# wolny/pytorch-3dunet

Measured on AMD Instinct MI355X. Metric: volumetric patches/sec (fwd+bwd), UNet3D f_maps=32 patch 64x128x128, higher is better.
Workload: dtype f32

## Files before the change

include/u3d.h:

```cpp
#ifndef U3D_H
#define U3D_H

#include <stddef.h>
#include <stdint.h>

#ifdef __cplusplus
extern "C" {
#endif

#define U3D_VERSION 128

#define U3D_OK 0
#define U3D_EINVAL (-1)
#define U3D_EHIP (-2)
#define U3D_EARCH (-3)
#define U3D_EWORKSPACE (-4)

typedef void* u3d_stream_t;

typedef struct {
    const float* p0;
    const float* p1;
    const int32_t* zmap;
    const int32_t* ymap;
    const int32_t* xmap;
    const float* affine;
    int32_t C0, C1;
    int32_t D1, H1, W1;
} u3d_src_t;

int u3d_version(void);
const char* u3d_last_error(void);
int u3d_check_device(int device);
int u3d_set_tuning(int key, int value);
int u3d_set_profile_buffer(void* device_buffer, size_t bytes);
int u3d_debug_stream_pass(int device, u3d_stream_t stream, float* buf, long long n, int blocks, int passes, double min_seconds);
int u3d_debug_mfma_f32_rate(int device, u3d_stream_t stream, float* sink, int iters, int mode, double* flop_out);

size_t u3d_packed_weight_floats(int Cin, int Cout, int mode);
int u3d_pack_weights(int device, u3d_stream_t stream, const float* w, int Cout, int Cin, int mode, float* packed);
typedef struct {
    const float* w;
    float* packed;
    int64_t first;
    int32_t Cout, Cin, mode, cin_stride;
} u3d_pack_desc_t;
int u3d_pack_weights_batch(int device, u3d_stream_t stream, const u3d_pack_desc_t* descs_device, int n,
                           int64_t total_floats);
long long u3d_pack_weights_cells_blocks(const float* w, int Cin, int Cout, int mode, int cin_stride);
int u3d_pack_weights_batch_cells(int device, u3d_stream_t stream, const u3d_pack_desc_t* descs_device, int n, long long total_blocks);

int u3d_conv3d(int device, u3d_stream_t stream, const u3d_src_t* src, const float* packed_w, float* out,
               int N, int D, int H, int W, int Cout, int relu, double* out_stats, const u3d_src_t* gx,
               double* gstats);

int u3d_conv3d_residual(int device, u3d_stream_t stream, const u3d_src_t* src, const float* packed_w, float* out,
                        int N, int D, int H, int W, int Cout, int relu, double* out_stats, const float* residual);

long long u3d_conv3d_workspace_floats(int N, int D, int H, int W, int Cin, int Cout);
int u3d_conv3d_ex(int device, u3d_stream_t stream, const u3d_src_t* src, const float* packed_w, float* out, int N,
                  int D, int H, int W, int Cout, int relu, double* out_stats, const u3d_src_t* gx, double* gstats,
                  const float* residual, float* workspace, long long workspace_floats);

int u3d_conv3d_ex_reps(int device, u3d_stream_t stream, const u3d_src_t* src, const float* packed_w, float* out, int N,
                       int D, int H, int W, int Cout, int relu, double* out_stats, const u3d_src_t* gx, double* gstats,
                       const float* residual, float* workspace, long long workspace_floats, int stat_reps);

long long u3d_subpixel_packed_floats(int C1, int Cout);
long long u3d_subpixel_dgrad_packed_floats(int Cout, int C1);
int u3d_pack_subpixel_dgrad_weights(int device, u3d_stream_t stream, const float* w, int Cout, int Cin_total, int c_off,
                                    int C1, float* packed);
int u3d_subpixel_conv_dgrad(int device, u3d_stream_t stream, const float* dz, const float* packed, const float* x_low,
                            float* dlow, double* gstats, int N, int D1, int H1, int W1, int C1, int Cout);
int u3d_subpixel_conv_dgrad_reps(int device, u3d_stream_t stream, const float* dz, const float* packed, const float* x_low, float* dlow,
                                 double* gstats, int N, int D1, int H1, int W1, int C1, int Cout, int reps);
int u3d_pack_subpixel_weights(int device, u3d_stream_t stream, const float* w, int Cout, int Cin_total, int c_off, int C1,
                              float* packed);
long long u3d_subpixel_fwd_workspace_floats(int N, int D1, int H1, int W1, int C1, int Cout);
int u3d_subpixel_conv_fwd(int device, u3d_stream_t stream, const float* low, const float* affine,
                          long long affine_sample_stride, const float* packed, float* out, int N, int D1, int H1, int W1,
                          int C1, int Cout, float* workspace, long long workspace_floats);

size_t u3d_wgrad_workspace_floats(int N, int D, int H, int W, int Cin, int Cout);
int u3d_conv3d_wgrad(int device, u3d_stream_t stream, const u3d_src_t* src, const float* dz, float* dw, int N,
                     int D, int H, int W, int Cout, float* workspace, size_t workspace_floats);

int u3d_conv3d_variant(int N, int D, int H, int W, int Cin, int Cout, int src_kind, int has_workspace);
int u3d_conv3d_wgrad_variant(int N, int D, int H, int W, int Cin, int Cout, int src_kind);

int u3d_conv3d_wgrad_strided(int device, u3d_stream_t stream, const u3d_src_t* src, const float* dz, float* dw,
                             int dw_cin_stride, int N, int D, int H, int W, int Cout, float* workspace,
                             size_t workspace_floats);

typedef struct u3d_gn_bwd_job {
    const double* gstats_lo;
    const double* gstats_hi;
    const float* mean_rstd;
    const float* gamma;
    float* dgamma;
    float* dbeta;
    float* coef;
    float* coef_hi;
    double count;
    int32_t C0, C1, N, G;
    float hi_scale;
    int32_t reps_lo;
    int32_t reps_hi;
    int32_t reserved;
} u3d_gn_bwd_job_t;
int u3d_conv3d_wgrad_job_supported(int N, int C, int G);
int u3d_conv3d_wgrad_job(int device, u3d_stream_t stream, const u3d_src_t* src, const float* dz, float* dw, int dw_cin_stride,
                         int N, int D, int H, int W, int Cout, float* workspace, size_t workspace_floats,
                         const u3d_gn_bwd_job_t* job);

long long u3d_subpixel_wgrad_workspace_floats(int N, int D1, int H1, int W1, int C1, int Cout);
int u3d_subpixel_conv_wgrad(int device, u3d_stream_t stream, const float* low, const float* affine,
                            long long affine_sample_stride, const float* dz, float* dw, int dw_cin_stride, int N, int D1,
                            int H1, int W1, int C1, int Cout, float* workspace, long long workspace_floats);

int u3d_subpixel_conv_fwd_win(int device, u3d_stream_t stream, const float* low, const float* affine, long long affine_sample_stride,
                              const float* packed, float* out, int N, int D1, int H1, int W1, int C1, int Cout, const int* win);
int u3d_subpixel_conv_dgrad_win(int device, u3d_stream_t stream, const float* dz, const float* packed, const float* x_low, float* dlow,
                                double* gstats, int N, int D1, int H1, int W1, int C1, int Cout, const int* win);
int u3d_subpixel_conv_wgrad_win(int device, u3d_stream_t stream, const float* low, const float* affine, long long affine_sample_stride,
                                const float* dz, float* dw, int dw_cin_stride, int N, int D1, int H1, int W1, int C1, int Cout,
                                float* workspace, long long workspace_floats, const int* win);
int u3d_conv3d_box(int device, u3d_stream_t stream, const u3d_src_t* src, const float* packed_w, float* out, int N, int D, int H, int W,
                   int Cout, const int* out_box, const int* in_mask);
int u3d_conv3d_wgrad_box(int device, u3d_stream_t stream, const u3d_src_t* src, const float* dz, float* dw, int N, int D, int H, int W,
                         int Cout, float* workspace, size_t workspace_floats, const int* box);
int u3d_gn_bwd_apply_children(int device, u3d_stream_t stream, const float* dlow, const float* x, const float* coef, int Ctot, int coff,
                              int N, int D1, int H1, int W1, int C, int ez, int ey, int ex, int relu_mask, float* out);
int u3d_chan_stats_children(int device, u3d_stream_t stream, const float* x_low, int N, int D1, int H1, int W1, int C, int ez, int ey,
                            int ex, double* stats);
int u3d_nearest_childsum_add(int device, u3d_stream_t stream, const float* dv, const float* x_low, float* dlow, double* gstats, int N,
                             int D, int H, int W, int D1, int H1, int W1, int C, const int32_t* zlo, const int32_t* ylo,
                             const int32_t* xlo, int cz, int cy, int cx);

int u3d_conv3d_small_cin_fwd(int device, u3d_stream_t stream, const float* x, const float* affine, const float* w,
                             float* out, int N, int D, int H, int W, int Cin, int Cout, int relu, double* out_stats);
int u3d_conv3d_small_cin_fwd_reps(int device, u3d_stream_t stream, const float* x, const float* affine, const float* w, float* out, int N,
                                  int D, int H, int W, int Cin, int Cout, int relu, double* out_stats, int reps);
size_t u3d_small_cin_bwd_workspace_floats(int N, int D, int H, int W, int Cin, int Cout);
int u3d_conv3d_small_cin_bwd(int device, u3d_stream_t stream, const float* x, const float* affine, const float* dz,
                             const float* w, float* dw, double* gstats, int N, int D, int H, int W, int Cin, int Cout,
                             float* workspace, size_t workspace_floats);

int u3d_conv3d_naive(int device, u3d_stream_t stream, const u3d_src_t* src, const float* w, float* out, int N,
                     int D, int H, int W, int Cin, int Cout, int relu, int flip);

int u3d_chan_stats(int device, u3d_stream_t stream, const u3d_src_t* src, int N, int D, int H, int W,
                   double* stats);
int u3d_chan_stats_reps(int device, u3d_stream_t stream, const u3d_src_t* src, int N, int D, int H, int W, double* stats, int reps);
int u3d_gn_finalize(int device, u3d_stream_t stream, const double* stats0, int C0, double scale0,
                    const double* stats1, int C1, double scale1, int N, int G, double count, const float* gamma,
                    const float* beta, float eps, float* affine, float* mean_rstd);

int u3d_gn_bwd_finalize(int device, u3d_stream_t stream, const double* gstats, const float* mean_rstd,
                        const float* gamma, int N, int C, int G, double count, float* dgamma, float* dbeta,
                        float* coef);
int u3d_gn_finalize_split(int device, u3d_stream_t stream, const double* stats0, int C0, double scale0, const double* stats1, int C1,
                          double scale1, int N, int G, double count, const float* gamma, const float* beta, float eps, float* affine,
                          float* mean_rstd, int Csplit, float* affine_lo, float* affine_hi);
int u3d_gn_finalize_reps(int device, u3d_stream_t stream, const double* stats0, int C0, double scale0, int reps0, const double* stats1,
                         int C1, double scale1, int reps1, int N, int G, double count, const float* gamma, const float* beta, float eps,
                         float* affine, float* mean_rstd, int Csplit, float* affine_lo, float* affine_hi);
int u3d_gn_bwd_finalize_split_supported(int N, int C, int G);
int u3d_gn_bwd_finalize_split(int device, u3d_stream_t stream, const double* gstats_lo, int C0, const double* gstats_hi, int C1,
                              const float* mean_rstd, const float* gamma, int N, int G, double count, float* dgamma, float* dbeta,
                              float* coef, float hi_scale, float* coef_hi);

int u3d_gn_bwd_apply(int device, u3d_stream_t stream, const float* dg, int Cdg, int coff, const float* x, int Cx,
                     const float* coef, int Ctot, int64_t voxels_per_n, int N, int relu_mask, float* out);

int u3d_gn_bwd_apply_add(int device, u3d_stream_t stream, const float* dg, int Cdg, int coff, const float* x, int Cx,
                         const float* coef, int Ctot, int64_t voxels_per_n, int N, int relu_mask, const float* add,
                         float* out);

int u3d_gn_bwd_apply_up(int device, u3d_stream_t stream, const float* dg, int Cdg, int coff, const float* x1,
                        int C1, const float* coef, int Ctot, int N, int D, int H, int W, int D1, int H1, int W1,
                        const int32_t* zlo, const int32_t* ylo, const int32_t* xlo, int relu_mask, float* out);

int u3d_maxpool2_fwd(int device, u3d_stream_t stream, const float* x, int N, int D, int H, int W, int C,
                     float* out, uint8_t* argmax, double* out_stats);
int u3d_maxpool2_bwd_merge(int device, u3d_stream_t stream, const float* dg, const float* pooled,
                           const uint8_t* argmax, const float* coef, const float* skip_grad, const float* e,
                           int N, int D, int H, int W, int C, int relu_mask, float* out);
int u3d_maxpool2_bwd_merge_gn(int device, u3d_stream_t stream, const float* dg, const float* pooled,
                              const uint8_t* argmax, const float* coef, const float* skip_dg, int Cdg,
                              const float* skip_coef, int Ctot, const float* e, int N, int D, int H, int W, int C,
                              int relu_mask, float* out);

int u3d_conv1x1_head_fwd(int device, u3d_stream_t stream, const float* x, const float* w, const float* b, int N,
                         int64_t V, int Cin, int Cout, int act, float* logits, float* probs);
int u3d_conv1x1_head_bwd(int device, u3d_stream_t stream, const float* dlogits, const float* x, const float* w,
                         int N, int64_t V, int Cin, int Cout, int relu_mask, float* dx, double* acc);
int u3d_conv1x1_head_bwd_reps(int device, u3d_stream_t stream, const float* dlogits, const float* x, const float* w, int N, int64_t V,
                              int Cin, int Cout, int relu_mask, float* dx, double* acc, int reps);
int u3d_cvt_f64_f32(int device, u3d_stream_t stream, const double* src, float* dst, int64_t n);
int u3d_cvt_f64_f32_sum(int device, u3d_stream_t stream, const double* src, float* dst, int64_t n, int reps);

typedef struct {
    float* p;
    const float* g;
    float* m;
    float* v;
    int64_t first;
    int64_t numel;
} u3d_adam_desc_t;
int u3d_adam_step(int device, u3d_stream_t stream, const u3d_adam_desc_t* descs_device, int n, int64_t total_padded, double lr,
                  double beta1, double beta2, double eps, double weight_decay, int64_t step);

int u3d_conv1x1_fwd(int device, u3d_stream_t stream, const float* x, const float* w, const float* bias, float* y, int N,
                    int64_t V, int Cin, int Cout, double* out_stats);
int u3d_conv1x1_bwd(int device, u3d_stream_t stream, const float* dy, const float* x, const float* w, int N, int64_t V,
                    int Cin, int Cout, float* dx, double* acc);
int u3d_pack_convtr_weights(int device, u3d_stream_t stream, const float* w, int Cin, int Cout, int mode, float* packed);
int u3d_convtr3d_fwd(int device, u3d_stream_t stream, const float* x, const float* w, float* t, int N, int D1, int H1,
                     int W1, int Cin, int Cout, const float* packed);
long long u3d_convtr3d_subpixel_packed_floats(int Cin, int Cout);
int u3d_pack_convtr3d_subpixel(int device, u3d_stream_t stream, const float* w, int Cin, int Cout, float* packed);
int u3d_convtr3d_fwd_subpixel(int device, u3d_stream_t stream, const float* x, const float* packed, float* t, int N, int D1,
                              int H1, int W1, int Cin, int Cout);
int u3d_convtr3d_bwd(int device, u3d_stream_t stream, const float* dt, const float* x, const float* w, int N, int D1,
                     int H1, int W1, int Cin, int Cout, int relu_mask, float* dx, double* acc, const float* packed_t);
int u3d_nearest_add_fwd(int device, u3d_stream_t stream, const float* skip, const float* t, const int32_t* zmap,
                        const int32_t* ymap, const int32_t* xmap, int N, int D, int H, int W, int Dt, int Ht, int Wt, int C,
                        float* out, double* out_stats);
int u3d_nearest_sum_bwd(int device, u3d_stream_t stream, const float* dj, const int32_t* zlo, const int32_t* ylo,
                        const int32_t* xlo, int N, int D, int H, int W, int Dt, int Ht, int Wt, int C, float* dt);

int u3d_se_gate_fwd(int device, u3d_stream_t stream, const double* ystats, double count, const float* w1, const float* b1,
                    const float* w2, const float* b2, int N, int C, int Cr, float* s, float* h, float* gc);
int u3d_se_apply_fwd(int device, u3d_stream_t stream, const float* y, const float* gc, const float* ws, const float* bs, int N,
                     int64_t V, int C, int mode, float* out, float* a);
int u3d_se_bwd_reduce(int device, u3d_stream_t stream, const float* dout, const float* y, const float* gc, const float* a,
                      const float* ws, int N, int64_t V, int C, int mode, float* dls, double* acc_gc, double* acc_ws);
int u3d_se_gate_bwd(int device, u3d_stream_t stream, const double* acc_gc, const float* gc, const float* h, const float* s,
                    const float* w1, const float* w2, int N, int C, int Cr, double count, float* dz2, float* dz1, float* ds,
                    float* dw1, float* db1, float* dw2, float* db2);
int u3d_se_bwd_apply(int device, u3d_stream_t stream, const float* dout, const float* y, const float* gc, const float* a,
                     const float* ws, const float* dls, const float* ds, int N, int64_t V, int C, int mode, int relu_mask,
                     float* out);

long long u3d_bce_dice_scratch_doubles(int N, int C, int64_t V);
int u3d_bce_dice_fwd(int device, u3d_stream_t stream, const float* logits, const float* target, const float* weight,
                     int N, int C, int64_t V, float w_bce, float w_dice, float eps, double* sums, float* loss,
                     float* coef);
int u3d_bce_dice_bwd(int device, u3d_stream_t stream, const float* logits, const float* target, const float* coef,
                     const float* grad_out, int N, int C, int64_t V, float* dlogits);

int u3d_conv3d_bf16_supported(int Cin, int Cout);
long long u3d_packed_weight_bf16_elems(int Cin, int Cout, int mode);
int u3d_pack_weights_bf16(int device, u3d_stream_t stream, const float* w, int Cout, int Cin, int mode, void* packed);
long long u3d_pack_weights_bf16_blocks(int Cin, int Cout, int mode);
int u3d_pack_weights_bf16_batch(int device, u3d_stream_t stream, const u3d_pack_desc_t* descs_device, int n, long long total_blocks);
int u3d_conv3d_bf16(int device, u3d_stream_t stream, const float* x, const float* affine, const void* packed_w, float* out,
                    int N, int D, int H, int W, int Cin, int Cout, int relu, double* out_stats, const float* gx,
                    double* gstats, const float* residual);
long long u3d_conv3d_bf16_workspace_floats(int N, int D, int H, int W, int Cin, int Cout);
int u3d_conv3d_bf16_tile_variant(int N, int D, int H, int W, int Cin, int Cout, int b16);
int u3d_conv3d_bf16_ex(int device, u3d_stream_t stream, const float* x, const float* affine, const void* packed_w, float* out,
                       int N, int D, int H, int W, int Cin, int Cout, int relu, double* out_stats, const float* gx,
                       double* gstats, const float* residual, float* workspace, long long workspace_floats);

long long u3d_packed_weight_f32s_elems(int Cin, int Cout, int mode);
// ... 125 lines not shown
```

pytorch-3dunet_amd/csrc/u3d_conv.hip:

```cpp
#include <type_traits>
#include <utility>

#include "u3d_common.h"
#include "u3d_gn.h"
#include "u3d_subpix.h"

int g_u3d_tune[24] = {0};

namespace cv {
constexpr int TZ = 4, TY = 8, TX = 8;
constexpr int HZ = TZ + 2, HY = TY + 2, HX = TX + 2;
constexpr int CC = 16;
constexpr int CS = 16;
constexpr int RS = HX * CS + 4;
constexpr int PS = HY * RS;
constexpr int TILE_FLOATS = HZ * PS + 4;
constexpr int CNT_OFF = 2 * TILE_FLOATS;
constexpr int RED_OFF = CNT_OFF + 16;
constexpr int LDS_FLOATS = RED_OFF + 4 * 3 * 32 * 2;
constexpr int NITEMS = HZ * HY * HX * (CC / 4);
constexpr int NIT = (NITEMS + 255) / 256;
constexpr int NSTEP = 27 * (CC / 8);
constexpr int NSTEP_PAIRY = 36 * (CC / 8);
constexpr int NSTEP_N16 = 27;
// ... 965 lines not shown
            using X1 = std::integral_constant<int, 0xB1>;
            using X2 = std::integral_constant<int, 0x4E>;
            const int vrow = ((n * D + z) * H + T.y0) * W + T.x0 + vl;
            const int xrow = ((n * p.gx.D1 + (z >> 1)) * p.gx.H1 + (T.y0 >> 1)) * p.gx.W1 + ((T.x0 + vl) >> 1);
#pragma unroll
            for (int nt = 0; nt < NT; ++nt) {
                f32x4 q1 = {0.f, 0.f, 0.f, 0.f}, q2 = {0.f, 0.f, 0.f, 0.f};
                f32x4 tq[4 * MT];
#pragma unroll
                for (int mt = 0; mt < MT; ++mt)
#pragma unroll
                    for (int bi = 0; bi < 4; ++bi) {
                        const float a0 = acc[mt][nt][4 * bi + 0], a1 = acc[mt][nt][4 * bi + 1];
                        const float a2 = acc[mt][nt][4 * bi + 2], a3 = acc[mt][nt][4 * bi + 3];
                        const float t0 = xlane(a1, X1{}), t1 = xlane(a0, X1{}), t2 = xlane(a3, X1{}), t3 = xlane(a2, X1{});
                        const float c0 = odd ? t0 : a0, c1 = odd ? a1 : t1, c2 = odd ? t2 : a2, c3 = odd ? a3 : t3;
                        const float u0 = xlane(c2, X2{}), u2 = xlane(c0, X2{}), u1 = xlane(c3, X2{}), u3 = xlane(c1, X2{});
                        tq[4 * mt + bi] = f32x4{hi ? u0 : c0, hi ? u1 : c1, hi ? c2 : u2, hi ? c3 : u3};
                    }
                const int ysh = PAIRY ? (cq >> 2) : 0;
                const int co = PAIRY ? 4 * (cq & 3) : (cb * NT + nt) * 32 + 4 * cq;
                auto yoff = [&](int st) { return PAIRY ? 2 * st + ysh : st; };
                const bool cok = co < p.Cout && (!RAG || T.x0 + vl < W);
                auto row_in = [&](int st) { return !RAG || (z < D && T.y0 + yoff(st) < H); };
                float* orow = p.out + (size_t)vrow * p.Cout + co;
                const bool xfrom0 = co < p.gx.C0 || !cok;
                const float* xb = !cok ? p.gx.p0 : (xfrom0 ? p.gx.p0 + co : p.gx.p1 + (co - p.gx.C0));
                const int xcs = xfrom0 ? p.gx.C0 : p.gx.C1;
#pragma unroll
                for (int half = 0; half < MT; ++half) {
                    f32x4 xv[4];
                    if (want_g) {
#pragma unroll
                        for (int k = 0; k < 4; ++k) {
                            const int yo = yoff(4 * half + k);
                            int xi = xfrom0 ? vrow + yo * W : xrow + (yo >> 1) * p.gx.W1;
                            if constexpr (RAG) xi = (cok && row_in(4 * half + k)) ? xi : 0;
                            xv[k] = *reinterpret_cast<const f32x4*>(xb + (size_t)xi * xcs);
                        }
                    } else if (p.res) {
#pragma unroll
                        for (int k = 0; k < 4; ++k) {
                            size_t ri = (size_t)(vrow + yoff(4 * half + k) * W) * p.Cout + (cok ? co : 0);
                            if constexpr (RAG) ri = (cok && row_in(4 * half + k)) ? ri : 0;
                            xv[k] = *reinterpret_cast<const f32x4*>(p.res + ri);
                        }
                    }
#pragma unroll
                    for (int k = 0; k < 4; ++k) {
                        const int st = 4 * half + k;
                        if (!row_in(st)) continue;
                        f32x4 val = tq[st];
                        if (p.res) val += xv[k];
                        if (p.relu) {
#pragma unroll
                            for (int e = 0; e < 4; ++e) val[e] = fmaxf(val[e], 0.f);
                        }
                        if (cok) *reinterpret_cast<f32x4*>(orow + (size_t)yoff(st) * W * p.Cout) = val;
                        if (RAG || p.Cout % 32 != 0) {
#pragma unroll
                            for (int e = 0; e < 4; ++e) val[e] = cok ? val[e] : 0.f;
                        }
                        q1 += val;
                        q2 += want_g ? val * xv[k] : val * val;
                    }
                }
                if (want_stats || want_g) {
                    if constexpr (CARRY) {
                        sq1 += q1;
                        sq2 += q2;
                    } else {
                        stat_reduce(q1, q2, n, nt, co - (PAIRY ? 0 : (cb * NT + nt) * 32));
                    }
                }
            }
        }
        if (ntiles == DBG_TILE) U3D_DBG_STAMP(22);
        ++ntiles;
        if (!has_next_tile || TN.n != T.n || TN.cb != T.cb) {
            if constexpr (CARRY) {
                if (want_stats || want_g) {
                    if constexpr (N16) {
#pragma unroll
                        for (int e = 0; e < 4; ++e) {
                            float a = sq1[e], b2 = sq2[e];
#pragma unroll
                            for (int msk = 8; msk > 0; msk >>= 1) {
                                a += __shfl_xor(a, msk);
                                b2 += __shfl_xor(b2, msk);
                            }
                            if (v16 == 0) {
                                double* r = &red[(((T.n & 1) * NT) * 32 + 4 * kq + e) * 2];
                                __hip_atomic_fetch_add(r, (double)a, __ATOMIC_RELAXED, __HIP_MEMORY_SCOPE_WORKGROUP);
                                __hip_atomic_fetch_add(r + 1, (double)b2, __ATOMIC_RELAXED, __HIP_MEMORY_SCOPE_WORKGROUP);
                            }
                        }
                    } else {
                        const int cq_ = (l >> 2) & 7;
                        stat_reduce(sq1, sq2, T.n, 0, PAIRY ? 4 * (cq_ & 3) : 4 * cq_);
                    }
                    sq1 = f32x4{0.f, 0.f, 0.f, 0.f};
                    sq2 = f32x4{0.f, 0.f, 0.f, 0.f};
                }
            }
            flush_stats(T.n, T.cb);
        }
        if (!has_next_tile) break;
        if constexpr (!ZEROC) {
#pragma unroll
            for (int mt = 0; mt < MT; ++mt)
#pragma unroll
                for (int nt = 0; nt < NT; ++nt)
#pragma unroll
                    for (int r = 0; r < 16; ++r) acc[mt][nt][r] = 0.f;
        }
        wi = nwi;
        dT = dTN;
        T = TN;
        wq = wqn;
    }
    if constexpr (DBG) {
        if (l == 0) dbgw[4] = ntiles;
    }
    U3D_DBG_STAMP(6);
}

namespace wg {
constexpr int TZ = 2, TY = 8, TX = 8;
constexpr int HZ = TZ + 2, HY = TY + 2, HX = TX + 2;
constexpr int CC = 32;
constexpr int CSg = 32, RSg = HX * CSg, PSg = HY * RSg;
constexpr int G_FLOATS = HZ * PSg;
constexpr int TV = TZ * TY * TX;
constexpr int DZ_FLOATS = TV * 32;
constexpr int DUMMY_OFF = G_FLOATS + DZ_FLOATS;
constexpr int BUF_FLOATS = G_FLOATS + DZ_FLOATS + 4;
constexpr int LDS_FLOATS = 2 * BUF_FLOATS;
constexpr int NTHR = 512;
constexpr int NITEMS_G = HZ * HY * HX * (CC / 4);
constexpr int NIT_G = (NITEMS_G + NTHR - 1) / NTHR;
constexpr int NIT_DZ = TV * 8 / NTHR;
constexpr int MAX_MAP_INTS = 4096;
}

struct WgradParams {
    u3d_src_t src;
    const float* dz;
    float* partial;
    int N, D, H, W, Cout;
    int nchunks, nkb, S;
    int tz, ty, tx, ntiles, tps;
    int vec, dzvec;
    int bz0, by0, bx0, bz1, by1, bx1;
};

template <bool VEC, bool REG = false, bool PAIR = false>
__global__ __launch_bounds__(512, 2) void conv3d_wgrad_kernel(const WgradParams p) {
    using namespace wg;
    constexpr int NA = PAIR ? 4 : 7;
    extern __shared__ __attribute__((aligned(16))) float lds[];
    int* zmapl = reinterpret_cast<int*>(lds + 2 * BUF_FLOATS);
    __builtin_amdgcn_s_setprio(3);
    const int t = threadIdx.x;
    const int l = t & 63, i = l & 31, h = l >> 5;
    const int w = __builtin_amdgcn_readfirstlane(t >> 6);
    const int tg = w & 3, hf = w >> 2;

    const int logical = u3d_xcd_remap(blockIdx.x, gridDim.x);
    const int kb = logical % p.nkb;
    const int chunk = (logical / p.nkb) % p.nchunks;
    const int s = logical / (p.nkb * p.nchunks);
    const int D = p.D, H = p.H, W = p.W;
    const int Ctot = p.src.C0 + p.src.C1;
    int* ymapl = zmapl + D;
    int* xmapl = ymapl + H;
    if (p.src.C1 > 0) {
        for (int k = t; k < D; k += NTHR) zmapl[k] = p.src.zmap[k];
        for (int k = t; k < H; k += NTHR) ymapl[k] = p.src.ymap[k];
        for (int k = t; k < W; k += NTHR) xmapl[k] = p.src.xmap[k];
        __syncthreads();
    }

    f32x16 acc[NA];
#pragma unroll
    for (int k = 0; k < NA; ++k)
#pragma unroll
        for (int r = 0; r < 16; ++r) acc[k][r] = 0.f;

    const int q = t & 7, tv = t >> 3;
    const int cq = chunk * CC + 4 * q;
    const int co = kb * 32 + 4 * q;
    const bool cok = cq < Ctot, from0 = cq < p.src.C0, dcok = co < p.Cout;
    const float* gbase = !cok ? p.src.p0 : (from0 ? p.src.p0 + cq : p.src.p1 + (cq - p.src.C0));
    const int Cs = (from0 || !cok) ? p.src.C0 : p.src.C1;
    const float* dzbase = p.dz + (dcok ? co : 0);

    constexpr int NPFC = NIT_G + NIT_DZ;
    int rel[NPFC], loff[NPFC];
    unsigned fz0 = 0, fz1 = 0, fy0 = 0, fy1 = 0, fx0 = 0, fx1 = 0, fdead = 0;
    if constexpr (REG) {
        const int vz = D % TZ ? D % TZ : TZ, vy = H % TY ? H % TY : TY, vx = W % TX ? W % TX : TX;
#pragma unroll
        for (int it = 0; it < NIT_G; ++it) {
            const int vox = tv + 64 * it;
            const int hz = vox / (HY * HX);
            const int rem = vox - hz * (HY * HX);
            const int hy = rem / HX;
            const int hx = rem - hy * HX;
            const bool in = vox < HZ * HY * HX;
            rel[it] = from0 ? ((hz - 1) * H + (hy - 1)) * W + (hx - 1)
                            : (((hz - 1) >> 1) * p.src.H1 + ((hy - 1) >> 1)) * p.src.W1 + ((hx - 1) >> 1);
            loff[it] = in ? hz * PSg + hy * RSg + hx * CSg + 4 * q : DUMMY_OFF;
            fz0 |= (in && hz == 0 ? 1u : 0u) << it;
            fz1 |= (in && hz > vz ? 1u : 0u) << it;
            fy0 |= (in && hy == 0 ? 1u : 0u) << it;
            fy1 |= (in && hy > vy ? 1u : 0u) << it;
            fx0 |= (in && hx == 0 ? 1u : 0u) << it;
            fx1 |= (in && hx > vx ? 1u : 0u) << it;
            fdead |= (in && cok ? 0u : 1u) << it;
        }
#pragma unroll
        for (int it = 0; it < NIT_DZ; ++it) {
            const int vox = tv + 64 * it;
            rel[NIT_G + it] = ((vox >> 6) * H + ((vox >> 3) & 7)) * W + (vox & 7);
            loff[NIT_G + it] = G_FLOATS + vox * 32 + 4 * q;
            fz1 |= ((vox >> 6) >= vz ? 1u : 0u) << (NIT_G + it);
            fy1 |= (((vox >> 3) & 7) >= vy ? 1u : 0u) << (NIT_G + it);
            fx1 |= ((vox & 7) >= vx ? 1u : 0u) << (NIT_G + it);
        }
        fdead |= (dcok ? 0u : 3u) << NIT_G;
    }
    auto tile_invalid = [&](int z0, int y0, int x0) {
        unsigned inv = fdead;
        inv |= z0 == 0 ? fz0 : 0u;
        inv |= z0 + TZ >= D ? fz1 : 0u;
        inv |= y0 == 0 ? fy0 : 0u;
        inv |= y0 + TY >= H ? fy1 : 0u;
        inv |= x0 == 0 ? fx0 : 0u;
        inv |= x0 + TX >= W ? fx1 : 0u;
        return inv;
    };

    struct TileC {
        int n, z0, y0, x0;
        int base, dzb;
        unsigned inv;
    };
    struct TileIdx {
        int xi, yi, zi, n;
    };
    auto tile_decode = [&](int tile) {
        TileIdx d;
        d.xi = tile % p.tx;
        tile /= p.tx;
        d.yi = tile % p.ty;
        tile /= p.ty;
        d.zi = tile % p.tz;
        d.n = tile / p.tz;
        return d;
    };
    auto tile_next = [&](const TileIdx& a) {
        TileIdx r = a;
        r.xi += 1;
        int c = r.xi >= p.tx ? 1 : 0;
        r.xi = c ? 0 : r.xi;
        r.yi += c;
        c = r.yi >= p.ty ? 1 : 0;
        r.yi = c ? 0 : r.yi;
        r.zi += c;
        c = r.zi >= p.tz ? 1 : 0;
        r.zi = c ? 0 : r.zi;
        r.n += c;
        return r;
    };
    auto tile_coords = [&](const TileIdx& d) {
        TileC c;
        c.x0 = (REG ? 0 : p.bx0) + d.xi * TX;
        c.y0 = (REG ? 0 : p.by0) + d.yi * TY;
        c.z0 = (REG ? 0 : p.bz0) + d.zi * TZ;
        c.n = d.n;
        c.base = c.dzb = 0;
        c.inv = 0;
        if constexpr (REG) {
            c.dzb = ((c.n * D + c.z0) * H + c.y0) * W + c.x0;
            const int b1 = ((c.n * p.src.D1 + (c.z0 >> 1)) * p.src.H1 + (c.y0 >> 1)) * p.src.W1 + (c.x0 >> 1);
            c.base = from0 ? c.dzb : b1;
            c.inv = tile_invalid(c.z0, c.y0, c.x0);
        }
        return c;
    };
    auto g_item = [&](const TileC& c, int it, int& off, bool& ok, int& idx) {
        const int vox = tv + 64 * it;
        const int hz = vox / (HY * HX);
        const int rem = vox - hz * (HY * HX);
        const int hy = rem / HX;
        const int hx = rem - hy * HX;
        off = vox < HZ * HY * HX ? hz * PSg + hy * RSg + hx * CSg + 4 * q : DUMMY_OFF;
        const int gz = c.z0 - 1 + hz, gy = c.y0 - 1 + hy, gxx = c.x0 - 1 + hx;
        ok = cok && vox < HZ * HY * HX && gz >= 0 && gz < D && gy >= 0 && gy < H && gxx >= 0 && gxx < W;
        const int zc = min(max(gz, 0), D - 1), yc = min(max(gy, 0), H - 1), xc = min(max(gxx, 0), W - 1);
        idx = ((c.n * D + zc) * H + yc) * W + xc;
        if (p.src.C1 > 0) {
            const int idx1 = ((c.n * p.src.D1 + zmapl[zc]) * p.src.H1 + ymapl[yc]) * p.src.W1 + xmapl[xc];
            idx = from0 ? idx : idx1;
        }
        idx = ok ? idx : 0;
    };
    auto dz_item = [&](const TileC& c, int it, bool& ok, int& idx) {
        const int vox = tv + 64 * it;
        const int z = c.z0 + (vox >> 6), y = c.y0 + ((vox >> 3) & 7), x = c.x0 + (vox & 7);
        ok = dcok && z < p.bz1 && y < p.by1 && x < p.bx1;
        idx = ok ? ((c.n * D + z) * H + y) * W + x : 0;
    };
    auto load_affine = [&](int n, f32x4& ga, f32x4& gb) {
        ga = f32x4{1.f, 1.f, 1.f, 1.f};
        gb = f32x4{0.f, 0.f, 0.f, 0.f};
        if (p.src.affine) {
            const float* ap = p.src.affine + ((size_t)n * Ctot + (cok ? cq : 0)) * 2;
            const f32x4 lo = *reinterpret_cast<const f32x4*>(ap);
            const f32x4 hi = *reinterpret_cast<const f32x4*>(ap + 4);
            ga = f32x4{lo[0], lo[2], hi[0], hi[2]};
            gb = f32x4{lo[1], lo[3], hi[1], hi[3]};
        }
    };
    auto pf_load = [&](const TileC& c, int k) {
        bool ok;
        int idx, off;
        if constexpr (REG) {
            ok = ((c.inv >> k) & 1u) == 0;
            if (k < NIT_G) return *reinterpret_cast<const f32x4*>(gbase + (size_t)(ok ? c.base + rel[k] : 0) * Cs);
            return *reinterpret_cast<const f32x4*>(dzbase + (size_t)(ok ? c.dzb + rel[k] : 0) * p.Cout);
        }
        if (k < NIT_G) {
            g_item(c, k, off, ok, idx);
            return *reinterpret_cast<const f32x4*>(gbase + (size_t)idx * Cs);
        }
        dz_item(c, k - NIT_G, ok, idx);
        return *reinterpret_cast<const f32x4*>(dzbase + (size_t)idx * p.Cout);
    };
    auto pf_store = [&](float* buf, const TileC& c, int k, f32x4 raw, const f32x4& ga, const f32x4& gb) {
        bool ok;
        int idx, off;
        if constexpr (REG) {
            ok = ((c.inv >> k) & 1u) == 0;
            f32x4 val = k < NIT_G ? raw * ga + gb : raw;
#pragma unroll
            for (int e = 0; e < 4; ++e) val[e] = ok ? val[e] : 0.f;
            *reinterpret_cast<f32x4*>(&buf[loff[k]]) = val;
            return;
        }
        if (k < NIT_G) {
            g_item(c, k, off, ok, idx);
            f32x4 val = raw * ga + gb;
#pragma unroll
            for (int e = 0; e < 4; ++e) val[e] = ok ? val[e] : 0.f;
            *reinterpret_cast<f32x4*>(&buf[off]) = val;
        } else {
            dz_item(c, k - NIT_G, ok, idx);
#pragma unroll
            for (int e = 0; e < 4; ++e) raw[e] = ok ? raw[e] : 0.f;
            *reinterpret_cast<f32x4*>(&buf[G_FLOATS + (tv + 64 * (k - NIT_G)) * 32 + 4 * q]) = raw;
        }
    };
    auto stage_scalar = [&](float* buf, const TileC& c) {
        f32x4 ga, gb;
        u3d_load_affine(p.src.affine, c.n, Ctot, cq, false, ga, gb);
#pragma unroll 1
        for (int it = 0; it < NIT_G; ++it) {
            const int vox = tv + 64 * it;
            if (vox >= HZ * HY * HX) continue;
            const int hz = vox / (HY * HX), rem = vox - hz * (HY * HX), hy = rem / HX, hx = rem - hy * HX;
            const int gz = c.z0 - 1 + hz, gy = c.y0 - 1 + hy, gxx = c.x0 - 1 + hx;
            f32x4 val = {0.f, 0.f, 0.f, 0.f};
            if (gz >= 0 && gz < D && gy >= 0 && gy < H && gxx >= 0 && gxx < W) {
                int v0, v1;
                u3d_vox_index(p.src, c.n, gz, gy, gxx, D, H, W, v0, v1);
                val = u3d_load_quad(p.src, v0, v1, cq, false) * ga + gb;
            }
            *reinterpret_cast<f32x4*>(&buf[hz * PSg + hy * RSg + hx * CSg + 4 * q]) = val;
        }
#pragma unroll 1
        for (int it = 0; it < NIT_DZ; ++it) {
            const int vox = tv + 64 * it;
            const int z = c.z0 + (vox >> 6), y = c.y0 + ((vox >> 3) & 7), x = c.x0 + (vox & 7);
            f32x4 val = {0.f, 0.f, 0.f, 0.f};
            if (z < p.bz1 && y < p.by1 && x < p.bx1) {
                const float* sp = p.dz + ((size_t)((c.n * D + z) * H + y) * W + x) * p.Cout + co;
#pragma unroll
                for (int e = 0; e < 4; ++e)
                    if (co + e < p.Cout) val[e] = sp[e];
            }
            *reinterpret_cast<f32x4*>(&buf[G_FLOATS + vox * 32 + 4 * q]) = val;
        }
    };

    constexpr int NPF = NIT_G + NIT_DZ;
    constexpr int ST0 = 20;
    static_assert(2 * (NPF - 1) < ST0 && ST0 + NPF <= 32, "prefetch schedule must fit the 32 groups of a tile");
    const int tile_begin = s * p.tps, tile_end = min(p.ntiles, (s + 1) * p.tps);

    TileIdx tix = tile_decode(tile_begin);
    if (tile_begin < tile_end) {
        const TileC c = tile_coords(tix);
        if constexpr (VEC) {
            f32x4 ga, gb;
            load_affine(c.n, ga, gb);
            f32x4 v[NPF];
#pragma unroll
            for (int k = 0; k < NPF; ++k) v[k] = pf_load(c, k);
#pragma unroll
            for (int k = 0; k < NPF; ++k) pf_store(lds, c, k, v[k], ga, gb);
        } else {
            stage_scalar(lds, c);
        }
    }
    __syncthreads();

    int abase[NA];
#pragma unroll
    for (int k = 0; k < NA; ++k) {
        const int tap = PAIR ? 2 * (tg + 4 * k) + (i >> 4) : tg + 4 * k;
        const int toff = tap < 27 ? (tap / 9) * PSg + ((tap / 3) % 3) * RSg + (tap % 3) * CSg : 0;
        abase[k] = (PAIR ? (i & 15) : i) + h * CSg + hf * PSg + toff;
    }
    int bbase = G_FLOATS + (hf * 64 + h) * 32 + i;
    int cur = 0;
    __builtin_amdgcn_s_setprio(0);

    f32x4 gan = {1.f, 1.f, 1.f, 1.f}, gbn = {0.f, 0.f, 0.f, 0.f};
    int n_aff = -1;
    for (int tile = tile_begin; tile < tile_end; ++tile) {
        const bool has_next = tile + 1 < tile_end;
        if (has_next) tix = tile_next(tix);
        const TileC cn = tile_coords(tix);
        float* nbuf = lds + (cur ^ 1) * BUF_FLOATS;
        f32x4 v[NPF];
        if constexpr (VEC) {
            if (cn.n != n_aff) {
                load_affine(cn.n, gan, gbn);
                n_aff = cn.n;
            }
        }
        const float* gl = lds + cur * BUF_FLOATS;

        float aop[2][NA], bop[2];
        bop[0] = gl[bbase];
#pragma unroll
        for (int k = 0; k < NA; ++k) aop[0][k] = gl[abase[k]];
#pragma unroll
        for (int g = 0; g < 32; ++g) {
            if constexpr (VEC) {
                if (g % 2 == 0 && g / 2 < NPF) v[g / 2] = pf_load(cn, g / 2);
                if (g >= ST0 && g - ST0 < NPF) pf_store(nbuf, cn, g - ST0, v[g - ST0], gan, gbn);
            }
            if (g + 1 < 32) {
                const int row = (g + 1) >> 2, tq = (g + 1) & 3;
                const int goff = row * RSg + 2 * tq * CSg;
                bop[(g + 1) & 1] = gl[bbase + (row * 8 + 2 * tq) * 32];
#pragma unroll
                for (int k = 0; k < NA; ++k) aop[(g + 1) & 1][k] = gl[abase[k] + goff];
            }
            __builtin_amdgcn_sched_barrier(0);
#pragma unroll
            for (int k = 0; k < NA; ++k) acc[k] = __builtin_amdgcn_mfma_f32_32x32x2f32(aop[g & 1][k], bop[g & 1], acc[k], 0, 0, 0);
            __builtin_amdgcn_sched_barrier(0);
        }
        if constexpr (!VEC) {
            if (has_next) stage_scalar(nbuf, cn);
        }
        __syncthreads();
        cur ^= 1;
    }

    __builtin_amdgcn_s_setprio(3);
    float* red = lds;
    if (hf == 1) {
#pragma unroll
        for (int k = 0; k < NA; ++k)
#pragma unroll
            for (int r = 0; r < 16; ++r) red[((tg * 7 + k) * 16 + r) * 64 + l] = acc[k][r];
    }
    __syncthreads();
    if (hf == 0) {
        float* dst = p.partial + ((size_t)((s * p.nchunks + chunk) * p.nkb + kb) * 27) * 1024;
#pragma unroll
        for (int k = 0; k < NA; ++k) {
#pragma unroll
            for (int r = 0; r < 16; ++r) {
                const int row = (r & 3) + 8 * (r >> 2) + 4 * h;
                const int tap = PAIR ? 2 * (tg + 4 * k) + (row >> 4) : tg + 4 * k;
                const int c = PAIR ? (row & 15) : row;
                if (tap < 27) dst[((size_t)tap * 32 + c) * 32 + i] = acc[k][r] + red[((tg * 7 + k) * 16 + r) * 64 + l];
            }
        }
    }
}

template <int G>
__global__ __launch_bounds__(256) void wgrad_reduce_kernel(const float* __restrict__ partial, float* __restrict__ dw,
                                                           int S, int nchunks, int nkb, int Cin, int Cout, int cstride,
                                                           int has_job, u3d_gn_bwd_job_t job) {
    __shared__ float red[4][64];
    if (has_job && blockIdx.x == 0) {
        extern __shared__ double shb[];
        u3d_gn_bwd_finalize_body(job.gstats_lo, job.mean_rstd, job.gamma, job.N, job.C0 + job.C1, job.G, job.count, 1, 1, job.dgamma,
                                 job.dbeta, job.coef, job.gstats_hi, job.C0, job.hi_scale, job.coef_hi, shb, job.reps_lo, job.reps_hi);
        return;
    }
    const long long total = (long long)Cin * 27 * Cout;
    const int lane = G == 1 ? (int)threadIdx.x : (int)(threadIdx.x & 63), grp = G == 1 ? 0 : (int)(threadIdx.x >> 6);
    const long long idx = (long long)(blockIdx.x - (has_job ? 1 : 0)) * (G == 1 ? 256 : 64) + lane;
    float sum = 0.f;
    int k = 0, tap = 0, c = 0;
    if (idx < total) {
        k = (int)(idx % Cout);
        const long long r = idx / Cout;
        tap = (int)(r % 27);
        c = (int)(r / 27);
        const int chunk = c >> 5, kb = k >> 5;
        const size_t off = ((size_t)(chunk * nkb + kb) * 27 + tap) * 1024 + (c & 31) * 32 + (k & 31);
        const size_t sstride = (size_t)nchunks * nkb * 27 * 1024;
        const int per = (S + G - 1) / G;
        const int s0 = grp * per, s1 = min(S, s0 + per);
        float a0 = 0.f, a1 = 0.f, a2 = 0.f, a3 = 0.f;
        int s = s0;
        for (; s + 3 < s1; s += 4) {
            a0 += partial[(size_t)s * sstride + off];
            a1 += partial[(size_t)(s + 1) * sstride + off];
            a2 += partial[(size_t)(s + 2) * sstride + off];
            a3 += partial[(size_t)(s + 3) * sstride + off];
        }
        for (; s < s1; ++s) a0 += partial[(size_t)s * sstride + off];
        sum = (a0 + a1) + (a2 + a3);
    }
    if constexpr (G == 1) {
        if (idx < total) dw[((size_t)k * cstride + c) * 27 + tap] = sum;
    } else {
        red[grp][lane] = sum;
        __syncthreads();
        if (grp == 0 && idx < total)
            dw[((size_t)k * cstride + c) * 27 + tap] = (red[0][lane] + red[1][lane]) + (red[2][lane] + red[3][lane]);
    }
}

__device__ __forceinline__ int pack_image_of(long long idx, int nchunks, int ntot, long long& id) {
    const long long std_total = ((long long)nchunks * cv::NSTEP + cv::PACK_PAD) * ntot * 256;
    const long long pair_total = ((long long)nchunks * cv::NSTEP_PAIRY + cv::PACK_PAD) * 256;
    if (idx < std_total) {
        id = idx;
        return 0;
    }
    if (idx < std_total + pair_total) {
        id = idx - std_total;
        return 1;
    }
    id = idx - std_total - pair_total;
    return 2;
}

__device__ __forceinline__ float pack_elem_n16(const float* __restrict__ w, int Cout, int Cin, int cstride, int mode, int nchunks,
                                               long long id) {
    const int j = (int)(id & 3);
    const int lane = (int)((id >> 2) & 63);
    const long long r = id >> 8;
    const int tap = (int)(r % cv::NSTEP_N16), ch = (int)(r / cv::NSTEP_N16);
    const int kc = ch * 16 + 4 * (lane >> 4) + j, nc = lane & 15;
    if (ch >= nchunks) return 0.f;
    if (mode == 0) return (kc < Cin && nc < Cout) ? w[((size_t)nc * cstride + kc) * 27 + tap] : 0.f;
    return (kc < Cout && nc < Cin) ? w[((size_t)kc * cstride + nc) * 27 + (26 - tap)] : 0.f;
}

__device__ __forceinline__ float pack_elem(const float* __restrict__ w, int Cout, int Cin, int cstride, int mode, int nchunks,
                                           int ntot, long long idx) {
    long long id;
    const int image = pack_image_of(idx, nchunks, ntot, id);
    if (image == 2) return pack_elem_n16(w, Cout, Cin, cstride, mode, nchunks, id);
    const bool pair = image == 1;
    const int j = (int)(id & 3);
    const int lane = (int)((id >> 2) & 63);
    long long r = id >> 8;
    const int nstep = pair ? cv::NSTEP_PAIRY : cv::NSTEP;
    const int ntg = pair ? 0 : (int)(r % ntot);
    if (!pair) r /= ntot;
    const int st = (int)(r % nstep);
    const int ch = (int)(r / nstep);
    const int kc = ch * 16 + 8 * (st & 1) + 4 * (lane >> 5) + j;
    int tap = st >> 1;
    int nc = ntg * 32 + (lane & 31);
    bool tap_ok = true;
    if (pair) {
        const int tz = tap / 12, ty4 = (tap / 3) % 4, tx = tap % 3;
        const int ty = ty4 - ((lane & 31) >> 4);
        tap_ok = ty >= 0 && ty <= 2;
        tap = (tz * 3 + ty) * 3 + tx;
        nc = lane & 15;
    }
    float v = 0.f;
    if (ch >= nchunks || !tap_ok) {
    } else if (mode == 0) {
        if (kc < Cin && nc < Cout) v = w[((size_t)nc * cstride + kc) * 27 + tap];
    } else {
        if (kc < Cout && nc < Cin) v = w[((size_t)kc * cstride + nc) * 27 + (26 - tap)];
    }
    return v;
}
// ... 598 lines not shown
        const dim3 rgrid((unsigned)slots), rblock(256);
        const bool virt = p.src.C1 > 0;
        const bool noaff = p.src.affine == nullptr && g_u3d_tune[7] == 0;
        p.dbg = (!ragged && g_u3d_prof_buf && (size_t)slots * 4 <= g_u3d_prof_records) ? g_u3d_prof_buf : nullptr;
        if (ragged) {
            if (Cout <= 16 && nt == 1 && p.ntot == 1) {
                p.wp = packed_w + ((size_t)p.nchunks * cv::NSTEP + cv::PACK_PAD) * 256 + ((size_t)p.nchunks * cv::NSTEP_PAIRY + cv::PACK_PAD) * 256;
                if (virt)
                    hipLaunchKernelGGL((conv3d_mfma_reg_kernel<1, true, false, false, true, true, true>), rgrid, rblock, shmem, st, p);
                else if (noaff)
                    hipLaunchKernelGGL((conv3d_mfma_reg_kernel<1, false, false, false, false, true, true>), rgrid, rblock, shmem, st, p);
                else
                    hipLaunchKernelGGL((conv3d_mfma_reg_kernel<1, false, false, false, true, true, true>), rgrid, rblock, shmem, st, p);
                U3D_LAUNCH_CHECK();
                return 0;
            }
#define U3D_RAG_LAUNCH(NT_)                                                                                                        \
    do {                                                                                                                           \
        if (virt)                                                                                                                  \
            hipLaunchKernelGGL((conv3d_mfma_reg_kernel<NT_, true, false, false, true, false, true>), rgrid, rblock, shmem, st, p);  \
        else if (noaff)                                                                                                            \
            hipLaunchKernelGGL((conv3d_mfma_reg_kernel<NT_, false, false, false, false, false, true>), rgrid, rblock, shmem, st, p); \
        else                                                                                                                       \
            hipLaunchKernelGGL((conv3d_mfma_reg_kernel<NT_, false, false, false, true, false, true>), rgrid, rblock, shmem, st, p); \
    } while (0)
            if (nt == 3)
                U3D_RAG_LAUNCH(3);
            else if (nt == 2)
                U3D_RAG_LAUNCH(2);
            else
                U3D_RAG_LAUNCH(1);
#undef U3D_RAG_LAUNCH
            U3D_LAUNCH_CHECK();
            return 0;
        }
        if (Cout <= 16 && nt == 1 && p.ntot == 1 && !p.dbg && g_u3d_tune[4] != 1) {
            const size_t std_floats = ((size_t)p.nchunks * cv::NSTEP + cv::PACK_PAD) * 256;
            if (g_u3d_tune[4] == 2) {
                p.wp = packed_w + std_floats;
                if (virt)
                    hipLaunchKernelGGL((conv3d_mfma_reg_kernel<1, true, false, true>), rgrid, rblock, shmem, st, p);
                else if (noaff)
                    hipLaunchKernelGGL((conv3d_mfma_reg_kernel<1, false, false, true, false>), rgrid, rblock, shmem, st, p);
                else
                    hipLaunchKernelGGL((conv3d_mfma_reg_kernel<1, false, false, true>), rgrid, rblock, shmem, st, p);
            } else {
                p.wp = packed_w + std_floats + ((size_t)p.nchunks * cv::NSTEP_PAIRY + cv::PACK_PAD) * 256;
                if (virt)
                    hipLaunchKernelGGL((conv3d_mfma_reg_kernel<1, true, false, false, true, true>), rgrid, rblock, shmem, st, p);
                else if (noaff)
                    hipLaunchKernelGGL((conv3d_mfma_reg_kernel<1, false, false, false, false, true>), rgrid, rblock, shmem, st, p);
                else
                    hipLaunchKernelGGL((conv3d_mfma_reg_kernel<1, false, false, false, true, true>), rgrid, rblock, shmem, st, p);
            }
            U3D_LAUNCH_CHECK();
            return 0;
        }
#define U3D_REG_LAUNCH(NT_)                                                                                \
    do {                                                                                                   \
        if (p.dbg && virt)                                                                                 \
            hipLaunchKernelGGL((conv3d_mfma_reg_kernel<NT_, true, true>), rgrid, rblock, shmem, st, p);    \
        else if (p.dbg)                                                                                    \
            hipLaunchKernelGGL((conv3d_mfma_reg_kernel<NT_, false, true>), rgrid, rblock, shmem, st, p);   \
        else if (virt)                                                                                     \
            hipLaunchKernelGGL((conv3d_mfma_reg_kernel<NT_, true, false>), rgrid, rblock, shmem, st, p);   \
        else if (noaff)                                                                                    \
            hipLaunchKernelGGL((conv3d_mfma_reg_kernel<NT_, false, false, false, false>), rgrid, rblock,   \
                               shmem, st, p);                                                              \
        else                                                                                               \
            hipLaunchKernelGGL((conv3d_mfma_reg_kernel<NT_, false, false>), rgrid, rblock, shmem, st, p);  \
    } while (0)
        if (nt == 3)
            U3D_REG_LAUNCH(3);
        else if (nt == 2)
            U3D_REG_LAUNCH(2);
        else
            U3D_REG_LAUNCH(1);
#undef U3D_REG_LAUNCH
        U3D_LAUNCH_CHECK();
        return 0;
    }
    const bool vec = p.vec != 0;
    const dim3 grid((unsigned)nblk), block(256);
    p.dbg = (vec && g_u3d_prof_buf && (size_t)nblk * 4 <= g_u3d_prof_records) ? g_u3d_prof_buf : nullptr;
#define U3D_CONV_LAUNCH(NT_)                                                                     \
    do {                                                                                         \
        if (p.dbg && NT_ == 1 && g_u3d_tune[2] == 1)                                             \
            hipLaunchKernelGGL((conv3d_mfma_kernel<1, true, true, 1>), grid, block, shmem, st, p); \
        else if (p.dbg && NT_ == 1 && g_u3d_tune[2] == 2)                                        \
            hipLaunchKernelGGL((conv3d_mfma_kernel<1, true, true, 2>), grid, block, shmem, st, p); \
        else if (p.dbg && NT_ == 1 && g_u3d_tune[2] == 3)                                        \
            hipLaunchKernelGGL((conv3d_mfma_kernel<1, true, true, 3>), grid, block, shmem, st, p); \
        else if (p.dbg && NT_ == 1 && g_u3d_tune[2] == 7)                                        \
            hipLaunchKernelGGL((conv3d_mfma_kernel<1, true, true, 7>), grid, block, shmem, st, p); \
        else if (p.dbg)                                                                          \
            hipLaunchKernelGGL((conv3d_mfma_kernel<NT_, true, true>), grid, block, shmem, st, p); \
        else if (vec)                                                                            \
            hipLaunchKernelGGL((conv3d_mfma_kernel<NT_, true>), grid, block, shmem, st, p);      \
        else                                                                                     \
            hipLaunchKernelGGL((conv3d_mfma_kernel<NT_, false>), grid, block, shmem, st, p);     \
    } while (0)
    if (nt == 3)
        U3D_CONV_LAUNCH(3);
    else if (nt == 2)
        U3D_CONV_LAUNCH(2);
    else
        U3D_CONV_LAUNCH(1);
#undef U3D_CONV_LAUNCH
    U3D_LAUNCH_CHECK();
    return 0;
}

static void wgrad_plan(int N, int D, int H, int W, int Cin, int Cout, WgradParams& p) {
    p.nchunks = cdiv(Cin, 32);
    p.nkb = cdiv(Cout, 32);
    p.tz = cdiv(D, wg::TZ), p.ty = cdiv(H, wg::TY), p.tx = cdiv(W, wg::TX);
    p.ntiles = N * p.tz * p.ty * p.tx;
    const int pairs = p.nchunks * p.nkb;
    const int ncu = 256;
    long long best_cost = -1;
    int best_S = 1;
    for (int rounds = 1; rounds <= 8; ++rounds) {
        int S = (rounds * ncu) / pairs;
        if (S < 1) S = 1;
        if (S > p.ntiles) S = p.ntiles;
        const int tps = cdiv(p.ntiles, S);
        S = cdiv(p.ntiles, tps);
        const long long cost = (long long)cdiv(S * pairs, ncu) * (tps + 2);
        if (best_cost < 0 || cost < best_cost) {
            best_cost = cost;
            best_S = S;
        }
    }
    if (g_u3d_tune[1] > 0) best_S = g_u3d_tune[1] > p.ntiles ? p.ntiles : g_u3d_tune[1];
    p.tps = cdiv(p.ntiles, best_S);
    p.S = cdiv(p.ntiles, p.tps);
}

extern "C" size_t u3d_wgrad_workspace_floats(int N, int D, int H, int W, int Cin, int Cout) {
    WgradParams p;
    wgrad_plan(N, D, H, W, Cin, Cout, p);
    return (size_t)p.S * p.nchunks * p.nkb * 27 * 1024;
}

static int wgrad_set_lds_once(int device) {
    static bool done[64] = {false};
    if (device >= 0 && device < 64 && done[device]) return 0;
    U3D_HIP(hipFuncSetAttribute(reinterpret_cast<const void*>(conv3d_wgrad_kernel<true, true>),
                                hipFuncAttributeMaxDynamicSharedMemorySize, (wg::LDS_FLOATS + wg::MAX_MAP_INTS) * sizeof(float)));
    U3D_HIP(hipFuncSetAttribute(reinterpret_cast<const void*>(conv3d_wgrad_kernel<true, true, true>),
                                hipFuncAttributeMaxDynamicSharedMemorySize, (wg::LDS_FLOATS + wg::MAX_MAP_INTS) * sizeof(float)));
    U3D_HIP(hipFuncSetAttribute(reinterpret_cast<const void*>(conv3d_wgrad_kernel<true>),
                                hipFuncAttributeMaxDynamicSharedMemorySize, (wg::LDS_FLOATS + wg::MAX_MAP_INTS) * sizeof(float)));
    U3D_HIP(hipFuncSetAttribute(reinterpret_cast<const void*>(conv3d_wgrad_kernel<false>),
                                hipFuncAttributeMaxDynamicSharedMemorySize, (wg::LDS_FLOATS + wg::MAX_MAP_INTS) * sizeof(float)));
    if (device >= 0 && device < 64) done[device] = true;
    return 0;
}

static int conv3d_wgrad_impl(int device, u3d_stream_t stream, const u3d_src_t* src, const float* dz, float* dw, int cstride,
                             int N, int D, int H, int W, int Cout, float* workspace, size_t workspace_floats, const int* box = nullptr,
                             const u3d_gn_bwd_job_t* job = nullptr);

extern "C" int u3d_conv3d_wgrad_box(int device, u3d_stream_t stream, const u3d_src_t* src, const float* dz, float* dw, int N, int D,
                                    int H, int W, int Cout, float* workspace, size_t workspace_floats, const int* box) {
    U3D_REQUIRE(box != nullptr, "u3d_conv3d_wgrad_box: box is NULL");
    return conv3d_wgrad_impl(device, stream, src, dz, dw, 0, N, D, H, W, Cout, workspace, workspace_floats, box);
}

extern "C" int u3d_conv3d_wgrad(int device, u3d_stream_t stream, const u3d_src_t* src, const float* dz, float* dw,
                                int N, int D, int H, int W, int Cout, float* workspace, size_t workspace_floats) {
    return conv3d_wgrad_impl(device, stream, src, dz, dw, 0, N, D, H, W, Cout, workspace, workspace_floats);
}

extern "C" int u3d_conv3d_wgrad_strided(int device, u3d_stream_t stream, const u3d_src_t* src, const float* dz, float* dw,
                                        int dw_cin_stride, int N, int D, int H, int W, int Cout, float* workspace,
                                        size_t workspace_floats) {
    U3D_REQUIRE(src && dw_cin_stride >= src->C0 + src->C1, "u3d_conv3d_wgrad_strided: dw_cin_stride < channels of src");
    return conv3d_wgrad_impl(device, stream, src, dz, dw, dw_cin_stride, N, D, H, W, Cout, workspace, workspace_floats);
}

static size_t wgrad_job_lds_bytes(int N, int C, int G) { return sizeof(double) * (4 * (size_t)N * C + 2 * (size_t)N * G); }

extern "C" int u3d_conv3d_wgrad_job_supported(int N, int C, int G) {
    return (N > 0 && C > 0 && G > 0 && C % G == 0 && wgrad_job_lds_bytes(N, C, G) + 1024 <= 64 * 1024) ? 1 : 0;
}

extern "C" int u3d_conv3d_wgrad_job(int device, u3d_stream_t stream, const u3d_src_t* src, const float* dz, float* dw,
                                    int dw_cin_stride, int N, int D, int H, int W, int Cout, float* workspace,
                                    size_t workspace_floats, const u3d_gn_bwd_job_t* job) {
    U3D_REQUIRE(src && (dw_cin_stride == 0 || dw_cin_stride >= src->C0 + src->C1), "u3d_conv3d_wgrad_job: dw_cin_stride < channels of src");
    if (job) {
        U3D_REQUIRE(job->gstats_lo && job->mean_rstd && job->gamma && job->dgamma && job->dbeta && job->coef && job->C0 > 0 &&
                        job->C1 >= 0 && (job->C1 == 0) == (job->gstats_hi == nullptr) && (job->coef_hi == nullptr || job->C1 > 0) &&
                        job->reps_lo >= 0 && job->reps_lo <= 64 && job->reps_hi >= 0 && job->reps_hi <= 64,
                    "u3d_conv3d_wgrad_job: bad job");
        U3D_REQUIRE(u3d_conv3d_wgrad_job_supported(job->N, job->C0 + job->C1, job->G) == 1,
                    "u3d_conv3d_wgrad_job: the reduction of %d x %d channels in %d groups does not fit one block's LDS", job->N,
                    job->C0 + job->C1, job->G);
    }
    return conv3d_wgrad_impl(device, stream, src, dz, dw, dw_cin_stride, N, D, H, W, Cout, workspace, workspace_floats, nullptr, job);
}

static int conv3d_wgrad_impl(int device, u3d_stream_t stream, const u3d_src_t* src, const float* dz, float* dw, int cstride,
                             int N, int D, int H, int W, int Cout, float* workspace, size_t workspace_floats, const int* box,
                             const u3d_gn_bwd_job_t* job) {
    U3D_ENTER(device);
    if (int e = check_src(src, "u3d_conv3d_wgrad")) return e;
    U3D_REQUIRE(dz && dw && workspace && N > 0 && D > 0 && H > 0 && W > 0 && Cout > 0, "u3d_conv3d_wgrad: bad argument");
    U3D_REQUIRE((long long)N * D * H * W < (1ll << 31), "u3d_conv3d_wgrad: N*D*H*W must be < 2^31");
    WgradParams p;
    const int Cin = src->C0 + src->C1;
    p.bz0 = p.by0 = p.bx0 = 0, p.bz1 = D, p.by1 = H, p.bx1 = W;
    if (box) {
        U3D_REQUIRE(box[0] >= 0 && box[1] >= 0 && box[2] >= 0 && box[3] <= D && box[4] <= H && box[5] <= W && box[0] < box[3] &&
                        box[1] < box[4] && box[2] < box[5], "u3d_conv3d_wgrad_box: box outside the volume or empty");
        p.bz0 = box[0], p.by0 = box[1], p.bx0 = box[2], p.bz1 = box[3], p.by1 = box[4], p.bx1 = box[5];
    }
    wgrad_plan(N, p.bz1 - p.bz0, p.by1 - p.by0, p.bx1 - p.bx0, Cin, Cout, p);
    const size_t need = (size_t)p.S * p.nchunks * p.nkb * 27 * 1024;
    if (workspace_floats < need)
        return u3d_set_err(U3D_EWORKSPACE, "u3d_conv3d_wgrad: workspace %zu < %zu floats", workspace_floats, need);
    p.src = *src;
    p.dz = dz;
    p.partial = workspace;
    p.N = N, p.D = D, p.H = H, p.W = W, p.Cout = Cout;
    p.vec = src_vec_ok(src) ? 1 : 0;
    p.dzvec = (Cout % 4 == 0 && ((uintptr_t)dz & 15) == 0) ? 1 : 0;
    if (int e = wgrad_set_lds_once(device)) return e;
    const int nblk = p.S * p.nchunks * p.nkb;
    U3D_REQUIRE(D + H + W <= wg::MAX_MAP_INTS, "u3d_conv3d_wgrad: D+H+W must be <= %d", wg::MAX_MAP_INTS);
    const size_t shmem = (wg::LDS_FLOATS + (size_t)(D + H + W)) * sizeof(float);
    const bool reg = !box && (g_u3d_tune[3] != 2 || (D % wg::TZ == 0 && H % wg::TY == 0 && W % wg::TX == 0)) &&
                     (src->C1 == 0 || (D == 2 * src->D1 && H == 2 * src->H1 && W == 2 * src->W1));
    if (p.vec && p.dzvec && reg && Cin <= 16)
        hipLaunchKernelGGL((conv3d_wgrad_kernel<true, true, true>), dim3(nblk), dim3(wg::NTHR), shmem, (hipStream_t)stream, p);
    else if (p.vec && p.dzvec && reg)
        hipLaunchKernelGGL((conv3d_wgrad_kernel<true, true>), dim3(nblk), dim3(wg::NTHR), shmem, (hipStream_t)stream, p);
    else if (p.vec && p.dzvec)
        hipLaunchKernelGGL(conv3d_wgrad_kernel<true>, dim3(nblk), dim3(wg::NTHR), shmem, (hipStream_t)stream, p);
    else
        hipLaunchKernelGGL(conv3d_wgrad_kernel<false>, dim3(nblk), dim3(wg::NTHR), shmem, (hipStream_t)stream, p);
    U3D_LAUNCH_CHECK();
    const long long total = (long long)Cin * 27 * Cout;
    const bool one_group = p.S <= 16 && g_u3d_tune[23] != 1;
    const int rblocks = (int)((total + (one_group ? 255 : 63)) / (one_group ? 256 : 64));
    u3d_gn_bwd_job_t jb = {};
    size_t job_lds = 0;
    if (job) {
        jb = *job;
        if (!jb.gstats_hi) jb.C1 = 0, jb.hi_scale = 1.0f, jb.coef_hi = nullptr;
        if (jb.reps_lo < 1) jb.reps_lo = 1;
        if (jb.reps_hi < 1 || !jb.gstats_hi) jb.reps_hi = 1;
        job_lds = wgrad_job_lds_bytes(jb.N, jb.C0 + jb.C1, jb.G);
    }
    if (one_group)
        hipLaunchKernelGGL(wgrad_reduce_kernel<1>, dim3(rblocks + (job ? 1 : 0)), dim3(256), job_lds, (hipStream_t)stream, workspace, dw, p.S,
                           p.nchunks, p.nkb, Cin, Cout, cstride > 0 ? cstride : Cin, job ? 1 : 0, jb);
    else
        hipLaunchKernelGGL(wgrad_reduce_kernel<4>, dim3(rblocks + (job ? 1 : 0)), dim3(256), job_lds, (hipStream_t)stream, workspace, dw, p.S,
                           p.nchunks, p.nkb, Cin, Cout, cstride > 0 ? cstride : Cin, job ? 1 : 0, jb);
    U3D_LAUNCH_CHECK();
    return 0;
}

extern "C" int u3d_conv3d_variant(int N, int D, int H, int W, int Cin, int Cout, int src_kind, int has_workspace) {
    if (N <= 0 || D <= 0 || H <= 0 || W <= 0 || Cin <= 0 || Cout <= 0) return -1;
    if (Cin % 4 != 0 || Cout % 4 != 0) return 0;
    const long long ntiles = (long long)N * cdiv(D, cv::TZ) * cdiv(H, cv::TY) * cdiv(W, cv::TX);
    const int nchunks = cdiv(Cin, 16), ntot = cdiv(Cout, 32);
    if (has_workspace && splitk_shape(N, D, H, W, Cin, Cout) && g_u3d_tune[7] != 2) {
        if (splitk_count(g_u3d_ncu_seen, ntiles, ntot, nchunks, nullptr) >= 2) return 3;
    }
    const bool ragged = D % cv::TZ != 0 || H % cv::TY != 0 || W % cv::TX != 0;
    if (src_kind == 2 || g_u3d_tune[3] == 1 || (g_u3d_tune[3] == 2 && ragged)) return 0;
    return ragged ? 2 : 1;
}

extern "C" int u3d_conv3d_wgrad_variant(int N, int D, int H, int W, int Cin, int Cout, int src_kind) {
    if (N <= 0 || D <= 0 || H <= 0 || W <= 0 || Cin <= 0 || Cout <= 0) return -1;
    if (Cin % 4 != 0 || Cout % 4 != 0) return 0;
    const bool ragged = D % wg::TZ != 0 || H % wg::TY != 0 || W % wg::TX != 0;
    if (src_kind == 2 || (g_u3d_tune[3] == 2 && ragged)) return 0;
    return (ragged ? 2 : 1) | (Cin <= 16 ? 4 : 0);
}

extern "C" int u3d_conv3d_naive(int device, u3d_stream_t stream, const u3d_src_t* src, const float* w, float* out,
                                int N, int D, int H, int W, int Cin, int Cout, int relu, int flip) {
    U3D_ENTER(device);
    if (int e = check_src(src, "u3d_conv3d_naive")) return e;
    U3D_REQUIRE(w && out && Cin == src->C0 + src->C1, "u3d_conv3d_naive: bad argument");
    const long long total = (long long)N * D * H * W * Cout;
    const int blocks = (int)((total + 255) / 256 > 65536 ? 65536 : (total + 255) / 256);
    hipLaunchKernelGGL(conv3d_naive_kernel, dim3(blocks), dim3(256), 0, (hipStream_t)stream, *src, w, out, N, D, H,
                       W, Cin, Cout, relu, flip);
    U3D_LAUNCH_CHECK();
    return 0;
}
```

pytorch-3dunet_amd/csrc/u3d_gn.h:

```cpp
#pragma once
#include "u3d_common.h"

__device__ __forceinline__ double u3d_sum_replicas(const double* __restrict__ p, size_t stride, int reps) {
    double v = p[0];
    for (int r0 = 1; r0 < reps; r0 += 8) {
        double t[8];
#pragma unroll
        for (int j = 0; j < 8; ++j) t[j] = r0 + j < reps ? p[(size_t)(r0 + j) * stride] : 0.0;
#pragma unroll
        for (int j = 0; j < 8; ++j) v += t[j];
    }
    return v;
}

__device__ inline void u3d_gn_bwd_finalize_body(const double* __restrict__ gs, const float* __restrict__ mean_rstd,
                                                const float* __restrict__ gamma, int N, int C, int G, double count, int staged, int par,
                                                float* __restrict__ dgamma, float* __restrict__ dbeta, float* __restrict__ coef,
                                                const double* __restrict__ gs_hi, int C0, float hi_scale, float* __restrict__ coef_hi,
                                                double* shb, int reps = 1, int reps_hi = 1) {

#pragma clang fp contract(off)
    const double* src = gs;
    if (staged) {
        if (gs_hi) {
            const int C1 = C - C0;
            for (int i = threadIdx.x; i < N * C * 2; i += blockDim.x) {
                const int e = i & 1, nc = i >> 1, n = nc / C, c = nc - n * C;
                shb[i] = c < C0 ? u3d_sum_replicas(gs + ((size_t)n * C0 + c) * 2 + e, (size_t)N * C0 * 2, reps)
                                : u3d_sum_replicas(gs_hi + ((size_t)n * C1 + (c - C0)) * 2 + e, (size_t)N * C1 * 2, reps_hi);
            }
        } else {
            for (int i = threadIdx.x; i < N * C * 2; i += blockDim.x) shb[i] = u3d_sum_replicas(gs + i, (size_t)N * C * 2, reps);
        }
        __syncthreads();
        src = shb;
    }
    const int cpg = C / G;
    const double m = count * cpg;
    double* pa = shb + 2 * (size_t)N * C;
    double* pb = pa + (size_t)N * C;
    double* qr = pb + (size_t)N * C;
    if (par) {
        for (int i = threadIdx.x; i < N * C; i += blockDim.x) {
            const int n = i / C, c = i - n * C, g = c / cpg;
            const double mean = (double)mean_rstd[((size_t)n * G + g) * 2], rstd = (double)mean_rstd[((size_t)n * G + g) * 2 + 1];
            const double S1 = src[(size_t)i * 2], S2 = src[(size_t)i * 2 + 1], gm = (double)gamma[c];
            pa[i] = gm * S1;
            pb[i] = gm * rstd * (S2 - mean * S1);
        }
        __syncthreads();
    }
    for (int pair = threadIdx.x; pair < N * G; pair += blockDim.x) {
        const int n = pair / G, g = pair - n * G;
        const double mean = (double)mean_rstd[(size_t)pair * 2], rstd = (double)mean_rstd[(size_t)pair * 2 + 1];
        double A = 0.0, B = 0.0;
        for (int c = g * cpg; c < (g + 1) * cpg; ++c) {
            if (par) {
                A += pa[(size_t)n * C + c];
                B += pb[(size_t)n * C + c];
            } else {
                const double S1 = src[((size_t)n * C + c) * 2], S2 = src[((size_t)n * C + c) * 2 + 1];
                const double gm = (double)gamma[c];
                A += gm * S1;
                B += gm * rstd * (S2 - mean * S1);
            }
        }
        const double q = -rstd * rstd * B / m;
        const double r = -rstd * A / m + rstd * rstd * mean * B / m;
        if (par) {
            qr[(size_t)pair * 2] = q;
            qr[(size_t)pair * 2 + 1] = r;
        } else {
            for (int c = g * cpg; c < (g + 1) * cpg; ++c) {
                coef[((size_t)n * 3 + 0) * C + c] = (float)(rstd * (double)gamma[c]);
                coef[((size_t)n * 3 + 1) * C + c] = (float)q;
                coef[((size_t)n * 3 + 2) * C + c] = (float)r;
            }
        }
    }
    if (par) {
        __syncthreads();
        for (int i = threadIdx.x; i < N * C; i += blockDim.x) {
            const int n = i / C, c = i - n * C, pair = n * G + c / cpg;
            const double rstd = (double)mean_rstd[(size_t)pair * 2 + 1];
            const float fp = (float)(rstd * (double)gamma[c]), fq = (float)qr[(size_t)pair * 2], fr = (float)qr[(size_t)pair * 2 + 1];
            coef[((size_t)n * 3 + 0) * C + c] = fp;
            coef[((size_t)n * 3 + 1) * C + c] = fq;
            coef[((size_t)n * 3 + 2) * C + c] = fr;
            if (coef_hi && c >= C0) {
                const int C1 = C - C0;
                coef_hi[((size_t)n * 3 + 0) * C1 + (c - C0)] = fp;
                coef_hi[((size_t)n * 3 + 1) * C1 + (c - C0)] = fq * hi_scale;
                coef_hi[((size_t)n * 3 + 2) * C1 + (c - C0)] = fr * hi_scale;
            }
        }
    }
    for (int c = threadIdx.x; c < C; c += blockDim.x) {
        const int g = c / cpg;
        double dg = 0.0, db = 0.0;
        for (int n = 0; n < N; ++n) {
            const double mean = (double)mean_rstd[((size_t)n * G + g) * 2], rstd = (double)mean_rstd[((size_t)n * G + g) * 2 + 1];
            const double S1 = src[((size_t)n * C + c) * 2], S2 = src[((size_t)n * C + c) * 2 + 1];
            dg += rstd * (S2 - mean * S1);
            db += S1;
        }
        dgamma[c] = (float)dg;
        dbeta[c] = (float)db;
    }
}
```

pytorch-3dunet_amd/csrc/u3d_ops.hip:

```cpp
#include "u3d_common.h"
#include "u3d_gn.h"

#include <string.h>

extern int g_u3d_tune[24];

static thread_local char g_err[512] = "";

int u3d_set_err(int code, const char* fmt, ...) {
    va_list ap;
    va_start(ap, fmt);
    vsnprintf(g_err, sizeof(g_err), fmt, ap);
    va_end(ap);
    return code;
}

int u3d_device_guard::enter(int device) {
    hipError_t e = hipGetDevice(&prev);
    if (e != hipSuccess) return u3d_set_err(U3D_EHIP, "hipGetDevice failed: %s", hipGetErrorString(e));
    if (device >= 0 && prev != device) {
        e = hipSetDevice(device);
        if (e != hipSuccess) return u3d_set_err(U3D_EHIP, "hipSetDevice(%d) failed: %s", device, hipGetErrorString(e));
        switched = true;
    }
// ... 318 lines not shown
        double s, ss;
        if (c < C0) {
            const double* q = st0 + ((size_t)n * C0 + c) * 2;
            s = sc0 * u3d_sum_replicas(q, (size_t)gridDim.x * C0 * 2, reps0);
            ss = sc0 * u3d_sum_replicas(q + 1, (size_t)gridDim.x * C0 * 2, reps0);
        } else {
            const double* q = st1 + ((size_t)n * C1 + (c - C0)) * 2;
            s = sc1 * u3d_sum_replicas(q, (size_t)gridDim.x * C1 * 2, reps1);
            ss = sc1 * u3d_sum_replicas(q + 1, (size_t)gridDim.x * C1 * 2, reps1);
        }
        sh[2 * c] = s;
        sh[2 * c + 1] = ss;
    }
    __syncthreads();
    for (int g = t; g < G; g += blockDim.x) {
        double s = 0.0, ss = 0.0;
        for (int c = g * cpg; c < (g + 1) * cpg; ++c) {
            s += sh[2 * c];
            ss += sh[2 * c + 1];
        }
        const double m = count * cpg;
        const double mean = s / m;
        double var = ss / m - mean * mean;
        if (var < 0.0) var = 0.0;
        const double rstd = 1.0 / sqrt(var + (double)eps);
        gmr[2 * g] = mean;
        gmr[2 * g + 1] = rstd;
        mean_rstd[((size_t)n * G + g) * 2] = (float)mean;
        mean_rstd[((size_t)n * G + g) * 2 + 1] = (float)rstd;
    }
    __syncthreads();
    for (int c = t; c < C; c += blockDim.x) {
        const int g = c / cpg;
        const double a = gmr[2 * g + 1] * (double)gamma[c];
        const float fa = (float)a, fb = (float)((double)beta[c] - gmr[2 * g] * a);
        affine[((size_t)n * C + c) * 2] = fa;
        affine[((size_t)n * C + c) * 2 + 1] = fb;
        if (affine_lo && c < Cs) {
            affine_lo[((size_t)n * Cs + c) * 2] = fa;
            affine_lo[((size_t)n * Cs + c) * 2 + 1] = fb;
        }
        if (affine_hi && c >= Cs) {
            affine_hi[((size_t)n * (C - Cs) + (c - Cs)) * 2] = fa;
            affine_hi[((size_t)n * (C - Cs) + (c - Cs)) * 2 + 1] = fb;
        }
    }
}

static int gn_finalize_impl(int device, u3d_stream_t stream, const double* stats0, int C0, double scale0, const double* stats1, int C1,
                            double scale1, int N, int G, double count, const float* gamma, const float* beta, float eps, float* affine,
                            float* mean_rstd, float* affine_lo, float* affine_hi, int Csplit, int reps0 = 1, int reps1 = 1) {
    U3D_ENTER(device);
    const int C = C0 + C1;
    U3D_REQUIRE(reps0 >= 1 && reps0 <= 64 && reps1 >= 1 && reps1 <= 64, "u3d_gn_finalize_reps: replica counts must be 1 .. 64");
    U3D_REQUIRE(stats0 && C0 > 0 && C1 >= 0 && (C1 == 0 || stats1) && gamma && beta && affine && mean_rstd && N > 0 && G > 0 &&
                    count > 0.0 && Csplit >= 0 && Csplit <= C, "u3d_gn_finalize: bad argument");
    U3D_REQUIRE(C % G == 0, "u3d_gn_finalize: channels %d not divisible by groups %d", C, G);
    U3D_REQUIRE(C <= 4096, "u3d_gn_finalize: more than 4096 channels");
    hipLaunchKernelGGL(gn_finalize_kernel, dim3(N), dim3(256), sizeof(double) * 2 * ((size_t)C + G), (hipStream_t)stream,
                       stats0, C0, scale0, stats1, C1, scale1, N, G, count, gamma, beta, eps, affine, mean_rstd, affine_lo, affine_hi, Csplit,
                       reps0, reps1);
    U3D_LAUNCH_CHECK();
    return 0;
}

extern "C" int u3d_gn_finalize(int device, u3d_stream_t stream, const double* stats0, int C0, double scale0,
                               const double* stats1, int C1, double scale1, int N, int G, double count,
                               const float* gamma, const float* beta, float eps, float* affine, float* mean_rstd) {
    return gn_finalize_impl(device, stream, stats0, C0, scale0, stats1, C1, scale1, N, G, count, gamma, beta, eps, affine, mean_rstd,
                            nullptr, nullptr, 0);
}

extern "C" int u3d_gn_finalize_split(int device, u3d_stream_t stream, const double* stats0, int C0, double scale0,
                                     const double* stats1, int C1, double scale1, int N, int G, double count,
                                     const float* gamma, const float* beta, float eps, float* affine, float* mean_rstd,
                                     int Csplit, float* affine_lo, float* affine_hi) {
    return gn_finalize_impl(device, stream, stats0, C0, scale0, stats1, C1, scale1, N, G, count, gamma, beta, eps, affine, mean_rstd,
                            affine_lo, affine_hi, Csplit);
}

extern "C" int u3d_gn_finalize_reps(int device, u3d_stream_t stream, const double* stats0, int C0, double scale0, int reps0,
                                    const double* stats1, int C1, double scale1, int reps1, int N, int G, double count,
                                    const float* gamma, const float* beta, float eps, float* affine, float* mean_rstd,
                                    int Csplit, float* affine_lo, float* affine_hi) {
    return gn_finalize_impl(device, stream, stats0, C0, scale0, stats1, C1, scale1, N, G, count, gamma, beta, eps, affine, mean_rstd,
                            affine_lo, affine_hi, Csplit, reps0, reps1);
}

__global__ __launch_bounds__(256) void gn_bwd_finalize_kernel(const double* __restrict__ gs, const float* __restrict__ mean_rstd,
                                                              const float* __restrict__ gamma, int N, int C, int G,
                                                              double count, int staged, int par, float* __restrict__ dgamma,
                                                              float* __restrict__ dbeta, float* __restrict__ coef,
                                                              const double* __restrict__ gs_hi, int C0, float hi_scale,
                                                              float* __restrict__ coef_hi) {
    extern __shared__ double shb[];
    u3d_gn_bwd_finalize_body(gs, mean_rstd, gamma, N, C, G, count, staged, par, dgamma, dbeta, coef, gs_hi, C0, hi_scale, coef_hi, shb);
}

extern "C" int u3d_gn_bwd_finalize(int device, u3d_stream_t stream, const double* gstats, const float* mean_rstd,
                                   const float* gamma, int N, int C, int G, double count, float* dgamma,
                                   float* dbeta, float* coef) {
    U3D_ENTER(device);
    U3D_REQUIRE(gstats && mean_rstd && gamma && dgamma && dbeta && coef && N > 0 && C > 0 && G > 0 && C % G == 0,
                "u3d_gn_bwd_finalize: bad argument");
    const size_t bytes = sizeof(double) * 2 * (size_t)N * C;
    const int staged = bytes <= 48 * 1024 ? 1 : 0;
    const size_t par_bytes = 2 * bytes + sizeof(double) * 2 * (size_t)N * G;
    const int par = staged && par_bytes <= 64 * 1024 ? 1 : 0;
    hipLaunchKernelGGL(gn_bwd_finalize_kernel, dim3(1), dim3(256), par ? par_bytes : (staged ? bytes : 0), (hipStream_t)stream, gstats,
                       mean_rstd, gamma, N, C, G, count, staged, par, dgamma, dbeta, coef, (const double*)nullptr, C, 1.0f, (float*)nullptr);
    U3D_LAUNCH_CHECK();
    return 0;
}

extern "C" int u3d_gn_bwd_finalize_split_supported(int N, int C, int G) {
    const size_t bytes = sizeof(double) * 2 * (size_t)N * C;
    return (N > 0 && C > 0 && G > 0 && 2 * bytes + sizeof(double) * 2 * (size_t)N * G <= 64 * 1024) ? 1 : 0;
}

extern "C" int u3d_gn_bwd_finalize_split(int device, u3d_stream_t stream, const double* gstats_lo, int C0, const double* gstats_hi,
                                         int C1, const float* mean_rstd, const float* gamma, int N, int G, double count,
                                         float* dgamma, float* dbeta, float* coef, float hi_scale, float* coef_hi) {
    U3D_ENTER(device);
    const int C = C0 + C1;
    U3D_REQUIRE(gstats_lo && gstats_hi && mean_rstd && gamma && dgamma && dbeta && coef && N > 0 && C0 > 0 && C1 > 0 && G > 0 &&
                    C % G == 0, "u3d_gn_bwd_finalize_split: bad argument");
    U3D_REQUIRE(u3d_gn_bwd_finalize_split_supported(N, C, G) == 1, "u3d_gn_bwd_finalize_split: N * C = %d exceeds the staged path", N * C);
    const size_t bytes = sizeof(double) * 2 * (size_t)N * C;
    const size_t par_bytes = 2 * bytes + sizeof(double) * 2 * (size_t)N * G;
    hipLaunchKernelGGL(gn_bwd_finalize_kernel, dim3(1), dim3(256), par_bytes, (hipStream_t)stream, gstats_lo, mean_rstd, gamma, N, C, G,
                       count, 1, 1, dgamma, dbeta, coef, gstats_hi, C0, hi_scale, coef_hi);
    U3D_LAUNCH_CHECK();
    return 0;
}

template <bool VEC, typename T = float>
__global__ void gn_bwd_apply_kernel(const T* __restrict__ dg, int Cdg, int coff, const T* __restrict__ x,
                                    int Cx, const float* __restrict__ coef, int Ctot, long long Vn, int N,
                                    int relu_mask, const T* __restrict__ add, T* __restrict__ out) {
    if (VEC) {
        const int Q = Cx >> 2;
        const long long total = (long long)N * Vn * Q;
        for (long long idx = (long long)blockIdx.x * blockDim.x + threadIdx.x; idx < total;
             idx += (long long)gridDim.x * blockDim.x) {
            const int qd = (int)(idx % Q);
            const long long v = idx / Q;
            const int n = (int)(v / Vn);
            const int c = 4 * qd;
            const f32x4 d = u3d_ldq(dg + (size_t)v * Cdg + coff + c);
            const f32x4 xv = u3d_ldq(x + (size_t)v * Cx + c);
            const f32x4 p = *reinterpret_cast<const f32x4*>(coef + ((size_t)n * 3 + 0) * Ctot + coff + c);
            const f32x4 q = *reinterpret_cast<const f32x4*>(coef + ((size_t)n * 3 + 1) * Ctot + coff + c);
            const f32x4 r = *reinterpret_cast<const f32x4*>(coef + ((size_t)n * 3 + 2) * Ctot + coff + c);
            f32x4 o = p * d + q * xv + r;
            if (add) o += u3d_ldq(add + (size_t)v * Cx + c);
            if (relu_mask) {
#pragma unroll
                for (int e = 0; e < 4; ++e) o[e] = xv[e] > 0.f ? o[e] : 0.f;
            }
            u3d_stq(out + (size_t)v * Cx + c, o);
        }
    } else {
        const long long total = (long long)N * Vn * Cx;
        for (long long idx = (long long)blockIdx.x * blockDim.x + threadIdx.x; idx < total;
             idx += (long long)gridDim.x * blockDim.x) {
            const int c = (int)(idx % Cx);
            const long long v = idx / Cx;
            const int n = (int)(v / Vn);
            const float d = u3d_ld(dg + (size_t)v * Cdg + coff + c);
            const float xv = u3d_ld(x + idx);
            float o = coef[((size_t)n * 3 + 0) * Ctot + coff + c] * d + coef[((size_t)n * 3 + 1) * Ctot + coff + c] * xv +
                      coef[((size_t)n * 3 + 2) * Ctot + coff + c];
            if (add) o += u3d_ld(add + idx);
            if (relu_mask && !(xv > 0.f)) o = 0.f;
            u3d_st(out + idx, o);
        }
    }
}

__global__ __launch_bounds__(256) void gn_bwd_apply_oct_b16_kernel(const __bf16* __restrict__ dg, int Cdg, int coff,
                                                                   const __bf16* __restrict__ x, int Cx, const float* __restrict__ coef,
                                                                   int Ctot, long long Vn, int N, int relu_mask,
                                                                   const __bf16* __restrict__ add, __bf16* __restrict__ out) {
    typedef __bf16 b16x8 __attribute__((ext_vector_type(8)));
    const int Q = Cx >> 3;
    const long long total = (long long)N * Vn * Q;
    for (long long idx = (long long)blockIdx.x * blockDim.x + threadIdx.x; idx < total; idx += (long long)gridDim.x * blockDim.x) {
        const int qd = (int)(idx % Q);
        const long long v = idx / Q;
        const int n = (int)(v / Vn);
        const int c = 8 * qd;
        const b16x8 d8 = *reinterpret_cast<const b16x8*>(dg + (size_t)v * Cdg + coff + c);
        const b16x8 x8 = *reinterpret_cast<const b16x8*>(x + (size_t)v * Cx + c);
        b16x8 a8 = {};
        if (add) a8 = *reinterpret_cast<const b16x8*>(add + (size_t)v * Cx + c);
        const float* cp = coef + ((size_t)n * 3) * Ctot + coff + c;
        b16x8 o8;
#pragma unroll
        for (int hq = 0; hq < 2; ++hq) {
            const f32x4 p = *reinterpret_cast<const f32x4*>(cp + 4 * hq);
            const f32x4 q = *reinterpret_cast<const f32x4*>(cp + Ctot + 4 * hq);
            const f32x4 r = *reinterpret_cast<const f32x4*>(cp + 2 * (size_t)Ctot + 4 * hq);
#pragma unroll
            for (int e = 0; e < 4; ++e) {
                const float xv = (float)x8[4 * hq + e];
                float o = p[e] * (float)d8[4 * hq + e] + q[e] * xv + r[e];
                if (add) o += (float)a8[4 * hq + e];
                if (relu_mask) o = xv > 0.f ? o : 0.f;
                o8[4 * hq + e] = (__bf16)o;
            }
        }
        *reinterpret_cast<b16x8*>(out + (size_t)v * Cx + c) = o8;
    }
}

template <typename T>
static int gn_bwd_apply_impl(int device, u3d_stream_t stream, const T* dg, int Cdg, int coff, const T* x, int Cx,
                             const float* coef, int Ctot, int64_t voxels_per_n, int N, int relu_mask, const T* add,
                             T* out);

extern "C" int u3d_gn_bwd_apply(int device, u3d_stream_t stream, const float* dg, int Cdg, int coff, const float* x,
                                int Cx, const float* coef, int Ctot, int64_t voxels_per_n, int N, int relu_mask,
                                float* out) {
    return gn_bwd_apply_impl<float>(device, stream, dg, Cdg, coff, x, Cx, coef, Ctot, voxels_per_n, N, relu_mask, nullptr, out);
}

extern "C" int u3d_gn_bwd_apply_b16(int device, u3d_stream_t stream, const void* dg, int Cdg, int coff, const void* x, int Cx,
                                    const float* coef, int Ctot, int64_t voxels_per_n, int N, int relu_mask, const void* add,
                                    void* out) {
    return gn_bwd_apply_impl<__bf16>(device, stream, (const __bf16*)dg, Cdg, coff, (const __bf16*)x, Cx, coef, Ctot, voxels_per_n, N,
                                     relu_mask, (const __bf16*)add, (__bf16*)out);
}

extern "C" int u3d_gn_bwd_apply_add(int device, u3d_stream_t stream, const float* dg, int Cdg, int coff, const float* x,
                                    int Cx, const float* coef, int Ctot, int64_t voxels_per_n, int N, int relu_mask,
                                    const float* add, float* out) {
    if (add == nullptr) return u3d_set_err(U3D_EINVAL, "u3d_gn_bwd_apply_add: add is NULL");
    return gn_bwd_apply_impl<float>(device, stream, dg, Cdg, coff, x, Cx, coef, Ctot, voxels_per_n, N, relu_mask, add, out);
}

template <typename T>
static int gn_bwd_apply_impl(int device, u3d_stream_t stream, const T* dg, int Cdg, int coff, const T* x, int Cx,
                             const float* coef, int Ctot, int64_t voxels_per_n, int N, int relu_mask, const T* add,
                             T* out) {
    U3D_ENTER(device);
    U3D_REQUIRE(dg && x && coef && out && Cdg > 0 && Cx > 0 && coff >= 0 && coff + Cx <= Cdg && Ctot >= coff + Cx &&
                    voxels_per_n > 0 && N > 0,
                "u3d_gn_bwd_apply: bad argument");
    const bool vec = (Cdg % 4 == 0) && (Cx % 4 == 0) && (coff % 4 == 0) && (Ctot % 4 == 0) &&
                     (((uintptr_t)dg | (uintptr_t)x | (uintptr_t)out | (uintptr_t)add) & u3d_vec_align<T>::mask) == 0 &&
                     ((uintptr_t)coef & 15) == 0;
    if constexpr (sizeof(T) == 2) {
        if (vec && Cdg % 8 == 0 && Cx % 8 == 0 && coff % 8 == 0 && Ctot % 8 == 0 &&
            (((uintptr_t)dg | (uintptr_t)x | (uintptr_t)out | (uintptr_t)add) & 15) == 0) {
            const long long total = (long long)N * voxels_per_n * (Cx / 8);
            hipLaunchKernelGGL(gn_bwd_apply_oct_b16_kernel, dim3(grid_for(total, 16384)), dim3(256), 0, (hipStream_t)stream,
                               reinterpret_cast<const __bf16*>(dg), Cdg, coff, reinterpret_cast<const __bf16*>(x), Cx, coef, Ctot,
                               (long long)voxels_per_n, N, relu_mask, reinterpret_cast<const __bf16*>(add), reinterpret_cast<__bf16*>(out));
            U3D_LAUNCH_CHECK();
            return 0;
        }
    }
    if (vec) {
        const long long total = (long long)N * voxels_per_n * (Cx / 4);
        hipLaunchKernelGGL((gn_bwd_apply_kernel<true, T>), dim3(grid_for(total, 16384)), dim3(256), 0, (hipStream_t)stream,
                           dg, Cdg, coff, x, Cx, coef, Ctot, (long long)voxels_per_n, N, relu_mask, add, out);
    } else {
        const long long total = (long long)N * voxels_per_n * Cx;
        hipLaunchKernelGGL((gn_bwd_apply_kernel<false, T>), dim3(grid_for(total, 16384)), dim3(256), 0,
                           (hipStream_t)stream, dg, Cdg, coff, x, Cx, coef, Ctot, (long long)voxels_per_n, N,
                           relu_mask, add, out);
    }
    U3D_LAUNCH_CHECK();
    return 0;
}

template <int VW>
__global__ void gn_bwd_apply_up_kernel(const float* __restrict__ dg, int Cdg, int coff, const float* __restrict__ x1,
                                       int C1, const float* __restrict__ coef, int Ctot, int N, int D, int H, int W,
                                       int D1, int H1, int W1, const int* __restrict__ zlo,
                                       const int* __restrict__ ylo, const int* __restrict__ xlo, int relu_mask,
                                       float* __restrict__ out) {
    const int Q = C1 / VW;
    const long long total = (long long)N * D1 * H1 * W1 * Q;
    for (long long idx = (long long)blockIdx.x * blockDim.x + threadIdx.x; idx < total;
         idx += (long long)gridDim.x * blockDim.x) {
        const int c = (int)(idx % Q) * VW;
        long long v = idx / Q;
        const int xx = (int)(v % W1);
        v /= W1;
        const int yy = (int)(v % H1);
        v /= H1;
        const int zz = (int)(v % D1);
        const int n = (int)(v / D1);
        float sum[VW];
#pragma unroll
        for (int k = 0; k < VW; ++k) sum[k] = 0.f;
        int cnt = 0;
        for (int z = zlo[zz]; z < zlo[zz + 1]; ++z)
            for (int y = ylo[yy]; y < ylo[yy + 1]; ++y)
                for (int x = xlo[xx]; x < xlo[xx + 1]; ++x) {
                    const float* src = dg + ((size_t)((n * D + z) * H + y) * W + x) * Cdg + coff + c;
                    if (VW == 4) {
                        const f32x4 t = *reinterpret_cast<const f32x4*>(src);
#pragma unroll
                        for (int k = 0; k < 4; ++k) sum[k] += t[k];
                    } else {
                        sum[0] += src[0];
                    }
                    ++cnt;
                }
        const size_t oi = (size_t)(idx / Q) * C1 + c;
// ... 1158 lines not shown
```

pytorch-3dunet_amd/pytorch3dunet_amd/_engine_base.py:

```python
from __future__ import annotations

import copy
import ctypes
import dataclasses
import os
import threading
from dataclasses import dataclass, field
from typing import List, Optional

import torch
import torch.nn.functional as F

from . import _native as nat
from ._native import U3DSrc

__all__ = [
    "ACT_ELU",
    "ACT_LEAKY",
    "ACT_NONE",
    "ACT_RELU",
    "CkptRec",
    "ConvRec",
    "F",
    "LayerSpec",
# ... 261 lines not shown
        if self.t1 is None:
            return None
        e = tuple(full - 2 * low for full, low in zip((self.D, self.H, self.W), (self.D1, self.H1, self.W1)))
        return e if all(v in (0, 1) for v in e) else None


def slab_boxes(dims, plus, t):
    boxes = []
    lo = [0, 0, 0]
    for a in range(3):
        if not plus[a]:
            continue
        b0, b1 = list(lo), list(dims)
        b1[a] = min(t, dims[a])
        if all(x < y for x, y in zip(b0, b1)):
            boxes.append(tuple(b0) + tuple(b1))
        lo[a] = min(t, dims[a])
    return boxes


ACT_NONE, ACT_RELU, ACT_LEAKY, ACT_ELU = 0, 1, 2, 3


@dataclass(frozen=True)
class LayerSpec:

    norm: Optional[str]
    pre: bool
    act: int
    slope: float
    inner: int
    islope: float
    drop: Optional[str]


_ACTS = {"r": (ACT_RELU, 0.0), "l": (ACT_LEAKY, 0.01), "e": (ACT_ELU, 0.0)}


def layer_spec(order: str) -> Optional[LayerSpec]:
    if not order or any(ch not in "gbcrledD" for ch in order) or order.count("c") != 1:
        return None
    drop = None
    if order[-1] in "dD":
        drop, order = order[-1], order[:-1]
    if any(ch in "dD" for ch in order) or not order:
        return None
    norms = [ch for ch in order if ch in "gb"]
    acts = [ch for ch in order if ch in "rle"]
    if len(norms) > 1 or len(acts) > 1:
        return None
    norm = norms[0] if norms else None
    a, sl = _ACTS[acts[0]] if acts else (ACT_NONE, 0.0)
    if drop and a == ACT_ELU:
        return None
    ci = order.index("c")
    if norm is None:
        return LayerSpec(None, False, a, sl, ACT_NONE, 0.0, drop) if order in ("c", "c" + "".join(acts)) else None
    ni = order.index(norm)
    if ni < ci:
        return LayerSpec(norm, True, a, sl, ACT_NONE, 0.0, drop) if order == norm + "c" + "".join(acts) else None
    if order == "c" + norm + "".join(acts):
        return LayerSpec(norm, False, a, sl, ACT_NONE, 0.0, drop)
    if acts and order == "c" + acts[0] + norm:
        return LayerSpec(norm, False, ACT_NONE, 0.0, a, sl, drop)
    return None


def parse_order(order: str):
    sp = layer_spec(order)
    return None if sp is None else (not sp.pre, sp.act, sp.slope)


@dataclass
class ConvRec:

    name: str
    src: VSrc
    affine: torch.Tensor
    mean_rstd: torch.Tensor
    y: torch.Tensor
    gn_w: torch.Tensor
    conv_w: torch.Tensor
    G: int
    idx_gw: int = -1
    idx_gb: int = -1
    idx_w: int = -1
    small: bool = False
    sub: Optional[tuple] = None
    pre_norm: bool = True
    post: Optional[tuple] = None
    norm: Optional[str] = "g"
    bn_training: bool = True
    drop: Optional[tuple] = None
    affine_lo: Optional[torch.Tensor] = None
    affine_hi: Optional[torch.Tensor] = None


@dataclass
class Tape:
    convs: List[ConvRec] = field(default_factory=list)
    pools: list = field(default_factory=list)
    head_x: Optional[torch.Tensor] = None
    dims: tuple = ()
    x0: Optional[torch.Tensor] = None
    blocks: list = field(default_factory=list)
    ups: list = field(default_factory=list)
    cats: dict = field(default_factory=dict)
    lean: bool = False
    consumed: bool = False
    bwd_pool: Optional[object] = None


class _StatPool:

    def __init__(self, dev, doubles: int):
        self.buf = torch.zeros(max(doubles, 2), dtype=torch.float64, device=dev)
        self.off = 0

    def take(self, n: int) -> torch.Tensor:
        if self.off + n > self.buf.numel():
            self.buf = torch.zeros(max(n, 1 << 16), dtype=torch.float64, device=self.buf.device)
            self.off = 0
        s = self.buf[self.off : self.off + n]
        self.off += n
        return s

    def carve(self, n: int) -> "_StatPool":
        sub = _StatPool.__new__(_StatPool)
        sub.buf = self.take(n)
        sub.off = 0
        return sub


_SIDE_STREAMS: dict = {}


def _side_stream(dev):
    key = (dev.type, dev.index)
    st = _SIDE_STREAMS.get(key)
    if st is None:
        st = _SIDE_STREAMS[key] = torch.cuda.Stream(dev)
    return st


class _BwdCtx:

    SIDE_MAX_VOXELS = int(os.environ.get("U3D_SIDE_VOXELS", 0))

    def __init__(self, dev, pool, ws, flat, engine):
        self.dev, self.pool, self.ws, self.flat = dev, pool, ws, flat
        self._e = engine
        self.side = None
        self.ws_side = None
        self.side_used = False
        self.coef_hi = None

    def gview(self, idx):
        e = self._e
        return self.flat[e.poffs[idx] : e.poffs[idx] + e.params[idx].numel()]

    def ensure_ws(self, floats):
        if self.ws.numel() < floats:
            self.ws = _empty(int(floats), dtype=_F32, device=self.dev)
        return self.ws

    def side_stream(self, ws_floats):
        if self.side is None:
            self.side = _side_stream(self.dev)
        if self.ws_side is None or self.ws_side.numel() < ws_floats:
            if self.ws_side is not None:
                self.join()
            self.ws_side = _empty(max(int(ws_floats), 4), dtype=_F32, device=self.dev)
        return self.side

    def join(self):
        if self.side_used:
            torch.cuda.current_stream(self.dev).wait_stream(self.side)
            self.side_used = False


_ALWAYS_REPACK = os.environ.get("U3D_ALWAYS_REPACK", "0") == "1"




@dataclass
class ResRec:

    name: str
    x_in: torch.Tensor
    r: torch.Tensor
    rec2: ConvRec
    rec3: ConvRec
    conv1: Optional[torch.nn.Module]
    se: Optional[dict] = None


@dataclass
class CkptRec:

    name: str
    bm: torch.nn.Module
    x_in: torch.Tensor
    out: torch.Tensor


@dataclass
class UpRec:

    x_low: torch.Tensor
    weight: torch.Tensor
    los: tuple
    tdims: tuple
    t8: bool = False
    concat: Optional[tuple] = None


_RECORD_TYPES.update({VSrc, ConvRec, Tape, ResRec, CkptRec, UpRec})
```

pytorch-3dunet_amd/pytorch3dunet_amd/_engine_conv.py:

```python
from __future__ import annotations

import copy
import ctypes
import dataclasses
import os
import threading
from dataclasses import dataclass, field
from typing import List, Optional

import torch
import torch.nn.functional as F

from . import _native as nat
from ._native import U3DSrc

from ._engine_base import *

_WGRAD_JOB = os.environ.get("U3D_WGRAD_JOB", "1") != "0"


def _reps(t) -> int:
    return getattr(t, "_u3d_reps", 1) if t is not None else 1


def _take_reps(pool, n: int, reps: int):
    t = pool.take(reps * n)
    if reps > 1:
        t._u3d_reps = reps
    return t


def _fold_reps(t):
    r = _reps(t)
    return t if r == 1 else t.view(r, -1).sum(0)


class _SubLayers(dict):

    plus = frozenset()


@dataclass
class _ConvCall:
    dev: torch.device
    conv: torch.nn.Module
    src: VSrc
    affine: torch.Tensor
    y: torch.Tensor
    N: int
    D: int
    H: int
    W: int
    Ctot: int
    Cout: int
    relu: int
    stats: bool
    pool: _StatPool
    residual: Optional[torch.Tensor]
    sub: dict
    b16: bool
    affine_lo: Optional[torch.Tensor] = None
    affine_hi: Optional[torch.Tensor] = None

    def take_stats(self, reps: int = 1):
        return _take_reps(self.pool, self.N * self.Cout * 2, reps) if self.stats else None

    @property
    def flops(self):
        return 54.0 * self.Ctot * self.Cout * self.N * self.D * self.H * self.W


@dataclass
class _BwdCall:
    cx: "_BwdCtx"
    rec: ConvRec
    dz: torch.Tensor
    src: VSrc
    N: int
    D: int
    H: int
    W: int
    Cout: int
    bf16: bool
    b16: bool
    job: object = None
    greps: int = 1

    @property
    def flops(self):
        return 54.0 * self.src.C * self.Cout * self.N * self.D * self.H * self.W


class ConvLayers:

    def _identity_affine(self, N, C, dev):
        key = ("ida", N, C, str(dev))
        t = self._const.get(key)
        if t is None:
            t = self._const[key] = torch.tensor([1.0, 0.0], dtype=_F32, device=dev).repeat(N, C, 1).contiguous()
        return t

    def _identity_coef(self, N, C, dev):
        key = ("idc", N, C, str(dev))
        t = self._const.get(key)
        if t is None:
            t = self._const[key] = torch.tensor([1.0, 0.0, 0.0], dtype=_F32, device=dev).view(1, 3, 1).repeat(N, 1, C).contiguous()
        return t

    def _unact(self, dev, g, y):
        if self.act in (ACT_LEAKY, ACT_ELU):
            nat.call("u3d_act_bwd", dev.index, _stream(dev), _p(g), _p(y), g.numel(), self.act, self.slope, _p(g))

    def _up_scale(self, dev):
        t = getattr(self, "_up_scale_t", None)
        if t is None or t.device != dev:
            t = self._up_scale_t = torch.tensor([1.0, 8.0, 8.0], dtype=_F32, device=dev).view(1, 3, 1)
        return t

    def _subpixel_layers(self, size):
        if not self.subpixel or any(ct is not None for ct in self.dec_up) or any(self.dec_interp):
            return _SubLayers()
        dims = [tuple(size)]
        for has_pool, _, _ in self.enc:
            if has_pool:
                dims.append(tuple(d // 2 for d in dims[-1]))
        out, plus = _SubLayers(), set()
        L = len(self.enc)
        for j, (c1, _) in enumerate(self.dec):
            skip_lvl, low_lvl = L - 2 - j, L - 1 - j
            if skip_lvl < 0 or low_lvl >= len(dims) or self._cat_bf16(c1):
                continue
            C0 = self.enc[skip_lvl][2].conv.out_channels
            C1 = c1.conv.in_channels - C0
            ratio = [a - 2 * b for a, b in zip(dims[skip_lvl], dims[low_lvl])]
            if (all(r in (0, 1) for r in ratio) and (self.subpixel_plus or not any(ratio)) and C0 > 0 and C1 > 0 and C0 % 4 == 0
                    and C1 % 4 == 0 and c1.conv.out_channels % 4 == 0):
                out[id(c1.conv.weight)] = (C0, C1)
                if any(ratio):
                    plus.add(id(c1.conv.weight))
        self._sub_pairs.update(out)
        out.plus = frozenset(plus)
        return out

    def _stats_of(self, src: VSrc, st0, st1, pool: _StatPool, dev):
        if src.t1 is None:
            if st0 is None:
                st0 = _take_reps(pool, src.N * src.C0 * 2, self.stat_reps)
                s = src.struct()
                nat.call("u3d_chan_stats_reps", dev.index, _stream(dev), ctypes.byref(s), src.N, src.D, src.H, src.W, _p(st0), _reps(st0))
            return st0, src.C0, 1.0, None, 0, 0.0
        if st0 is not None and st1 is not None and src.exact2x and self.fused_stats:
            return st0, src.C0, 1.0, st1, src.C1, 8.0
        plus = src.plus
        if st0 is not None and plus is not None and any(plus) and self.fused_stats and src.C1 % 4 == 0 and src.t1.dtype == _F32:
            st1w = pool.take(src.N * src.C1 * 2)
            nat.call("u3d_chan_stats_children", dev.index, _stream(dev), _p(src.t1), src.N, src.D1, src.H1, src.W1, src.C1, *plus, _p(st1w))
            return st0, src.C0, 1.0, st1w, src.C1, 1.0
        st = _take_reps(pool, src.N * src.C * 2, self.stat_reps)
        s = src.struct()
        nat.call("u3d_chan_stats_reps", dev.index, _stream(dev), ctypes.byref(s), src.N, src.D, src.H, src.W, _p(st), _reps(st))
        return st, src.C, 1.0, None, 0, 0.0

    def _norm_finalize(self, kind, mod, st0, C0, sc0, st1, C1, sc1, N, G, count, affine, dev, split=None):
        r0, r1 = _reps(st0), _reps(st1)
        if kind == "g" and (r0 > 1 or r1 > 1):
            mean_rstd = _empty((N, G, 2), dtype=_F32, device=dev)
            sp = split if split is not None else (0, None, None)
            nat.call("u3d_gn_finalize_reps", dev.index, _stream(dev), _p(st0), C0, sc0, r0, _p(st1), C1, sc1, r1, N, G, count,
                     _p(mod.weight.detach()), _p(mod.bias.detach()), float(mod.eps), _p(affine), _p(mean_rstd), sp[0], _p(sp[1]), _p(sp[2]))
            return mean_rstd
        st0, st1 = _fold_reps(st0), _fold_reps(st1)
        if kind == "g":
            mean_rstd = _empty((N, G, 2), dtype=_F32, device=dev)
            if split is not None:
                nat.call("u3d_gn_finalize_split", dev.index, _stream(dev), _p(st0), C0, sc0, _p(st1), C1, sc1, N, G, count,
                         _p(mod.weight.detach()), _p(mod.bias.detach()), float(mod.eps), _p(affine), _p(mean_rstd), split[0],
                         _p(split[1]), _p(split[2]))
                return mean_rstd
            nat.call("u3d_gn_finalize", dev.index, _stream(dev), _p(st0), C0, sc0, _p(st1), C1, sc1, N, G, count,
                     _p(mod.weight.detach()), _p(mod.bias.detach()), float(mod.eps), _p(affine), _p(mean_rstd))
            return mean_rstd
        C = C0 + C1
        training = bool(mod.training) or mod.running_mean is None
        mean_rstd = _empty((C, 2), dtype=_F32, device=dev)
        momentum = 0.0
        rm, rv = mod.running_mean, mod.running_var
        if training and rm is not None:
            if getattr(self, "_in_recompute", False):
                rm = rv = None
            else:
                mod.num_batches_tracked.add_(1)
                momentum = (1.0 / float(mod.num_batches_tracked.item())) if mod.momentum is None else float(mod.momentum)
        nat.call("u3d_bn_finalize", dev.index, _stream(dev), _p(st0), C0, sc0, _p(st1), C1, sc1, N, count, _p(mod.weight.detach()),
                 _p(mod.bias.detach()), float(mod.eps), 1 if training else 0, momentum, _p(rm), _p(rv), _p(affine), _p(mean_rstd))
        return mean_rstd

    def _norm_bwd_job(self, cx, rec: ConvRec, gst, N, C, count, coef):
        if rec.norm != "g" or not _WGRAD_JOB or nat.get_lib().u3d_conv3d_wgrad_job_supported(N, C, rec.G) != 1:
            return None
        dev, gview = cx.dev, cx.gview
        cx.coef_hi = None
        job = nat.U3DGnBwdJob()
        if isinstance(gst, tuple):
            g0, g1 = gst
            C0 = g0.numel() // (2 * N * _reps(g0))
            coef_hi = _empty((N, 3, C - C0), dtype=_F32, device=dev) if not any(rec.src.plus) else None
            job.gstats_lo, job.gstats_hi, job.C0, job.C1, job.hi_scale, job.coef_hi = _p(g0), _p(g1), C0, C - C0, 8.0, _p(coef_hi)
            cx.coef_hi = coef_hi
        else:
            job.gstats_lo, job.gstats_hi, job.C0, job.C1, job.hi_scale, job.coef_hi = _p(gst), None, C, 0, 1.0, None
        job.reps_lo = _reps(gst[0] if isinstance(gst, tuple) else gst)
        job.reps_hi = _reps(gst[1]) if isinstance(gst, tuple) else 1
        job.mean_rstd, job.gamma = _p(rec.mean_rstd), _p(rec.gn_w.detach())
        job.dgamma, job.dbeta, job.coef = _p(gview(rec.idx_gw)), _p(gview(rec.idx_gb)), _p(coef)
        job.count, job.N, job.G = count, N, rec.G
        return job

    def _norm_bwd_finalize(self, cx, rec: ConvRec, gst, N, C, count, coef):
        dev, gview = cx.dev, cx.gview
        cx.coef_hi = None
        gst = tuple(_fold_reps(g) for g in gst) if isinstance(gst, tuple) else _fold_reps(gst)
        if isinstance(gst, tuple):
            g0, g1 = gst
            C0 = g0.numel() // (2 * N)
            if rec.norm == "g" and nat.get_lib().u3d_gn_bwd_finalize_split_supported(N, C, rec.G) == 1:
                coef_hi = _empty((N, 3, C - C0), dtype=_F32, device=dev) if not any(rec.src.plus) else None
                nat.call("u3d_gn_bwd_finalize_split", dev.index, _stream(dev), _p(g0), C0, _p(g1), C - C0, _p(rec.mean_rstd),
                         _p(rec.gn_w.detach()), N, rec.G, count, _p(gview(rec.idx_gw)), _p(gview(rec.idx_gb)), _p(coef), 8.0, _p(coef_hi))
                cx.coef_hi = coef_hi
                return
            gst = torch.cat((g0.view(N, C0, 2), g1.view(N, C - C0, 2)), dim=1)
        if rec.norm == "g":
            nat.call("u3d_gn_bwd_finalize", dev.index, _stream(dev), _p(gst), _p(rec.mean_rstd), _p(rec.gn_w.detach()), N, C, rec.G,
                     count, _p(gview(rec.idx_gw)), _p(gview(rec.idx_gb)), _p(coef))
        else:
            nat.call("u3d_bn_bwd_finalize", dev.index, _stream(dev), _p(gst), _p(rec.mean_rstd), _p(rec.gn_w.detach()), N, C, count,
                     1 if rec.bn_training else 0, _p(gview(rec.idx_gw)), _p(gview(rec.idx_gb)), _p(coef))

    _FWD_KERNELS = {
# ... 102 lines not shown
        conv_res = None if post else residual
        want_stats = ((post and spec.norm is not None and inner in (ACT_NONE, ACT_RELU))
                      or (not post and want_stats and act in (ACT_NONE, ACT_RELU)))
        bn_training = (bool(gn.training) or gn.running_mean is None) if spec.norm == "b" else True
        split = None
        if post:
            affine, mean_rstd = self._identity_affine(N, Ctot, dev), None
        else:
            st0, C0, sc0, st1, C1, sc1 = st_in
            affine = _empty((N, Ctot, 2), dtype=_F32, device=dev)
            if spec.norm == "g" and src.t1 is not None and residual is None and sub and id(conv.weight) in sub:
                Cs0, Cs1 = sub[id(conv.weight)]
                split = (Cs0, _empty((N, Cs0, 2), dtype=_F32, device=dev),
                         _empty((N, Cs1, 2), dtype=_F32, device=dev) if any(src.plus) else None)
            mean_rstd = self._norm_finalize(spec.norm, gn, st0, C0, sc0, st1, C1, sc1, N, G, float(D * H * W), affine, dev, split)
        b16 = src.t0.dtype == torch.bfloat16
        if b16:
            assert self.act_bf16 and src.t1 is None and not post and self._bf16_layer(Ctot, Cout) and act == ACT_RELU, \
                "bf16 activation storage reached a layer outside its envelope"
        y = y_out if (y_out is not None and not post) else _empty((N, D, H, W, Cout), dtype=src.t0.dtype if b16 else _F32, device=dev)
        call = _ConvCall(dev, conv, src, affine, y, N, D, H, W, Ctot, Cout, relu, bool(want_stats and self.fused_stats), pool, conv_res,
                         sub, b16, *(split[1:] if split is not None else (None, None)))
        family = self._fwd_family(call, residual)
        small = family == "small"
        dmod = getattr(sc, "dropout", None) if spec.drop == "d" else (getattr(sc, "dropout2d", None) if spec.drop == "D" else None)
        if record_only and y_out is not None and not post and not (dmod is not None and dmod.training and dmod.p > 0.0):
            if tape is not None:
                nw = gn.weight if gn is not None else None
                tape.convs.append(
                    ConvRec(name, src, affine, mean_rstd, y, nw, conv.weight, G,
                            self._pindex[id(gn.weight)] if gn is not None else -1,
                            self._pindex[id(gn.bias)] if gn is not None else self._pindex[id(conv.bias)],
                            self._pindex[id(conv.weight)], small,
                            sub.get(id(conv.weight)) if (sub and src.t1 is not None and residual is None) else None,
                            not post, None, spec.norm, bn_training, None, call.affine_lo, call.affine_hi)
                )
            return y, None
        ystats = getattr(self, self._FWD_KERNELS[family])(call)
        post_rec = None
        if post:
            if inner in (ACT_LEAKY, ACT_ELU):
                nat.call("u3d_act_fwd", dev.index, _stream(dev), _p(y), y.numel(), inner, islope, _p(y))
            z, zst = y, ystats
            aff2 = _empty((N, Cout, 2), dtype=_F32, device=dev)
            if spec.norm is None:
                nat.call("u3d_bias_table", dev.index, _stream(dev), _p(conv.bias.detach()), N, Cout, _p(aff2))
            else:
                if zst is None and (spec.norm == "g" or bn_training):
                    zst = self._stats_of(VSrc(z), None, None, pool, dev)[0]
                mean_rstd = self._norm_finalize(spec.norm, gn, zst, Cout, 1.0, None, 0, 0.0, N, G, float(D * H * W), aff2, dev)
            y = y_out if y_out is not None else _empty_like(z)
            nat.call("u3d_affine_add_act_fwd", dev.index, _stream(dev), _p(z), _p(aff2), _p(residual), N, D * H * W, Cout, act,
                     slope, _p(y))
            post_rec, ystats = (z, aff2, inner, islope), None
        elif act in (ACT_LEAKY, ACT_ELU):
            nat.call("u3d_act_fwd", dev.index, _stream(dev), _p(y), y.numel(), act, slope, _p(y))
            ystats = None
        drop_rec = None
        if dmod is not None and dmod.training and dmod.p > 0.0:
            if spec.drop == "d":
                m = F.dropout(torch.ones((N, Cout, D, H, W), dtype=_F32, device=dev), dmod.p, True)
                if Cout == 1:
                    mask = m.view(N, D, H, W, 1)
                else:
                    mask = _empty((N, D, H, W, Cout), dtype=_F32, device=dev)
                    nat.call("u3d_ncdhw_to_ndhwc", dev.index, _stream(dev), _p(m), _p(mask), N, Cout, D * H * W)
                nat.call("u3d_mul", dev.index, _stream(dev), _p(y), _p(mask), y.numel(), _p(y))
                drop_rec = ("d", mask)
            else:
                m = torch.feature_dropout(torch.ones((N, Cout, 1, 1, 1), dtype=_F32, device=dev), dmod.p, True).view(N, Cout)
                table = torch.stack((m, torch.zeros_like(m)), dim=-1).contiguous()
                nat.call("u3d_affine_act_fwd", dev.index, _stream(dev), _p(y), _p(table), N, D * H * W, Cout, ACT_NONE, 0.0, _p(y))
                drop_rec = ("D", table)
            ystats = None
        if tape is not None:
            nw = gn.weight if gn is not None else None
            tape.convs.append(
                ConvRec(name, src, affine, mean_rstd, y, nw, conv.weight, G,
                        self._pindex[id(gn.weight)] if gn is not None else -1,
                        self._pindex[id(gn.bias)] if gn is not None else self._pindex[id(conv.bias)],
                        self._pindex[id(conv.weight)], small,
                        sub.get(id(conv.weight)) if (sub and src.t1 is not None and residual is None) else None,
                        not post, post_rec, spec.norm, bn_training, drop_rec, call.affine_lo, call.affine_hi)
            )
        return y, ystats

    _WGRAD_KERNELS = {
        "bf16": "_wgrad_bf16",
        "subpixel": "_wgrad_subpixel",
        "fp32_side": "_wgrad_fp32_side",
        "fp32": "_wgrad_fp32",
    }
    _DGRAD_KERNELS = {
        "subpixel": "_dgrad_subpixel",
        "f32s": "_dgrad_f32s",
        "bf16": "_dgrad_bf16",
        "fp32": "_dgrad_fp32",
    }

    def _wgrad_family(self, c: "_BwdCall") -> str:
        if c.bf16 and c.Cout % 32 == 0:
            return "bf16"
        if c.rec.sub is not None:
            return "subpixel"
        if self.overlap_small_wgrad and c.N * c.D * c.H * c.W <= c.cx.SIDE_MAX_VOXELS and self.debug is None:
            return "fp32_side"
        return "fp32"

    def _dgrad_family(self, c: "_BwdCall") -> str:
        if c.rec.sub is not None:
            return "subpixel"
        if c.src.t1 is None and not c.rec.small and self._split_dgrad(c.src.C, c.Cout):
            return "f32s"
        return "bf16" if c.bf16 else "fp32"

    def _wgrad_bf16(self, c: "_BwdCall"):
        cx, dev, src, rec = c.cx, c.cx.dev, c.src, c.rec
        need = nat.get_lib().u3d_wgrad_bf16_workspace_floats(c.N, c.D, c.H, c.W, src.C, c.Cout)
        ws = cx.ensure_ws(need)
        dw = cx.gview(rec.idx_w)
        job = c.job
        if job is not None and nat.get_lib().u3d_conv3d_wgrad_bf16_job_supported(c.N, c.D, c.H, c.W, src.C, c.Cout, 1 if c.b16 else 0, _p(dw),
                                                                                  job.N, job.C0 + job.C1, job.G) != 1:
            job = None
        nat.call("u3d_conv3d_wgrad_bf16" + ("_b16" if c.b16 else "") + "_job", dev.index, _stream(dev), _p(src.t0), _p(rec.affine), _p(c.dz),
                 _p(dw), c.N, c.D, c.H, c.W, src.C, c.Cout, _p(ws), ws.numel(), ctypes.byref(job) if job is not None else None,
                 flops=c.flops)
        if job is not None:
            c.job = None

    def _wgrad_subpixel(self, c: "_BwdCall"):
        cx, dev, src, rec, ws = c.cx, c.cx.dev, c.src, c.rec, c.cx.ws
        C0, C1 = rec.sub
        Ct = src.C
        dwv = cx.gview(rec.idx_w)
        plus = src.plus
        if any(plus):
            win = (ctypes.c_int * 9)(c.D, c.H, c.W, *plus, *plus)
            nat.call("u3d_subpixel_conv_wgrad_win", dev.index, _stream(dev), _p(src.t1), _p(rec.affine.view(-1)[2 * C0:]), Ct * 2,
                     _p(c.dz), _p(dwv[C0 * 27:]), Ct, c.N, src.D1, src.H1, src.W1, C1, c.Cout, _p(ws), ws.numel(), win,
                     flops=128.0 * C1 * c.Cout * c.N * src.D1 * src.H1 * src.W1)
            s_up = src.up_only_struct(rec.affine_hi if rec.affine_hi is not None else rec.affine[:, C0:].contiguous())
            slice_view = dwv.view(c.Cout, Ct, 27)[:, C0:, :]
            for box in slab_boxes((c.D, c.H, c.W), plus, 2):
                tmp = _empty((c.Cout, C1, 27), dtype=_F32, device=dev)
                nat.call("u3d_conv3d_wgrad_box", dev.index, _stream(dev), ctypes.byref(s_up), _p(c.dz), _p(tmp), c.N, c.D, c.H, c.W,
                         c.Cout, _p(ws), ws.numel(), (ctypes.c_int * 6)(*box),
                         flops=54.0 * C1 * c.Cout * c.N * (box[3] - box[0]) * (box[4] - box[1]) * (box[5] - box[2]))
                slice_view += tmp
        else:
            nat.call("u3d_subpixel_conv_wgrad", dev.index, _stream(dev), _p(src.t1), _p(rec.affine.view(-1)[2 * C0:]), Ct * 2,
                     _p(c.dz), _p(dwv[C0 * 27:]), Ct, c.N, src.D1, src.H1, src.W1, C1, c.Cout, _p(ws), ws.numel(),
                     flops=128.0 * C1 * c.Cout * c.N * src.D1 * src.H1 * src.W1)
        a0 = rec.affine_lo if rec.affine_lo is not None else rec.affine[:, :C0].contiguous()
        s0 = VSrc(src.t0).struct(a0)
        nat.call("u3d_conv3d_wgrad_job", dev.index, _stream(dev), ctypes.byref(s0), _p(c.dz), _p(dwv), Ct, c.N, c.D, c.H, c.W,
                 c.Cout, _p(ws), ws.numel(), ctypes.byref(c.job) if c.job is not None else None,
                 flops=54.0 * C0 * c.Cout * c.N * c.D * c.H * c.W)
        c.job = None

    def _wgrad_fp32_side(self, c: "_BwdCall"):
        cx, dev, src, rec = c.cx, c.cx.dev, c.src, c.rec
        s_aff = src.struct(rec.affine)
        need = nat.get_lib().u3d_wgrad_workspace_floats(c.N, c.D, c.H, c.W, src.C, c.Cout)
        side = cx.side_stream(need)
        side.wait_stream(torch.cuda.current_stream(dev))
        with torch.cuda.stream(side):
            nat.call("u3d_conv3d_wgrad", dev.index, _stream(dev), ctypes.byref(s_aff), _p(c.dz), _p(cx.gview(rec.idx_w)), c.N,
                     c.D, c.H, c.W, c.Cout, _p(cx.ws_side), cx.ws_side.numel(), flops=c.flops)
        c.dz.record_stream(side)
        cx.side_used = True

    def _wgrad_fp32(self, c: "_BwdCall"):
        cx, dev, src, rec, ws = c.cx, c.cx.dev, c.src, c.rec, c.cx.ws
        s_aff = src.struct(rec.affine)
        nat.call("u3d_conv3d_wgrad_job", dev.index, _stream(dev), ctypes.byref(s_aff), _p(c.dz), _p(cx.gview(rec.idx_w)), 0, c.N, c.D,
                 c.H, c.W, c.Cout, _p(ws), ws.numel(), ctypes.byref(c.job) if c.job is not None else None, flops=c.flops)
        c.job = None

    def _dgrad_subpixel(self, c: "_BwdCall"):
        cx, dev, src, rec, ws, pool = c.cx, c.cx.dev, c.src, c.rec, c.cx.ws, c.cx.pool
        Nn, Dd, Hh, Ww, Cout = c.N, c.D, c.H, c.W, c.Cout
        C0, C1 = rec.sub
        dg0 = _empty((Nn, Dd, Hh, Ww, C0), dtype=_F32, device=dev)
        dlow = _empty_like(src.t1)
        split0 = self._split_dgrad(C0, Cout)
        plus = src.plus
        gst0 = _take_reps(pool, Nn * C0 * 2, 1 if split0 else c.greps)
        gst1 = _take_reps(pool, Nn * C1 * 2, 1 if any(plus) else c.greps)
        if split0:
            need = nat.get_lib().u3d_conv3d_bf16_workspace_floats(Nn, Dd, Hh, Ww, Cout, C0)
            kws = cx.ensure_ws(need) if need > 0 else None
            nat.call("u3d_conv3d_f32s", dev.index, _stream(dev), _p(c.dz), None, _p(self._packed_f32s(rec.conv_w, 1, dev, C0, 0)),
                     _p(dg0), Nn, Dd, Hh, Ww, Cout, C0, 0, None, _p(src.t0), _p(gst0), None, _p(kws), need,
                     flops=54.0 * C0 * Cout * Nn * Dd * Hh * Ww)
        else:
            s_dz = VSrc(c.dz).struct()
            s_x0 = VSrc(src.t0).struct()
            nat.call("u3d_conv3d_ex_reps", dev.index, _stream(dev), ctypes.byref(s_dz), _p(self._packed_sub(rec, 11, dev)), _p(dg0),
                     Nn, Dd, Hh, Ww, C0, 0, None, ctypes.byref(s_x0), _p(gst0), None, _p(ws), ws.numel(), _reps(gst0),
                     flops=54.0 * C0 * Cout * Nn * Dd * Hh * Ww)
        plus = src.plus
        if any(plus):
            win = (ctypes.c_int * 9)(Dd, Hh, Ww, *plus, *plus)
            nat.call("u3d_subpixel_conv_dgrad_win", dev.index, _stream(dev), _p(c.dz), _p(self._packed_sub(rec, 13, dev)), _p(src.t1),
                     _p(dlow), _p(gst1), Nn, src.D1, src.H1, src.W1, C1, Cout, win,
                     flops=128.0 * C1 * Cout * Nn * src.D1 * src.H1 * src.W1)
            dv = _empty((Nn, Dd, Hh, Ww, C1), dtype=_F32, device=dev)
            s_dz2 = VSrc(c.dz).struct()
            wpd1 = self._packed_sub(rec, 15, dev)
            mask = (ctypes.c_int * 3)(*(2 * e for e in plus))
            for box in slab_boxes((Dd, Hh, Ww), plus, 3):
                nat.call("u3d_conv3d_box", dev.index, _stream(dev), ctypes.byref(s_dz2), _p(wpd1), _p(dv), Nn, Dd, Hh, Ww, C1,
                         (ctypes.c_int * 6)(*box), mask,
                         flops=54.0 * C1 * Cout * Nn * (box[3] - box[0]) * (box[4] - box[1]) * (box[5] - box[2]))
            lz, ly, lx = src.los
            nat.call("u3d_nearest_childsum_add", dev.index, _stream(dev), _p(dv), _p(src.t1), _p(dlow), _p(gst1), Nn, Dd, Hh, Ww,
                     src.D1, src.H1, src.W1, C1, _p(lz), _p(ly), _p(lx), *plus)
            del dv
        else:
            nat.call("u3d_subpixel_conv_dgrad_reps", dev.index, _stream(dev), _p(c.dz), _p(self._packed_sub(rec, 13, dev)), _p(src.t1),
                     _p(dlow), _p(gst1), Nn, src.D1, src.H1, src.W1, C1, Cout, _reps(gst1),
                     flops=128.0 * C1 * Cout * Nn * src.D1 * src.H1 * src.W1)
        return (dg0, dlow), (gst0, gst1)

    def _dgrad_f32s(self, c: "_BwdCall"):
        cx, dev, src, rec = c.cx, c.cx.dev, c.src, c.rec
        dg = _empty((c.N, c.D, c.H, c.W, src.C), dtype=_F32, device=dev)
        gst = cx.pool.take(c.N * src.C * 2)
        need = nat.get_lib().u3d_conv3d_bf16_workspace_floats(c.N, c.D, c.H, c.W, c.Cout, src.C)
        kws = cx.ensure_ws(need) if need > 0 else None
        nat.call("u3d_conv3d_f32s", dev.index, _stream(dev), _p(c.dz), None, _p(self._packed_f32s(rec.conv_w, 1, dev)), _p(dg),
                 c.N, c.D, c.H, c.W, c.Cout, src.C, 0, None, _p(src.t0), _p(gst), None, _p(kws), need, flops=c.flops)
        return dg, gst

    def _dgrad_bf16(self, c: "_BwdCall"):
        cx, dev, src, rec = c.cx, c.cx.dev, c.src, c.rec
        dg = _empty((c.N, c.D, c.H, c.W, src.C), dtype=c.dz.dtype if c.b16 else _F32, device=dev)
        gst = cx.pool.take(c.N * src.C * 2)
        need = nat.get_lib().u3d_conv3d_bf16_workspace_floats(c.N, c.D, c.H, c.W, c.Cout, src.C)
        kws = cx.ensure_ws(need) if need > 0 else None
        nat.call("u3d_conv3d_bf16_ex" + ("_b16" if c.b16 else ""), dev.index, _stream(dev), _p(c.dz), None,
                 _p(self._packed_bf16(rec.conv_w, 1, dev)), _p(dg), c.N, c.D, c.H, c.W, c.Cout, src.C, 0, None, _p(src.t0), _p(gst),
                 None, _p(kws), need, flops=c.flops)
        return dg, gst

    def _dgrad_fp32(self, c: "_BwdCall"):
        cx, dev, src, rec, ws = c.cx, c.cx.dev, c.src, c.rec, c.cx.ws
        wpd = self._packed(rec.conv_w, 1, dev)
        dg = _empty((c.N, c.D, c.H, c.W, src.C), dtype=_F32, device=dev)
        gst = _take_reps(cx.pool, c.N * src.C * 2, c.greps)
        s_dz = VSrc(c.dz).struct()
        s_x = src.struct()
        nat.call("u3d_conv3d_ex_reps", dev.index, _stream(dev), ctypes.byref(s_dz), _p(wpd), _p(dg), c.N, c.D, c.H, c.W, src.C, 0, None,
                 ctypes.byref(s_x), _p(gst), None, _p(ws), ws.numel(), _reps(gst), flops=c.flops)
        return dg, gst

    def _conv_bwd(self, cx, rec: ConvRec, dz_, need_dg=True):
        dev, pool, ws, gview = cx.dev, cx.pool, cx.ws, cx.gview
        src = rec.src
        Nn, Dd, Hh, Ww = src.N, src.D, src.H, src.W
        Cout = rec.y.shape[-1]
        if rec.drop is not None:
            kind, mask = rec.drop
            g = _empty_like(dz_)
            if kind == "d":
                nat.call("u3d_mul", dev.index, _stream(dev), _p(dz_), _p(mask), dz_.numel(), _p(g))
            else:
                nat.call("u3d_affine_act_fwd", dev.index, _stream(dev), _p(dz_), _p(mask), Nn, Dd * Hh * Ww, Cout, ACT_NONE, 0.0, _p(g))
            dz_ = g
        if rec.post is not None:
            z, _, inner, islope = rec.post
            Vz = Dd * Hh * Ww
            gst2 = pool.take(Nn * Cout * 2)
            nat.call("u3d_pair_stats", dev.index, _stream(dev), _p(dz_), _p(z), Nn, Vz, Cout, _p(gst2))
            if rec.norm is None:
                nat.call("u3d_bias_grad", dev.index, _stream(dev), _p(gst2), Nn, Cout, _p(gview(rec.idx_gb)))
            else:
                coef2 = _empty((Nn, 3, Cout), dtype=_F32, device=dev)
                self._norm_bwd_finalize(cx, rec, gst2, Nn, Cout, float(Vz), coef2)
                dz_ = self._plain_apply(cx, dz_, coef2, z, 1 if inner == ACT_RELU else 0)
                if inner in (ACT_LEAKY, ACT_ELU):
                    nat.call("u3d_act_bwd", dev.index, _stream(dev), _p(dz_), _p(z), dz_.numel(), inner, islope, _p(dz_))
        if self.debug is not None:
            self.debug[rec.name + ".dz"] = dz_.clone()
        if rec.small and not need_dg:
            gst = pool.take(Nn * src.C * 2)
            nat.call("u3d_conv3d_small_cin_bwd", dev.index, _stream(dev), _p(src.t0), _p(rec.affine), _p(dz_),
                     _p(rec.conv_w.detach()), _p(gview(rec.idx_w)), _p(gst), Nn, Dd, Hh, Ww, src.C, Cout, _p(ws), ws.numel(),
                     flops=2 * 54.0 * src.C * Cout * Nn * Dd * Hh * Ww)
            if not rec.pre_norm:
                return None, self._identity_coef(Nn, src.C, dev)
            coef = _empty((Nn, 3, src.C), dtype=_F32, device=dev)
            self._norm_bwd_finalize(cx, rec, gst, Nn, src.C, float(Dd * Hh * Ww), coef)
            return None, coef
        bf16 = src.t1 is None and rec.sub is None and not rec.small and self._bf16_layer(src.C, Cout)
        b16 = src.t0.dtype == torch.bfloat16
        assert not b16 or (bf16 and Cout % 64 == 0 and dz_.dtype == torch.bfloat16)
        call = _BwdCall(cx, rec, dz_, src, Nn, Dd, Hh, Ww, Cout, bf16, b16)
        if (self.stat_reps > 1 and rec.pre_norm and rec.norm == "g" and _WGRAD_JOB and self._wgrad_family(call) in ("fp32", "subpixel")
                and nat.get_lib().u3d_conv3d_wgrad_job_supported(Nn, src.C, rec.G) == 1):
            call.greps = self.stat_reps
        dg, gst = getattr(self, self._DGRAD_KERNELS[self._dgrad_family(call)])(call)
        if self.debug is not None and rec.sub is None:
            self.debug[rec.name + ".dg"] = dg.clone()
        coef = None
        if rec.pre_norm:
            coef = _empty((Nn, 3, src.C), dtype=_F32, device=dev)
            call.job = self._norm_bwd_job(cx, rec, gst, Nn, src.C, float(Dd * Hh * Ww), coef)
        had_job = call.job is not None
        getattr(self, self._WGRAD_KERNELS[self._wgrad_family(call)])(call)
        if not rec.pre_norm:
            return dg, self._identity_coef(Nn, src.C, dev)
        if not had_job or call.job is not None:
            self._norm_bwd_finalize(cx, rec, gst, Nn, src.C, float(Dd * Hh * Ww), coef)
        return dg, coef

    def _plain_apply(self, cx, dg, coef, x, relu_mask, add=None):
        dev = cx.dev
        out = _empty_like(x)
        Nn = x.shape[0]
        C = x.shape[-1]
        if x.dtype == torch.bfloat16:
            nat.call("u3d_gn_bwd_apply_b16", dev.index, _stream(dev), _p(dg), C, 0, _p(x), C, _p(coef), C, x.numel() // (Nn * C), Nn,
                     relu_mask, _p(add), _p(out))
            return out
        if add is None:
            nat.call("u3d_gn_bwd_apply", dev.index, _stream(dev), _p(dg), C, 0, _p(x), C, _p(coef), C, x.numel() // (Nn * C), Nn,
                     relu_mask, _p(out))
        else:
            nat.call("u3d_gn_bwd_apply_add", dev.index, _stream(dev), _p(dg), C, 0, _p(x), C, _p(coef), C,
                     x.numel() // (Nn * C), Nn, relu_mask, _p(add), _p(out))
        return out

    def _wgrad_workspace(self, tape, dev):
        return _empty(max(self._wgrad_workspace_floats(tape.convs), 4), dtype=_F32, device=dev)

    def _layer_ws_floats(self, N, D, H, W, Cin, Cout, sub=None, small=False, virtual=False):
        lib = nat.get_lib()
        if small:
            return lib.u3d_small_cin_bwd_workspace_floats(N, D, H, W, Cin, Cout)
        if sub is not None:
            boxes = slab_boxes((D, H, W), (D % 2, H % 2, W % 2), 2)
            return max([lib.u3d_wgrad_workspace_floats(N, D, H, W, sub[0], Cout),
                        lib.u3d_subpixel_wgrad_workspace_floats(N, D // 2, H // 2, W // 2, sub[1], Cout),
                        lib.u3d_conv3d_workspace_floats(N, D, H, W, Cout, sub[0])] +
                       [lib.u3d_wgrad_workspace_floats(N, b[3] - b[0], b[4] - b[1], b[5] - b[2], sub[1], Cout) for b in boxes])
        if not virtual and self._bf16_layer(Cin, Cout):
            need = lib.u3d_conv3d_bf16_workspace_floats(N, D, H, W, Cout, Cin)
            wg = lib.u3d_wgrad_bf16_workspace_floats(N, D, H, W, Cin, Cout)
            return max(need, wg)
        return max(lib.u3d_wgrad_workspace_floats(N, D, H, W, Cin, Cout), lib.u3d_conv3d_workspace_floats(N, D, H, W, Cout, Cin))

    def _wgrad_workspace_floats(self, convs):
        need = 0
        for r in convs:
            need = max(need, self._layer_ws_floats(r.src.N, r.src.D, r.src.H, r.src.W, r.src.C, r.y.shape[-1], r.sub, r.small,
                                                   r.src.t1 is not None))
        return int(need)
```

pytorch-3dunet_amd/pytorch3dunet_amd/_engine_unet.py:

```python
from __future__ import annotations

import copy
import ctypes
import dataclasses
import os
import threading
from dataclasses import dataclass, field
from typing import List, Optional

import torch
import torch.nn.functional as F

from . import _native as nat
from ._native import U3DSrc

from ._engine_base import *
from ._engine_conv import ConvLayers, _reps, _take_reps
from ._engine_weights import WeightImages



class UNet3DEngine(WeightImages, ConvLayers):

    def __init__(self, model):
        self.model = model
        self._pack_cache: dict = {}
        self.grad_sync = None
        self.debug = None
        self.fused_stats = True
        self.stat_reps = max(1, min(64, int(os.environ.get("U3D_STAT_REPS", "8"))))
        self.small_cin = True
        self.overlap_small_wgrad = True
        self.subpixel = os.environ.get("U3D_SUBPIXEL", "1") != "0"
        self.subpixel_plus = os.environ.get("U3D_SUBPIXEL_PLUS", "1") != "0"
        self.bf16 = bool(getattr(model, "compute_bf16", False))
        self.split = bool(getattr(model, "compute_split", False)) and not self.bf16
        self.checkpoint_encoders = bool(getattr(model, "checkpoint_encoders", False))
        self.checkpoint_levels = getattr(model, "checkpoint_levels", None)
        self.lean_tape = False
        self.act_bf16 = False
        self._sub_pairs: dict = {}
        self._lock = threading.RLock()
        self.hip_graph = bool(getattr(model, "hip_graph", False))
        self._graph_steps: dict = {}
        self._graph_off_reason = None
        self._placed = None
        self._salt = 0
        self._const: dict = {}
        spec = parse_order(getattr(model, "layer_order", "gcr")) or (False, ACT_RELU, 0.0)
        self.post_norm, self.act, self.slope = spec
        self.mask = 1 if self.act == ACT_RELU else 0
        self.params = module_params(model)
        self._pids = [id(p) for p in self.params]
        self._first_param_owner, self._first_param_name = next(
            ((mod, name) for mod in model.modules() for name, p in mod._parameters.items() if p is self.params[0]), (None, None))
        self._pindex = _PIndex({id(p): i for i, p in enumerate(self.params)})
        self._build_layer_table(model)
        self._virtual_w = self._virtual_weights()
        n_enc = sum(p.numel() for p in module_params(model.encoders))
        self.n_enc_params = n_enc
        self.enc_level_offs = [0]
        for enc in model.encoders:
            self.enc_level_offs.append(self.enc_level_offs[-1] + sum(p.numel() for p in module_params(enc)))
        assert self.enc_level_offs[-1] == n_enc
        self.n_params = sum(p.numel() for p in self.params)
        offs, o = [], 0
        for p in self.params:
            offs.append(o)
            o += p.numel()
        self.poffs = offs

    MIN_BUCKET_FLOATS = int(os.environ.get("U3D_MIN_BUCKET_MB", "1")) * (1 << 20) // 4

    def _sync_encoder_level(self, cx, flat, level: int, pending_hi: int) -> int:
        lo = self.enc_level_offs[level]
        if level > 0 and pending_hi - lo < self.MIN_BUCKET_FLOATS:
            return pending_hi
        if pending_hi > lo:
            cx.join()
            self.grad_sync.launch(flat[lo:pending_hi])
        return lo

    def _virtual_weights(self):
        return {id(c1.conv.weight) for c1, _ in self.dec if not self._cat_bf16(c1)}

    def _cat_bf16(self, c1) -> bool:
        return bool(self.bf16) and layer_spec(c1.order).pre and self._bf16_layer(c1.conv.in_channels, c1.conv.out_channels) and \
            os.environ.get("U3D_BF16_CAT", "1") != "0"

    def _build_layer_table(self, model):
        self.enc = []
        for enc in model.encoders:
            bm = enc.basic_module
            self.enc.append((enc.pooling is not None, bm.SingleConv1, bm.SingleConv2))
        self.dec = []
        self.dec_up = []
        for dec in model.decoders:
            bm = dec.basic_module
            self.dec.append((bm.SingleConv1, bm.SingleConv2))
            self.dec_up.append(getattr(getattr(dec.upsampling, "upsample", None), "conv_transposed", None))
        self.dec_interp = [getattr(dec.upsampling, "mode", None) if getattr(dec.upsampling, "mode", None) in ("trilinear", "area")
                           else None for dec in model.decoders]

    def forward(self, x: torch.Tensor, save: bool):
        m = self.model
        dev = x.device
        N, Cin, D, H, W = x.shape
        x = x.contiguous()
        if Cin == 1:
            x0 = x.view(N, D, H, W, 1)
        else:
            x0 = _empty((N, D, H, W, Cin), dtype=_F32, device=dev)
            nat.call("u3d_ncdhw_to_ndhwc", dev.index, _stream(dev), _p(x), _p(x0), N, Cin, D * H * W)
        tape = Tape() if save else None
        if tape is not None:
            tape.x0 = x0
            tape.dims = (N, Cin, D, H, W)
        sub = self._subpixel_layers((D, H, W))
        self._repack_all(dev, (0, 1) if save else (0,), sub)
        tot = 0
        R = self.stat_reps
        for _, c1, c2 in self.enc:
            tot += N * (4 * c1.conv.in_channels + (3 + R) * (c1.conv.out_channels + c2.conv.out_channels)) * 2
        for c1, c2 in self.dec:
            tot += N * (4 * c1.conv.in_channels + (3 + R) * (c1.conv.out_channels + c2.conv.out_channels)) * 2
        fcm = self.model.final_conv
        btot = 0
        if save:
            btot = R * (fcm.out_channels * fcm.in_channels + fcm.out_channels)
            for _, c1, c2 in self.enc:
                btot += R * N * (c1.conv.in_channels + c2.conv.in_channels) * 2
            for c1, c2 in self.dec:
                btot += R * N * (c1.conv.in_channels + c2.conv.in_channels) * 2
        pool = _StatPool(dev, tot + btot)
        if tape is not None:
            tape.bwd_pool = pool.carve(btot)

        feats = []
        cur, cur_st = x0, None
        for i, (has_pool, c1, c2) in enumerate(self.enc):
            if has_pool:
                Np, Dp, Hp, Wp, Cp = cur.shape
                pooled = _empty((Np, Dp // 2, Hp // 2, Wp // 2, Cp), dtype=_F32, device=dev)
                argmax = _empty(pooled.shape, dtype=torch.uint8, device=dev)
                pst = None if self.post_norm else _take_reps(pool, Np * Cp * 2, self.stat_reps)
                nat.call("u3d_maxpool2_fwd", dev.index, _stream(dev), _p(cur), Np, Dp, Hp, Wp, Cp, _p(pooled), _p(argmax), None)
                if pst is not None:
                    s_p = VSrc(pooled).struct()
                    nat.call("u3d_chan_stats_reps", dev.index, _stream(dev), ctypes.byref(s_p), Np, Dp // 2, Hp // 2, Wp // 2, _p(pst),
                             _reps(pst))
                if tape is not None:
                    tape.pools.append((pooled, argmax, cur))
                cur, cur_st = pooled, pst
            src = VSrc(cur)
            stats_of = (lambda *a: None) if self.post_norm else self._stats_of
            y1, s1 = self._single_conv_fwd(c1, f"enc{i}.c1", src, stats_of(src, cur_st, None, pool, dev), pool, tape)
            src2 = VSrc(y1)
            y2, s2 = self._single_conv_fwd(c2, f"enc{i}.c2", src2, stats_of(src2, s1, None, pool, dev), pool, tape)
            feats.append((y2, s2))
            cur, cur_st = y2, s2

        skips = feats[:-1][::-1]
        for j, ((c1, c2), (sk, sk_st)) in enumerate(zip(self.dec, skips)):
            ct = self.dec_up[j]
            if ct is not None:
                Nl, D1, H1, W1, Cl = cur.shape
                Cs = ct.out_channels
                t = _empty((Nl, 2 * D1 - 1, 2 * H1 - 1, 2 * W1 - 1, Cs), dtype=_F32, device=dev)
                if self.subpixel and Cl % 4 == 0 and Cs % 4 == 0:
                    nat.call("u3d_convtr3d_fwd_subpixel", dev.index, _stream(dev), _p(cur), _p(self._packed_convtr(ct.weight, 2, dev)),
                             _p(t), Nl, D1, H1, W1, Cl, Cs, flops=2.0 * 27 * Cl * Cs * Nl * D1 * H1 * W1)
                else:
                    nat.call("u3d_convtr3d_fwd", dev.index, _stream(dev), _p(cur), _p(ct.weight.detach()), _p(t), Nl, D1, H1, W1, Cl,
                             Cs, _p(self._packed_convtr(ct.weight, 0, dev)), flops=2.0 * 27 * Cl * Cs * Nl * D1 * H1 * W1)
                if tape is not None:
                    tape.ups.append(UpRec(cur, ct.weight, None, tuple(t.shape[1:4])))
                cur, cur_st = t, None
            elif self.dec_interp[j] is not None:
                Nl, D1, H1, W1, Cl = cur.shape
                _, Ds, Hs, Ws, _ = sk.shape
                tabs = [_resample_tables(dev, self.dec_interp[j], a, b) for a, b in ((D1, Ds), (H1, Hs), (W1, Ws))]
                up = _empty((Nl, Ds, Hs, Ws, Cl), dtype=_F32, device=dev)
                nat.call("u3d_resample2_fwd", dev.index, _stream(dev), _p(cur), _p(tabs[0][0]), _p(tabs[1][0]), _p(tabs[2][0]),
                         _p(tabs[0][1]), _p(tabs[1][1]), _p(tabs[2][1]), Nl, D1, H1, W1, Ds, Hs, Ws, Cl, _p(up))
                if tape is not None:
                    tape.ups.append(UpRec(cur, None, tabs, (Ds, Hs, Ws)))
                cur, cur_st = up, None
            src = VSrc(sk, cur)
            st_in = stats_of(src, sk_st, cur_st, pool, dev)
            if self._cat_bf16(c1):
                cat = _empty((src.N, src.D, src.H, src.W, src.C), dtype=_F32, device=dev)
                nat.call("u3d_nearest_cat_fwd", dev.index, _stream(dev), _p(sk), _p(cur), _p(src.maps[0]), _p(src.maps[1]), _p(src.maps[2]),
                         src.N, src.D, src.H, src.W, src.D1, src.H1, src.W1, src.C0, src.C1, _p(cat))
                if tape is not None:
                    tape.cats[j] = src
                y1, s1 = self._single_conv_fwd(c1, f"dec{j}.c1", VSrc(cat), st_in, pool, tape)
                del cat
            else:
                y1, s1 = self._single_conv_fwd(c1, f"dec{j}.c1", src, st_in, pool, tape, sub=sub)
            src2 = VSrc(y1)
            y2, s2 = self._single_conv_fwd(c2, f"dec{j}.c2", src2, stats_of(src2, s1, None, pool, dev), pool, tape)
            cur, cur_st = y2, s2

        fc = m.final_conv
        Co, Cf = fc.out_channels, fc.in_channels
        V = D * H * W
        logits = _empty((N, Co, D, H, W), dtype=_F32, device=dev)
        act = 0
        probs = None
        if m.final_activation is not None:
            act = 1 if isinstance(m.final_activation, torch.nn.Sigmoid) else 2
            probs = _empty_like(logits)
        nat.call("u3d_conv1x1_head_fwd", dev.index, _stream(dev), _p(cur), _p(fc.weight.detach()), _p(fc.bias.detach()), N, V,
                 Cf, Co, act, _p(logits), _p(probs))
        if tape is not None:
            tape.head_x = cur
            if self.debug is not None:
                self.debug["tape"] = tape
        return logits, probs, tape

    def backward(self, tape: Tape, dlogits: torch.Tensor, need_input_grad: bool):
        m = self.model
        dev = dlogits.device
        N, Cin, D, H, W = tape.dims
        V = D * H * W
        dlogits = dlogits.contiguous()
        flat = _empty(self.n_params, dtype=_F32, device=dev)

        def gview(idx):
            p = self.params[idx]
            return flat[self.poffs[idx] : self.poffs[idx] + p.numel()]

        fc = m.final_conv
        Co, Cf = fc.out_channels, fc.in_channels
        tot = self.stat_reps * (Co * Cf + Co) + sum(self.stat_reps * N * r.src.C * 2 for r in tape.convs)
        pool = getattr(tape, "bwd_pool", None)
        tape.bwd_pool = None
        if pool is None or pool.buf.numel() < tot or pool.buf.device != dev or torch.cuda.is_current_stream_capturing():
            pool = _StatPool(dev, tot)
        ws = self._wgrad_workspace(tape, dev)

        hreps = self.stat_reps
        hacc = pool.take(hreps * (Co * Cf + Co))
        dz = _empty_like(tape.head_x)
        nat.call("u3d_conv1x1_head_bwd_reps", dev.index, _stream(dev), _p(dlogits), _p(tape.head_x), _p(fc.weight.detach()), N, V,
                 Cf, Co, self.mask, _p(dz), _p(hacc), hreps)
        self._unact(dev, dz, tape.head_x)
        iw, ib = self._pindex[id(fc.weight)], self._pindex[id(fc.bias)]
        assert self.poffs[ib] == self.poffs[iw] + Co * Cf
        nat.call("u3d_cvt_f64_f32_sum", dev.index, _stream(dev), _p(hacc), _p(gview(iw)), Co * Cf + Co, hreps)

        n_levels = len(self.enc)
        n_dec = len(self.dec)
        mk = self.mask
        skip_grad = {}

        cx = _BwdCtx(dev, pool, ws, flat, self)

        def conv_bwd(rec: ConvRec, dz_, need_dg=True):
            return self._conv_bwd(cx, rec, dz_, need_dg)

        def plain_apply(dg, coef, x, relu_mask):
            return self._plain_apply(cx, dg, coef, x, relu_mask)

        recs = tape.convs
        enc_recs = [(recs[2 * i], recs[2 * i + 1]) for i in range(n_levels)]
        dec_recs = [(recs[2 * n_levels + 2 * j], recs[2 * n_levels + 2 * j + 1]) for j in range(n_dec)]

        for j in range(n_dec - 1, -1, -1):
            r1, r2 = dec_recs[j]
            dg2, coef2 = conv_bwd(r2, dz)
            dz1 = plain_apply(dg2, coef2, r2.src.t0, mk)
            self._unact(dev, dz1, r2.src.t0)
            del dg2
            dg1, coef1 = conv_bwd(r1, dz1)
            src = tape.cats.get(j, r1.src)
            C0, C1, Ct = src.C0, src.C1, src.C
            lvl = n_levels - 2 - j
            dzl = _empty_like(src.t1)
            if r1.sub is not None:
                dg0, dlow = dg1
                skip_grad[lvl] = (dg0, C0, coef1, Ct)
                if any(src.plus):
                    nat.call("u3d_gn_bwd_apply_children", dev.index, _stream(dev), _p(dlow), _p(src.t1), _p(coef1), Ct, C0, src.N, src.D1,
                             src.H1, src.W1, C1, *src.plus, mk, _p(dzl))
                else:
                    coef_up = cx.coef_hi if cx.coef_hi is not None else coef1[:, :, C0:] * self._up_scale(dev)
                    nat.call("u3d_gn_bwd_apply", dev.index, _stream(dev), _p(dlow), C1, 0, _p(src.t1), C1, _p(coef_up), C1,
                             src.D1 * src.H1 * src.W1, src.N, mk, _p(dzl))
                del dg0, dlow
            else:
                skip_grad[lvl] = (dg1, Ct, coef1, Ct)
                lz, ly, lx = src.los
                nat.call("u3d_gn_bwd_apply_up", dev.index, _stream(dev), _p(dg1), Ct, C0, _p(src.t1), C1, _p(coef1), Ct, src.N,
                         src.D, src.H, src.W, src.D1, src.H1, src.W1, _p(lz), _p(ly), _p(lx),
                         0 if (self.dec_up[j] is not None or self.dec_interp[j] is not None) else mk, _p(dzl))
            del dg1
            if self.dec_up[j] is not None:
                up = tape.ups[j]
                xl = up.x_low
                Nl, D1, H1, W1, Cl = xl.shape
                Cs = up.weight.shape[1]
                acc = pool.take(up.weight.numel())
                dxl = _empty_like(xl)
                nat.call("u3d_convtr3d_bwd", dev.index, _stream(dev), _p(dzl), _p(xl), _p(up.weight.detach()), Nl, D1, H1, W1, Cl, Cs,
                         mk, _p(dxl), _p(acc), _p(self._packed_convtr(up.weight, 1, dev)), flops=4.0 * 27 * Cl * Cs * Nl * D1 * H1 * W1)
                nat.call("u3d_cvt_f64_f32", dev.index, _stream(dev), _p(acc), _p(gview(self._pindex[id(up.weight)])),
                         up.weight.numel())
                self._unact(dev, dxl, xl)
                dzl = dxl
            elif self.dec_interp[j] is not None:
                up = tape.ups[j]
                xl = up.x_low
                Nl, D1, H1, W1, Cl = xl.shape
                Ds, Hs, Ws = up.tdims
                tz, ty, tx = up.los
                dxl = _empty_like(xl)
                nat.call("u3d_resample2_bwd", dev.index, _stream(dev), _p(dzl), _p(tz[2]), _p(ty[2]), _p(tx[2]), _p(tz[0]), _p(ty[0]),
                         _p(tx[0]), _p(tz[1]), _p(ty[1]), _p(tx[1]), Nl, D1, H1, W1, Ds, Hs, Ws, Cl, _p(dxl))
                if self.act != ACT_NONE:
                    nat.call("u3d_act_bwd", dev.index, _stream(dev), _p(dxl), _p(xl), dxl.numel(), self.act, self.slope, _p(dxl))
                dzl = dxl
            else:
                self._unact(dev, dzl, src.t1)
            dz = dzl

        if self.grad_sync is not None:
            cx.join()
            self.grad_sync.launch(flat[self.n_enc_params :])

        dx0 = None
        pending_hi = self.n_enc_params
        for i in range(n_levels - 1, -1, -1):
            r1, r2 = enc_recs[i]
            dg2, coef2 = conv_bwd(r2, dz)
            dz1 = plain_apply(dg2, coef2, r2.src.t0, mk)
            self._unact(dev, dz1, r2.src.t0)
            del dg2
            dg1, coef1 = conv_bwd(r1, dz1, need_dg=(i > 0 or need_input_grad))
            if self.grad_sync is not None:
                pending_hi = self._sync_encoder_level(cx, flat, i, pending_hi)
            if i > 0:
                pooled, argmax, e_in = tape.pools[i - 1]
                Ne, De, He, We, Ce = e_in.shape
                out = _empty_like(e_in)
                sk = skip_grad.pop(i - 1, None)
                if sk is None:
                    nat.call("u3d_maxpool2_bwd_merge", dev.index, _stream(dev), _p(dg1), _p(pooled), _p(argmax), _p(coef1), None,
                             _p(e_in), Ne, De, He, We, Ce, mk, _p(out))
                else:
                    sdg, sCdg, scoef, sCt = sk
                    nat.call("u3d_maxpool2_bwd_merge_gn", dev.index, _stream(dev), _p(dg1), _p(pooled), _p(argmax), _p(coef1),
                             _p(sdg), sCdg, _p(scoef), sCt, _p(e_in), Ne, De, He, We, Ce, mk, _p(out))
                    del sk, sdg, scoef
                self._unact(dev, out, e_in)
                dz = out
            elif need_input_grad:
                dx0 = plain_apply(dg1, coef1, tape.x0, 0)
            del dg1

        cx.join()
        if self.grad_sync is not None:
            self.grad_sync.finish()

        dx = None
        if dx0 is not None:
            if Cin == 1:
                dx = dx0.view(N, 1, D, H, W)
            else:
                dx = _empty((N, Cin, D, H, W), dtype=_F32, device=dev)
                nat.call("u3d_ndhwc_to_ncdhw", dev.index, _stream(dev), _p(dx0), _p(dx), N, Cin, V)
        return flat, dx
```

pytorch-3dunet_amd/pytorch3dunet_amd/_native.py:

```python
from __future__ import annotations

import ctypes
import os
import threading
from ctypes import POINTER, c_char_p, c_double, c_float, c_int, c_int32, c_int64, c_size_t, c_void_p

_HERE = os.path.dirname(os.path.abspath(__file__))
LIB_PATH = os.environ.get("U3D_LIB_PATH") or os.path.join(_HERE, "lib", "libu3d_hip.so")

U3D_OK = 0


class U3DSrc(ctypes.Structure):

    _fields_ = [
        ("p0", c_void_p),
        ("p1", c_void_p),
        ("zmap", c_void_p),
        ("ymap", c_void_p),
        ("xmap", c_void_p),
        ("affine", c_void_p),
        ("C0", c_int32),
        ("C1", c_int32),
        ("D1", c_int32),
        ("H1", c_int32),
        ("W1", c_int32),
    ]


class U3DAdamDesc(ctypes.Structure):

    _fields_ = [("p", c_void_p), ("g", c_void_p), ("m", c_void_p), ("v", c_void_p), ("first", c_int64), ("numel", c_int64)]


class U3DGnBwdJob(ctypes.Structure):

    _fields_ = [("gstats_lo", c_void_p), ("gstats_hi", c_void_p), ("mean_rstd", c_void_p), ("gamma", c_void_p), ("dgamma", c_void_p),
                ("dbeta", c_void_p), ("coef", c_void_p), ("coef_hi", c_void_p), ("count", ctypes.c_double), ("C0", c_int32),
                ("C1", c_int32), ("N", c_int32), ("G", c_int32), ("hi_scale", ctypes.c_float), ("reps_lo", c_int32), ("reps_hi", c_int32), ("reserved", c_int32)]


class U3DPackDesc(ctypes.Structure):

    _fields_ = [("w", c_void_p), ("packed", c_void_p), ("first", c_int64), ("Cout", c_int32), ("Cin", c_int32),
                ("mode", c_int32), ("cin_stride", c_int32)]


_PROTOS = {
    "u3d_version": (c_int, []),
    "u3d_debug_stream_pass": (c_int, [c_int, c_void_p, c_void_p, c_int64, c_int, c_int, c_double]),
    "u3d_debug_mfma_f32_rate": (c_int, [c_int, c_void_p, c_void_p, c_int, c_int, POINTER(c_double)]),
    "u3d_last_error": (c_char_p, []),
    "u3d_check_device": (c_int, [c_int]),
    "u3d_set_tuning": (c_int, [c_int, c_int]),
    "u3d_set_profile_buffer": (c_int, [c_void_p, c_size_t]),
    "u3d_packed_weight_floats": (c_size_t, [c_int, c_int, c_int]),
    "u3d_pack_weights": (c_int, [c_int, c_void_p, c_void_p, c_int, c_int, c_int, c_void_p]),
    "u3d_pack_weights_batch": (c_int, [c_int, c_void_p, c_void_p, c_int, c_int64]),
    "u3d_pack_weights_cells_blocks": (c_int64, [c_void_p, c_int, c_int, c_int, c_int]),
    "u3d_pack_weights_batch_cells": (c_int, [c_int, c_void_p, c_void_p, c_int, c_int64]),
    "u3d_conv3d": (
        c_int,
        [c_int, c_void_p, POINTER(U3DSrc), c_void_p, c_void_p, c_int, c_int, c_int, c_int, c_int, c_int, c_void_p,
         POINTER(U3DSrc), c_void_p],
    ),
    "u3d_wgrad_workspace_floats": (c_size_t, [c_int, c_int, c_int, c_int, c_int, c_int]),
    "u3d_conv3d_variant": (c_int, [c_int, c_int, c_int, c_int, c_int, c_int, c_int, c_int]),
    "u3d_conv3d_wgrad_variant": (c_int, [c_int, c_int, c_int, c_int, c_int, c_int, c_int]),
    "u3d_conv3d_wgrad": (
        c_int,
        [c_int, c_void_p, POINTER(U3DSrc), c_void_p, c_void_p, c_int, c_int, c_int, c_int, c_int, c_void_p, c_size_t],
    ),
    "u3d_conv3d_small_cin_fwd": (
        c_int,
        [c_int, c_void_p, c_void_p, c_void_p, c_void_p, c_void_p, c_int, c_int, c_int, c_int, c_int, c_int, c_int, c_void_p],
    ),
    "u3d_conv3d_small_cin_fwd_reps": (
        c_int,
        [c_int, c_void_p, c_void_p, c_void_p, c_void_p, c_void_p, c_int, c_int, c_int, c_int, c_int, c_int, c_int, c_void_p, c_int],
    ),
    "u3d_small_cin_bwd_workspace_floats": (c_size_t, [c_int, c_int, c_int, c_int, c_int, c_int]),
    "u3d_conv3d_small_cin_bwd": (
        c_int,
        [c_int, c_void_p, c_void_p, c_void_p, c_void_p, c_void_p, c_void_p, c_void_p, c_int, c_int, c_int, c_int, c_int,
         c_int, c_void_p, c_size_t],
    ),
    "u3d_conv3d_naive": (
        c_int,
        [c_int, c_void_p, POINTER(U3DSrc), c_void_p, c_void_p, c_int, c_int, c_int, c_int, c_int, c_int, c_int, c_int],
    ),
    "u3d_chan_stats": (c_int, [c_int, c_void_p, POINTER(U3DSrc), c_int, c_int, c_int, c_int, c_void_p]),
    "u3d_chan_stats_reps": (c_int, [c_int, c_void_p, POINTER(U3DSrc), c_int, c_int, c_int, c_int, c_void_p, c_int]),
    "u3d_gn_finalize": (
        c_int,
        [c_int, c_void_p, c_void_p, c_int, c_double, c_void_p, c_int, c_double, c_int, c_int, c_double, c_void_p,
         c_void_p, c_float, c_void_p, c_void_p],
    ),
    "u3d_gn_bwd_finalize": (
        c_int,
        [c_int, c_void_p, c_void_p, c_void_p, c_void_p, c_int, c_int, c_int, c_double, c_void_p, c_void_p, c_void_p],
    ),
    "u3d_gn_finalize_split": (
        c_int,
        [c_int, c_void_p, c_void_p, c_int, c_double, c_void_p, c_int, c_double, c_int, c_int, c_double, c_void_p,
         c_void_p, c_float, c_void_p, c_void_p, c_int, c_void_p, c_void_p],
    ),
    "u3d_gn_bwd_finalize_split_supported": (c_int, [c_int, c_int, c_int]),
    "u3d_chan_stats_children": (c_int, [c_int, c_void_p, c_void_p, c_int, c_int, c_int, c_int, c_int, c_int, c_int, c_int, c_void_p]),
    "u3d_adam_step": (c_int, [c_int, c_void_p, c_void_p, c_int, c_int64, c_double, c_double, c_double, c_double, c_double, c_int64]),
    "u3d_gn_bwd_finalize_split": (
        c_int,
        [c_int, c_void_p, c_void_p, c_int, c_void_p, c_int, c_void_p, c_void_p, c_int, c_int, c_double, c_void_p, c_void_p,
         c_void_p, c_float, c_void_p],
    ),
    "u3d_gn_bwd_apply": (
        c_int,
        [c_int, c_void_p, c_void_p, c_int, c_int, c_void_p, c_int, c_void_p, c_int, c_int64, c_int, c_int, c_void_p],
    ),
    "u3d_gn_bwd_apply_up": (
        c_int,
        [c_int, c_void_p, c_void_p, c_int, c_int, c_void_p, c_int, c_void_p, c_int, c_int, c_int, c_int, c_int, c_int,
         c_int, c_int, c_void_p, c_void_p, c_void_p, c_int, c_void_p],
    ),
    "u3d_maxpool2_fwd": (c_int, [c_int, c_void_p, c_void_p, c_int, c_int, c_int, c_int, c_int, c_void_p, c_void_p, c_void_p]),
    "u3d_maxpool2_bwd_merge": (
        c_int,
        [c_int, c_void_p, c_void_p, c_void_p, c_void_p, c_void_p, c_void_p, c_void_p, c_int, c_int, c_int, c_int, c_int,
         c_int, c_void_p],
    ),
    "u3d_maxpool2_bwd_merge_gn": (
        c_int,
        [c_int, c_void_p, c_void_p, c_void_p, c_void_p, c_void_p, c_void_p, c_int, c_void_p, c_int, c_void_p, c_int, c_int,
         c_int, c_int, c_int, c_int, c_void_p],
    ),
    "u3d_conv1x1_head_fwd": (
        c_int,
        [c_int, c_void_p, c_void_p, c_void_p, c_void_p, c_int, c_int64, c_int, c_int, c_int, c_void_p, c_void_p],
    ),
    "u3d_conv1x1_head_bwd": (
        c_int,
        [c_int, c_void_p, c_void_p, c_void_p, c_void_p, c_int, c_int64, c_int, c_int, c_int, c_void_p, c_void_p],
    ),
    "u3d_conv1x1_head_bwd_reps": (
        c_int,
        [c_int, c_void_p, c_void_p, c_void_p, c_void_p, c_int, c_int64, c_int, c_int, c_int, c_void_p, c_void_p, c_int],
    ),
    "u3d_conv3d_wgrad_strided": (
        c_int,
        [c_int, c_void_p, POINTER(U3DSrc), c_void_p, c_void_p, c_int, c_int, c_int, c_int, c_int, c_int, c_void_p, c_size_t],
    ),
    "u3d_conv3d_ex_reps": (
        c_int,
        [c_int, c_void_p, POINTER(U3DSrc), c_void_p, c_void_p, c_int, c_int, c_int, c_int, c_int, c_int, c_void_p, POINTER(U3DSrc),
         c_void_p, c_void_p, c_void_p, c_int64, c_int],
    ),
    "u3d_gn_finalize_reps": (
        c_int,
        [c_int, c_void_p, c_void_p, c_int, c_double, c_int, c_void_p, c_int, c_double, c_int, c_int, c_int, c_double, c_void_p, c_void_p,
         c_float, c_void_p, c_void_p, c_int, c_void_p, c_void_p],
    ),
    "u3d_conv3d_wgrad_job_supported": (c_int, [c_int, c_int, c_int]),
    "u3d_conv3d_wgrad_job": (
        c_int,
        [c_int, c_void_p, POINTER(U3DSrc), c_void_p, c_void_p, c_int, c_int, c_int, c_int, c_int, c_int, c_void_p, c_size_t,
         POINTER(U3DGnBwdJob)],
    ),
    "u3d_subpixel_wgrad_workspace_floats": (c_int64, [c_int, c_int, c_int, c_int, c_int, c_int]),
    "u3d_subpixel_conv_wgrad": (
        c_int,
        [c_int, c_void_p, c_void_p, c_void_p, c_int64, c_void_p, c_void_p, c_int, c_int, c_int, c_int, c_int, c_int, c_int,
         c_void_p, c_int64],
    ),
    "u3d_convtr3d_subpixel_packed_floats": (c_int64, [c_int, c_int]),
    "u3d_pack_convtr3d_subpixel": (c_int, [c_int, c_void_p, c_void_p, c_int, c_int, c_void_p]),
    "u3d_convtr3d_fwd_subpixel": (
        c_int, [c_int, c_void_p, c_void_p, c_void_p, c_void_p, c_int, c_int, c_int, c_int, c_int, c_int],
    ),
    "u3d_subpixel_packed_floats": (c_int64, [c_int, c_int]),
    "u3d_subpixel_dgrad_packed_floats": (c_int64, [c_int, c_int]),
    "u3d_pack_subpixel_dgrad_weights": (c_int, [c_int, c_void_p, c_void_p, c_int, c_int, c_int, c_int, c_void_p]),
    "u3d_subpixel_conv_dgrad": (
        c_int,
        [c_int, c_void_p, c_void_p, c_void_p, c_void_p, c_void_p, c_void_p, c_int, c_int, c_int, c_int, c_int, c_int],
    ),
    "u3d_subpixel_conv_dgrad_reps": (
        c_int,
        [c_int, c_void_p, c_void_p, c_void_p, c_void_p, c_void_p, c_void_p, c_int, c_int, c_int, c_int, c_int, c_int, c_int],
    ),
    "u3d_pack_subpixel_weights": (c_int, [c_int, c_void_p, c_void_p, c_int, c_int, c_int, c_int, c_void_p]),
    "u3d_subpixel_conv_fwd_win": (c_int, [c_int, c_void_p, c_void_p, c_void_p, c_int64, c_void_p, c_void_p, c_int, c_int, c_int, c_int,
                                          c_int, c_int, POINTER(c_int)]),
    "u3d_subpixel_conv_dgrad_win": (c_int, [c_int, c_void_p, c_void_p, c_void_p, c_void_p, c_void_p, c_void_p, c_int, c_int, c_int, c_int,
                                            c_int, c_int, POINTER(c_int)]),
    "u3d_subpixel_conv_wgrad_win": (c_int, [c_int, c_void_p, c_void_p, c_void_p, c_int64, c_void_p, c_void_p, c_int, c_int, c_int, c_int,
                                            c_int, c_int, c_int, c_void_p, c_int64, POINTER(c_int)]),
    "u3d_conv3d_box": (c_int, [c_int, c_void_p, POINTER(U3DSrc), c_void_p, c_void_p, c_int, c_int, c_int, c_int, c_int, POINTER(c_int),
                               POINTER(c_int)]),
    "u3d_conv3d_wgrad_box": (c_int, [c_int, c_void_p, POINTER(U3DSrc), c_void_p, c_void_p, c_int, c_int, c_int, c_int, c_int, c_void_p,
                                     c_size_t, POINTER(c_int)]),
    "u3d_gn_bwd_apply_children": (c_int, [c_int, c_void_p, c_void_p, c_void_p, c_void_p, c_int, c_int, c_int, c_int, c_int, c_int, c_int,
                                          c_int, c_int, c_int, c_int, c_void_p]),
    "u3d_nearest_childsum_add": (c_int, [c_int, c_void_p, c_void_p, c_void_p, c_void_p, c_void_p, c_int, c_int, c_int, c_int, c_int, c_int,
                                         c_int, c_int, c_void_p, c_void_p, c_void_p, c_int, c_int, c_int]),
    "u3d_subpixel_fwd_workspace_floats": (c_int64, [c_int, c_int, c_int, c_int, c_int, c_int]),
    "u3d_subpixel_conv_fwd": (
        c_int,
        [c_int, c_void_p, c_void_p, c_void_p, c_int64, c_void_p, c_void_p, c_int, c_int, c_int, c_int, c_int, c_int,
         c_void_p, c_int64],
    ),
    "u3d_conv3d_workspace_floats": (c_int64, [c_int, c_int, c_int, c_int, c_int, c_int]),
    "u3d_conv3d_ex": (
        c_int,
        [c_int, c_void_p, POINTER(U3DSrc), c_void_p, c_void_p, c_int, c_int, c_int, c_int, c_int, c_int, c_void_p,
         POINTER(U3DSrc), c_void_p, c_void_p, c_void_p, c_int64],
    ),
    "u3d_conv3d_residual": (
        c_int,
        [c_int, c_void_p, POINTER(U3DSrc), c_void_p, c_void_p, c_int, c_int, c_int, c_int, c_int, c_int, c_void_p, c_void_p],
    ),
    "u3d_gn_bwd_apply_add": (
        c_int,
        [c_int, c_void_p, c_void_p, c_int, c_int, c_void_p, c_int, c_void_p, c_int, c_int64, c_int, c_int, c_void_p, c_void_p],
    ),
    "u3d_conv1x1_fwd": (c_int, [c_int, c_void_p, c_void_p, c_void_p, c_void_p, c_void_p, c_int, c_int64, c_int, c_int, c_void_p]),
    "u3d_conv1x1_bwd": (c_int, [c_int, c_void_p, c_void_p, c_void_p, c_void_p, c_int, c_int64, c_int, c_int, c_void_p, c_void_p]),
    "u3d_pack_convtr_weights": (c_int, [c_int, c_void_p, c_void_p, c_int, c_int, c_int, c_void_p]),
    "u3d_convtr3d_fwd": (c_int, [c_int, c_void_p, c_void_p, c_void_p, c_void_p, c_int, c_int, c_int, c_int, c_int, c_int, c_void_p]),
    "u3d_convtr3d_bwd": (
        c_int,
        [c_int, c_void_p, c_void_p, c_void_p, c_void_p, c_int, c_int, c_int, c_int, c_int, c_int, c_int, c_void_p, c_void_p,
         c_void_p],
    ),
    "u3d_nearest_add_fwd": (
        c_int,
        [c_int, c_void_p, c_void_p, c_void_p, c_void_p, c_void_p, c_void_p, c_int, c_int, c_int, c_int, c_int, c_int, c_int,
         c_int, c_void_p, c_void_p],
    ),
    "u3d_nearest_sum_bwd": (
        c_int,
        [c_int, c_void_p, c_void_p, c_void_p, c_void_p, c_void_p, c_int, c_int, c_int, c_int, c_int, c_int, c_int, c_int,
         c_void_p],
    ),
    "u3d_se_gate_fwd": (
        c_int,
        [c_int, c_void_p, c_void_p, c_double, c_void_p, c_void_p, c_void_p, c_void_p, c_int, c_int, c_int, c_void_p, c_void_p,
         c_void_p],
    ),
    "u3d_se_apply_fwd": (
        c_int, [c_int, c_void_p, c_void_p, c_void_p, c_void_p, c_void_p, c_int, c_int64, c_int, c_int, c_void_p, c_void_p]),
    "u3d_se_bwd_reduce": (
        c_int,
        [c_int, c_void_p, c_void_p, c_void_p, c_void_p, c_void_p, c_void_p, c_int, c_int64, c_int, c_int, c_void_p, c_void_p,
         c_void_p],
    ),
    "u3d_se_gate_bwd": (
        c_int,
        [c_int, c_void_p, c_void_p, c_void_p, c_void_p, c_void_p, c_void_p, c_void_p, c_int, c_int, c_int, c_double, c_void_p,
         c_void_p, c_void_p, c_void_p, c_void_p, c_void_p, c_void_p],
    ),
    "u3d_se_bwd_apply": (
        c_int,
        [c_int, c_void_p, c_void_p, c_void_p, c_void_p, c_void_p, c_void_p, c_void_p, c_void_p, c_int, c_int64, c_int, c_int,
         c_int, c_void_p],
    ),
    "u3d_se_apply_fwd_b16": (
        c_int, [c_int, c_void_p, c_void_p, c_void_p, c_void_p, c_void_p, c_int, c_int64, c_int, c_int, c_void_p, c_void_p]),
    "u3d_se_bwd_reduce_b16": (
        c_int,
        [c_int, c_void_p, c_void_p, c_void_p, c_void_p, c_void_p, c_void_p, c_int, c_int64, c_int, c_int, c_void_p, c_void_p,
         c_void_p],
    ),
    "u3d_se_bwd_apply_b16": (
        c_int,
        [c_int, c_void_p, c_void_p, c_void_p, c_void_p, c_void_p, c_void_p, c_void_p, c_void_p, c_int, c_int64, c_int, c_int,
         c_int, c_void_p],
    ),
    "u3d_bce_dice_scratch_doubles": (c_int64, [c_int, c_int, c_int64]),
    "u3d_bce_dice_fwd": (
        c_int,
        [c_int, c_void_p, c_void_p, c_void_p, c_void_p, c_int, c_int, c_int64, c_float, c_float, c_float, c_void_p, c_void_p,
         c_void_p],
    ),
    "u3d_bce_dice_bwd": (c_int, [c_int, c_void_p, c_void_p, c_void_p, c_void_p, c_void_p, c_int, c_int, c_int64, c_void_p]),
    "u3d_conv3d_bf16_supported": (c_int, [c_int, c_int]),
    "u3d_packed_weight_bf16_elems": (c_int64, [c_int, c_int, c_int]),
    "u3d_packed_weight_f32s_elems": (c_int64, [c_int, c_int, c_int]),
    "u3d_pack_weights_f32s": (c_int, [c_int, c_void_p, c_void_p, c_int, c_int, c_int, c_int, c_int, c_void_p]),
    "u3d_conv3d_f32s": (
        c_int,
        [c_int, c_void_p, c_void_p, c_void_p, c_void_p, c_void_p] + [c_int] * 7 + [c_void_p, c_void_p, c_void_p, c_void_p, c_void_p,
                                                                                 c_int64],
    ),
    "u3d_pack_weights_bf16": (c_int, [c_int, c_void_p, c_void_p, c_int, c_int, c_int, c_void_p]),
    "u3d_conv3d_bf16_ex_b16": (c_int, [c_int, c_void_p, c_void_p, c_void_p, c_void_p, c_void_p, c_int, c_int, c_int, c_int, c_int,
                                       c_int, c_int, c_void_p, c_void_p, c_void_p, c_void_p, c_void_p, c_int64]),
    "u3d_conv3d_wgrad_bf16_b16": (c_int, [c_int, c_void_p, c_void_p, c_void_p, c_void_p, c_void_p, c_int, c_int, c_int, c_int, c_int,
                                          c_int, c_void_p, c_int64]),
    "u3d_convtr3d_fwd_t8_b16": (c_int, [c_int, c_void_p, c_void_p, c_void_p, c_void_p, c_int, c_int, c_int, c_int, c_int, c_int]),
    "u3d_convtr3d_dgrad_t8_b16": (c_int, [c_int, c_void_p, c_void_p, c_void_p, c_void_p, c_void_p, c_int, c_int, c_int, c_int, c_int,
                                          c_int]),
    "u3d_convtr3d_wgrad_t8_b16": (c_int, [c_int, c_void_p, c_void_p, c_void_p, c_void_p, c_int, c_int, c_int, c_int, c_int, c_int,
                                          c_void_p, c_int64]),
    "u3d_conv1x1_fwd_b16": (c_int, [c_int, c_void_p, c_void_p, c_int, c_void_p, c_void_p, c_void_p, c_int, c_int64, c_int, c_int,
                                    c_void_p]),
    "u3d_conv1x1_mfma_b16_supported": (c_int, [c_int, c_int]),
    "u3d_conv1x1_fwd_mfma_b16": (c_int, [c_int, c_void_p, c_void_p, c_void_p, c_void_p, c_void_p, c_int, c_int64, c_int, c_int,
                                         c_void_p]),
    "u3d_conv1x1_bwd_mfma_b16_workspace_floats": (c_int64, [c_int, c_int, c_int, c_int, c_int, c_int]),
    "u3d_conv1x1_bwd_mfma_b16": (c_int, [c_int, c_void_p, c_void_p, c_void_p, c_void_p, c_int, c_int, c_int, c_int, c_int, c_int,
                                         c_void_p, c_void_p, c_void_p, c_void_p, c_int64]),
    "u3d_conv1x1_bwd_b16": (c_int, [c_int, c_void_p, c_void_p, c_void_p, c_int, c_void_p, c_int, c_int64, c_int, c_int, c_void_p,
                                    c_void_p]),
    "u3d_maxpool2_fwd_b16": (c_int, [c_int, c_void_p, c_void_p, c_int, c_int, c_int, c_int, c_int, c_void_p, c_void_p]),
    "u3d_maxpool2_bwd_merge_b16": (c_int, [c_int, c_void_p, c_void_p, c_void_p, c_void_p, c_void_p, c_void_p, c_void_p, c_int, c_int,
# ... 184 lines not shown
```

Baseline: 121.0.

## Fuse GroupNorm-backward apply into conv wgrad staging via virtual dz source

The weight-gradient kernel now stages dz by reading the raw upstream gradient and the saved activation, then applying the GroupNorm-backward affine and ReLU mask in registers. Chunk-0 blocks write the materialized dz so the dgrad pass can still read it. This removes the separate plain_apply pass that produced dz before the wgrad. The wgrad main launch is split from its reduce launch so the reduce can run later with the GN job. Costs are extra loads of x and the coefficients in the wgrad prefetch, more register pressure, and a separate workspace.

```diff
diff --git a/include/u3d.h b/include/u3d.h
--- a/include/u3d.h
+++ b/include/u3d.h
@@ -112,6 +112,22 @@
 int u3d_conv3d_wgrad_job(int device, u3d_stream_t stream, const u3d_src_t* src, const float* dz, float* dw, int dw_cin_stride,
                          int N, int D, int H, int W, int Cout, float* workspace, size_t workspace_floats,
                          const u3d_gn_bwd_job_t* job);
+
+typedef struct u3d_dz_src {
+    int32_t kind;
+    int32_t relu_mask;
+    const float* dg;
+    const float* x;
+    const float* coef;
+    int32_t Cdg, coff, Ctot, reserved;
+} u3d_dz_src_t;
+#define U3D_DZ_PLAIN 0
+#define U3D_DZ_GN_APPLY 1
+int u3d_conv3d_wgrad_vdz_supported(int N, int D, int H, int W, int Cin, int Cout, int src_kind);
+int u3d_conv3d_wgrad_vdz(int device, u3d_stream_t stream, const u3d_src_t* src, const u3d_dz_src_t* dzs, float* dz_out, int N, int D,
+                         int H, int W, int Cout, float* workspace, size_t workspace_floats);
+int u3d_conv3d_wgrad_reduce_job(int device, u3d_stream_t stream, const u3d_src_t* src, float* dw, int dw_cin_stride, int N, int D,
+                                int H, int W, int Cout, const float* workspace, size_t workspace_floats, const u3d_gn_bwd_job_t* job);
 
 long long u3d_subpixel_wgrad_workspace_floats(int N, int D1, int H1, int W1, int C1, int Cout);
 int u3d_subpixel_conv_wgrad(int device, u3d_stream_t stream, const float* low, const float* affine,
diff --git a/pytorch-3dunet_amd/csrc/u3d_conv.hip b/pytorch-3dunet_amd/csrc/u3d_conv.hip
--- a/pytorch-3dunet_amd/csrc/u3d_conv.hip
+++ b/pytorch-3dunet_amd/csrc/u3d_conv.hip
@@ -1141,11 +1141,15 @@
     int tz, ty, tx, ntiles, tps;
     int vec, dzvec;
     int bz0, by0, bx0, bz1, by1, bx1;
+    u3d_dz_src_t dzs;
+    float* dz_out;
 };
 
-template <bool VEC, bool REG = false, bool PAIR = false>
+template <bool VEC, bool REG = false, bool PAIR = false, int DZK = U3D_DZ_PLAIN>
 __global__ __launch_bounds__(512, 2) void conv3d_wgrad_kernel(const WgradParams p) {
     using namespace wg;
+    static_assert(DZK == U3D_DZ_PLAIN || (VEC && REG), "virtual dz: constant-offset staging only");
+    constexpr bool VDZ = DZK == U3D_DZ_GN_APPLY;
     constexpr int NA = PAIR ? 4 : 7;
     extern __shared__ __attribute__((aligned(16))) float lds[];
     int* zmapl = reinterpret_cast<int*>(lds + 2 * BUF_FLOATS);
@@ -1183,6 +1187,10 @@
     const float* gbase = !cok ? p.src.p0 : (from0 ? p.src.p0 + cq : p.src.p1 + (cq - p.src.C0));
     const int Cs = (from0 || !cok) ? p.src.C0 : p.src.C1;
     const float* dzbase = p.dz + (dcok ? co : 0);
+    const float* dgbase = VDZ ? p.dzs.dg + p.dzs.coff + (dcok ? co : 0) : nullptr;
+    const float* xdbase = VDZ ? p.dzs.x + (dcok ? co : 0) : nullptr;
+    float* dzout = VDZ ? p.dz_out + (dcok ? co : 0) : nullptr;
+    const bool dz_writer = VDZ && chunk == 0;
 
     constexpr int NPFC = NIT_G + NIT_DZ;
     int rel[NPFC], loff[NPFC];
@@ -1318,6 +1326,7 @@
         if constexpr (REG) {
             ok = ((c.inv >> k) & 1u) == 0;
             if (k < NIT_G) return *reinterpret_cast<const f32x4*>(gbase + (size_t)(ok ? c.base + rel[k] : 0) * Cs);
+            if constexpr (VDZ) return *reinterpret_cast<const f32x4*>(dgbase + (size_t)(ok ? c.dzb + rel[k] : 0) * p.dzs.Cdg);
             return *reinterpret_cast<const f32x4*>(dzbase + (size_t)(ok ? c.dzb + rel[k] : 0) * p.Cout);
         }
         if (k < NIT_G) {
@@ -1326,13 +1335,33 @@
         }
         dz_item(c, k - NIT_G, ok, idx);
         return *reinterpret_cast<const f32x4*>(dzbase + (size_t)idx * p.Cout);
+    };
+    f32x4 vx[NIT_DZ];
+    f32x4 dcp = {0.f, 0.f, 0.f, 0.f}, dcq = dcp, dcr = dcp;
+    auto pf_load_x = [&](const TileC& c, int k) {
+        const bool ok = ((c.inv >> k) & 1u) == 0;
+        return *reinterpret_cast<const f32x4*>(xdbase + (size_t)(ok ? c.dzb + rel[k] : 0) * p.Cout);
+    };
+    auto load_dzcoef = [&](int n) {
+        const float* cp = p.dzs.coef + (size_t)n * 3 * p.dzs.Ctot + p.dzs.coff + (dcok ? co : 0);
+        dcp = *reinterpret_cast<const f32x4*>(cp);
+        dcq = *reinterpret_cast<const f32x4*>(cp + p.dzs.Ctot);
+        dcr = *reinterpret_cast<const f32x4*>(cp + 2 * (size_t)p.dzs.Ctot);
     };
     auto pf_store = [&](float* buf, const TileC& c, int k, f32x4 raw, const f32x4& ga, const f32x4& gb) {
         bool ok;
         int idx, off;
         if constexpr (REG) {
             ok = ((c.inv >> k) & 1u) == 0;
-            f32x4 val = k < NIT_G ? raw * ga + gb : raw;
+            f32x4 val = raw;
+            if (k < NIT_G) {
+                val = raw * ga + gb;
+            } else if constexpr (VDZ) {
+                const f32x4 xv = vx[k - NIT_G];
+                val = u3d_gn_bwd_quad(dcp, raw, dcq, xv, dcr);
+                if (p.dzs.relu_mask) val = u3d_relu_mask_quad(val, xv);
+                if (dz_writer && ok) *reinterpret_cast<f32x4*>(dzout + (size_t)(c.dzb + rel[k]) * p.Cout) = val;
+            }
 #pragma unroll
             for (int e = 0; e < 4; ++e) val[e] = ok ? val[e] : 0.f;
             *reinterpret_cast<f32x4*>(&buf[loff[k]]) = val;
@@ -1394,9 +1423,14 @@
         if constexpr (VEC) {
             f32x4 ga, gb;
             load_affine(c.n, ga, gb);
+            if constexpr (VDZ) load_dzcoef(c.n);
             f32x4 v[NPF];
 #pragma unroll
             for (int k = 0; k < NPF; ++k) v[k] = pf_load(c, k);
+            if constexpr (VDZ) {
+#pragma unroll
+                for (int k = NIT_G; k < NPF; ++k) vx[k - NIT_G] = pf_load_x(c, k);
+            }
 #pragma unroll
             for (int k = 0; k < NPF; ++k) pf_store(lds, c, k, v[k], ga, gb);
         } else {
@@ -1427,6 +1461,7 @@
         if constexpr (VEC) {
             if (cn.n != n_aff) {
                 load_affine(cn.n, gan, gbn);
+                if constexpr (VDZ) load_dzcoef(cn.n);
                 n_aff = cn.n;
             }
         }
@@ -1440,6 +1475,9 @@
         for (int g = 0; g < 32; ++g) {
             if constexpr (VEC) {
                 if (g % 2 == 0 && g / 2 < NPF) v[g / 2] = pf_load(cn, g / 2);
+                if constexpr (VDZ) {
+                    if (g % 2 == 0 && g / 2 >= NIT_G && g / 2 < NPF) vx[g / 2 - NIT_G] = pf_load_x(cn, g / 2);
+                }
                 if (g >= ST0 && g - ST0 < NPF) pf_store(nbuf, cn, g - ST0, v[g - ST0], gan, gbn);
             }
             if (g + 1 < 32) {
@@ -2344,6 +2382,10 @@
                                 hipFuncAttributeMaxDynamicSharedMemorySize, (wg::LDS_FLOATS + wg::MAX_MAP_INTS) * sizeof(float)));
     U3D_HIP(hipFuncSetAttribute(reinterpret_cast<const void*>(conv3d_wgrad_kernel<true>),
                                 hipFuncAttributeMaxDynamicSharedMemorySize, (wg::LDS_FLOATS + wg::MAX_MAP_INTS) * sizeof(float)));
+    U3D_HIP(hipFuncSetAttribute(reinterpret_cast<const void*>(conv3d_wgrad_kernel<true, true, false, U3D_DZ_GN_APPLY>),
+                                hipFuncAttributeMaxDynamicSharedMemorySize, (wg::LDS_FLOATS + wg::MAX_MAP_INTS) * sizeof(float)));
+    U3D_HIP(hipFuncSetAttribute(reinterpret_cast<const void*>(conv3d_wgrad_kernel<true, true, true, U3D_DZ_GN_APPLY>),
+                                hipFuncAttributeMaxDynamicSharedMemorySize, (wg::LDS_FLOATS + wg::MAX_MAP_INTS) * sizeof(float)));
     U3D_HIP(hipFuncSetAttribute(reinterpret_cast<const void*>(conv3d_wgrad_kernel<false>),
                                 hipFuncAttributeMaxDynamicSharedMemorySize, (wg::LDS_FLOATS + wg::MAX_MAP_INTS) * sizeof(float)));
     if (device >= 0 && device < 64) done[device] = true;
@@ -2378,30 +2420,31 @@
     return (N > 0 && C > 0 && G > 0 && C % G == 0 && wgrad_job_lds_bytes(N, C, G) + 1024 <= 64 * 1024) ? 1 : 0;
 }
 
+static int check_wgrad_job(const u3d_gn_bwd_job_t* job, const char* what) {
+    if (!job) return 0;
+    U3D_REQUIRE(job->gstats_lo && job->mean_rstd && job->gamma && job->dgamma && job->dbeta && job->coef && job->C0 > 0 &&
+                    job->C1 >= 0 && (job->C1 == 0) == (job->gstats_hi == nullptr) && (job->coef_hi == nullptr || job->C1 > 0) &&
+                    job->reps_lo >= 0 && job->reps_lo <= 64 && job->reps_hi >= 0 && job->reps_hi <= 64,
+                "%s: bad job", what);
+    U3D_REQUIRE(u3d_conv3d_wgrad_job_supported(job->N, job->C0 + job->C1, job->G) == 1,
+                "%s: the reduction of %d x %d channels in %d groups does not fit one block's LDS", what, job->N, job->C0 + job->C1, job->G);
+    return 0;
+}
+
 extern "C" int u3d_conv3d_wgrad_job(int device, u3d_stream_t stream, const u3d_src_t* src, const float* dz, float* dw,
                                     int dw_cin_stride, int N, int D, int H, int W, int Cout, float* workspace,
                                     size_t workspace_floats, const u3d_gn_bwd_job_t* job) {
     U3D_REQUIRE(src && (dw_cin_stride == 0 || dw_cin_stride >= src->C0 + src->C1), "u3d_conv3d_wgrad_job: dw_cin_stride < channels of src");
-    if (job) {
-        U3D_REQUIRE(job->gstats_lo && job->mean_rstd && job->gamma && job->dgamma && job->dbeta && job->coef && job->C0 > 0 &&
-                        job->C1 >= 0 && (job->C1 == 0) == (job->gstats_hi == nullptr) && (job->coef_hi == nullptr || job->C1 > 0) &&
-                        job->reps_lo >= 0 && job->reps_lo <= 64 && job->reps_hi >= 0 && job->reps_hi <= 64,
-                    "u3d_conv3d_wgrad_job: bad job");
-        U3D_REQUIRE(u3d_conv3d_wgrad_job_supported(job->N, job->C0 + job->C1, job->G) == 1,
-                    "u3d_conv3d_wgrad_job: the reduction of %d x %d channels in %d groups does not fit one block's LDS", job->N,
-                    job->C0 + job->C1, job->G);
-    }
+    if (int e = check_wgrad_job(job, "u3d_conv3d_wgrad_job")) return e;
     return conv3d_wgrad_impl(device, stream, src, dz, dw, dw_cin_stride, N, D, H, W, Cout, workspace, workspace_floats, nullptr, job);
 }
 
-static int conv3d_wgrad_impl(int device, u3d_stream_t stream, const u3d_src_t* src, const float* dz, float* dw, int cstride,
-                             int N, int D, int H, int W, int Cout, float* workspace, size_t workspace_floats, const int* box,
-                             const u3d_gn_bwd_job_t* job) {
-    U3D_ENTER(device);
+static int wgrad_main_launch(u3d_stream_t stream, const u3d_src_t* src, const float* dz, int N, int D, int H, int W, int Cout,
+                             float* workspace, size_t workspace_floats, const int* box, const u3d_dz_src_t* dzs, float* dz_out,
+                             WgradParams& p, int device) {
     if (int e = check_src(src, "u3d_conv3d_wgrad")) return e;
-    U3D_REQUIRE(dz && dw && workspace && N > 0 && D > 0 && H > 0 && W > 0 && Cout > 0, "u3d_conv3d_wgrad: bad argument");
+    U3D_REQUIRE(dz && workspace && N > 0 && D > 0 && H > 0 && W > 0 && Cout > 0, "u3d_conv3d_wgrad: bad argument");
     U3D_REQUIRE((long long)N * D * H * W < (1ll << 31), "u3d_conv3d_wgrad: N*D*H*W must be < 2^31");
-    WgradParams p;
     const int Cin = src->C0 + src->C1;
     p.bz0 = p.by0 = p.bx0 = 0, p.bz1 = D, p.by1 = H, p.bx1 = W;
     if (box) {
@@ -2415,6 +2458,8 @@
         return u3d_set_err(U3D_EWORKSPACE, "u3d_conv3d_wgrad: workspace %zu < %zu floats", workspace_floats, need);
     p.src = *src;
     p.dz = dz;
+    p.dzs = dzs ? *dzs : u3d_dz_src_t{};
+    p.dz_out = dz_out;
     p.partial = workspace;
     p.N = N, p.D = D, p.H = H, p.W = W, p.Cout = Cout;
     p.vec = src_vec_ok(src) ? 1 : 0;
@@ -2425,7 +2470,15 @@
     const size_t shmem = (wg::LDS_FLOATS + (size_t)(D + H + W)) * sizeof(float);
     const bool reg = !box && (g_u3d_tune[3] != 2 || (D % wg::TZ == 0 && H % wg::TY == 0 && W % wg::TX == 0)) &&
                      (src->C1 == 0 || (D == 2 * src->D1 && H == 2 * src->H1 && W == 2 * src->W1));
-    if (p.vec && p.dzvec && reg && Cin <= 16)
+    if (dzs && dzs->kind == U3D_DZ_GN_APPLY) {
+        U3D_REQUIRE(p.vec && p.dzvec && reg, "u3d_conv3d_wgrad_vdz: shape / alignment outside the constant-offset staging");
+        if (Cin <= 16)
+            hipLaunchKernelGGL((conv3d_wgrad_kernel<true, true, true, U3D_DZ_GN_APPLY>), dim3(nblk), dim3(wg::NTHR), shmem,
+                               (hipStream_t)stream, p);
+        else
+            hipLaunchKernelGGL((conv3d_wgrad_kernel<true, true, false, U3D_DZ_GN_APPLY>), dim3(nblk), dim3(wg::NTHR), shmem,
+                               (hipStream_t)stream, p);
+    } else if (p.vec && p.dzvec && reg && Cin <= 16)
         hipLaunchKernelGGL((conv3d_wgrad_kernel<true, true, true>), dim3(nblk), dim3(wg::NTHR), shmem, (hipStream_t)stream, p);
     else if (p.vec && p.dzvec && reg)
         hipLaunchKernelGGL((conv3d_wgrad_kernel<true, true>), dim3(nblk), dim3(wg::NTHR), shmem, (hipStream_t)stream, p);
@@ -2434,7 +2487,12 @@
     else
         hipLaunchKernelGGL(conv3d_wgrad_kernel<false>, dim3(nblk), dim3(wg::NTHR), shmem, (hipStream_t)stream, p);
     U3D_LAUNCH_CHECK();
-    const long long total = (long long)Cin * 27 * Cout;
+    return 0;
+}
+
+static int wgrad_reduce_launch(u3d_stream_t stream, const WgradParams& p, int Cin, float* dw, int cstride, const float* workspace,
+                               const u3d_gn_bwd_job_t* job) {
+    const long long total = (long long)Cin * 27 * p.Cout;
     const bool one_group = p.S <= 16 && g_u3d_tune[23] != 1;
     const int rblocks = (int)((total + (one_group ? 255 : 63)) / (one_group ? 256 : 64));
     u3d_gn_bwd_job_t jb = {};
@@ -2448,12 +2506,59 @@
     }
     if (one_group)
         hipLaunchKernelGGL(wgrad_reduce_kernel<1>, dim3(rblocks + (job ? 1 : 0)), dim3(256), job_lds, (hipStream_t)stream, workspace, dw, p.S,
-                           p.nchunks, p.nkb, Cin, Cout, cstride > 0 ? cstride : Cin, job ? 1 : 0, jb);
+                           p.nchunks, p.nkb, Cin, p.Cout, cstride > 0 ? cstride : Cin, job ? 1 : 0, jb);
     else
         hipLaunchKernelGGL(wgrad_reduce_kernel<4>, dim3(rblocks + (job ? 1 : 0)), dim3(256), job_lds, (hipStream_t)stream, workspace, dw, p.S,
-                           p.nchunks, p.nkb, Cin, Cout, cstride > 0 ? cstride : Cin, job ? 1 : 0, jb);
+                           p.nchunks, p.nkb, Cin, p.Cout, cstride > 0 ? cstride : Cin, job ? 1 : 0, jb);
     U3D_LAUNCH_CHECK();
     return 0;
+}
+
+static int conv3d_wgrad_impl(int device, u3d_stream_t stream, const u3d_src_t* src, const float* dz, float* dw, int cstride,
+                             int N, int D, int H, int W, int Cout, float* workspace, size_t workspace_floats, const int* box,
+                             const u3d_gn_bwd_job_t* job) {
+    U3D_ENTER(device);
+    U3D_REQUIRE(dw, "u3d_conv3d_wgrad: bad argument");
+    WgradParams p;
+    if (int e = wgrad_main_launch(stream, src, dz, N, D, H, W, Cout, workspace, workspace_floats, box, nullptr, nullptr, p, device)) return e;
+    return wgrad_reduce_launch(stream, p, src->C0 + src->C1, dw, cstride, workspace, job);
+}
+
+extern "C" int u3d_conv3d_wgrad_vdz_supported(int N, int D, int H, int W, int Cin, int Cout, int src_kind) {
+    const int v = u3d_conv3d_wgrad_variant(N, D, H, W, Cin, Cout, src_kind);
+    return v > 0 && (v & 3) != 0 ? 1 : 0;
+}
+
+extern "C" int u3d_conv3d_wgrad_vdz(int device, u3d_stream_t stream, const u3d_src_t* src, const u3d_dz_src_t* dzs, float* dz_out, int N,
+                                    int D, int H, int W, int Cout, float* workspace, size_t workspace_floats) {
+    U3D_ENTER(device);
+    U3D_REQUIRE(dzs && dz_out && (dzs->kind == U3D_DZ_PLAIN || dzs->kind == U3D_DZ_GN_APPLY), "u3d_conv3d_wgrad_vdz: bad dz source");
+    if (dzs->kind == U3D_DZ_GN_APPLY) {
+        U3D_REQUIRE(dzs->dg && dzs->x && dzs->coef && dzs->Cdg > 0 && dzs->coff >= 0 && dzs->coff + Cout <= dzs->Cdg &&
+                        dzs->Ctot >= dzs->coff + Cout && dzs->Cdg % 4 == 0 && dzs->coff % 4 == 0 && dzs->Ctot % 4 == 0 &&
+                        (((uintptr_t)dzs->dg | (uintptr_t)dzs->x | (uintptr_t)dzs->coef) & 15) == 0,
+                    "u3d_conv3d_wgrad_vdz: bad gn_apply source");
+    }
+    WgradParams p;
+    return wgrad_main_launch(stream, src, dz_out, N, D, H, W, Cout, workspace, workspace_floats, nullptr,
+                             dzs->kind == U3D_DZ_PLAIN ? nullptr : dzs, dz_out, p, device);
+}
+
+extern "C" int u3d_conv3d_wgrad_reduce_job(int device, u3d_stream_t stream, const u3d_src_t* src, float* dw, int dw_cin_stride, int N,
+                                           int D, int H, int W, int Cout, const float* workspace, size_t workspace_floats,
+                                           const u3d_gn_bwd_job_t* job) {
+    U3D_ENTER(device);
+    U3D_REQUIRE(src && dw && workspace && N > 0 && D > 0 && H > 0 && W > 0 && Cout > 0 &&
+                    (dw_cin_stride == 0 || dw_cin_stride >= src->C0 + src->C1),
+                "u3d_conv3d_wgrad_reduce_job: bad argument");
+    if (int e = check_wgrad_job(job, "u3d_conv3d_wgrad_reduce_job")) return e;
+    WgradParams p;
+    wgrad_plan(N, D, H, W, src->C0 + src->C1, Cout, p);
+    p.Cout = Cout;
+    const size_t need = (size_t)p.S * p.nchunks * p.nkb * 27 * 1024;
+    if (workspace_floats < need)
+        return u3d_set_err(U3D_EWORKSPACE, "u3d_conv3d_wgrad_reduce_job: workspace %zu < %zu floats", workspace_floats, need);
+    return wgrad_reduce_launch(stream, p, src->C0 + src->C1, dw, dw_cin_stride, workspace, job);
 }
 
 extern "C" int u3d_conv3d_variant(int N, int D, int H, int W, int Cin, int Cout, int src_kind, int has_workspace) {
diff --git a/pytorch-3dunet_amd/csrc/u3d_gn.h b/pytorch-3dunet_amd/csrc/u3d_gn.h
--- a/pytorch-3dunet_amd/csrc/u3d_gn.h
+++ b/pytorch-3dunet_amd/csrc/u3d_gn.h
@@ -1,5 +1,18 @@
 #pragma once
 #include "u3d_common.h"
+
+__device__ __forceinline__ f32x4 u3d_gn_bwd_quad(const f32x4& p, const f32x4& d, const f32x4& q, const f32x4& x, const f32x4& r) {
+#pragma clang fp contract(off)
+    f32x4 o;
+#pragma unroll
+    for (int e = 0; e < 4; ++e) o[e] = __builtin_fmaf(p[e], d[e], q[e] * x[e]) + r[e];
+    return o;
+}
+__device__ __forceinline__ f32x4 u3d_relu_mask_quad(f32x4 o, const f32x4& x) {
+#pragma unroll
+    for (int e = 0; e < 4; ++e) o[e] = x[e] > 0.f ? o[e] : 0.f;
+    return o;
+}
 
 __device__ __forceinline__ double u3d_sum_replicas(const double* __restrict__ p, size_t stride, int reps) {
     double v = p[0];
diff --git a/pytorch-3dunet_amd/csrc/u3d_ops.hip b/pytorch-3dunet_amd/csrc/u3d_ops.hip
--- a/pytorch-3dunet_amd/csrc/u3d_ops.hip
+++ b/pytorch-3dunet_amd/csrc/u3d_ops.hip
@@ -494,12 +494,9 @@
             const f32x4 p = *reinterpret_cast<const f32x4*>(coef + ((size_t)n * 3 + 0) * Ctot + coff + c);
             const f32x4 q = *reinterpret_cast<const f32x4*>(coef + ((size_t)n * 3 + 1) * Ctot + coff + c);
             const f32x4 r = *reinterpret_cast<const f32x4*>(coef + ((size_t)n * 3 + 2) * Ctot + coff + c);
-            f32x4 o = p * d + q * xv + r;
+            f32x4 o = u3d_gn_bwd_quad(p, d, q, xv, r);
             if (add) o += u3d_ldq(add + (size_t)v * Cx + c);
-            if (relu_mask) {
-#pragma unroll
-                for (int e = 0; e < 4; ++e) o[e] = xv[e] > 0.f ? o[e] : 0.f;
-            }
+            if (relu_mask) o = u3d_relu_mask_quad(o, xv);
             u3d_stq(out + (size_t)v * Cx + c, o);
         }
     } else {
diff --git a/pytorch-3dunet_amd/pytorch3dunet_amd/_engine_base.py b/pytorch-3dunet_amd/pytorch3dunet_amd/_engine_base.py
--- a/pytorch-3dunet_amd/pytorch3dunet_amd/_engine_base.py
+++ b/pytorch-3dunet_amd/pytorch3dunet_amd/_engine_base.py
@@ -437,6 +437,7 @@
         self._e = engine
         self.side = None
         self.ws_side = None
+        self.ws_vdz = None
         self.side_used = False
         self.coef_hi = None
 
@@ -448,6 +449,11 @@
         if self.ws.numel() < floats:
             self.ws = _empty(int(floats), dtype=_F32, device=self.dev)
         return self.ws
+
+    def ensure_ws_vdz(self, floats):
+        if self.ws_vdz is None or self.ws_vdz.numel() < floats:
+            self.ws_vdz = _empty(max(int(floats), 4), dtype=_F32, device=self.dev)
+        return self.ws_vdz
 
     def side_stream(self, ws_floats):
         if self.side is None:
diff --git a/pytorch-3dunet_amd/pytorch3dunet_amd/_engine_conv.py b/pytorch-3dunet_amd/pytorch3dunet_amd/_engine_conv.py
--- a/pytorch-3dunet_amd/pytorch3dunet_amd/_engine_conv.py
+++ b/pytorch-3dunet_amd/pytorch3dunet_amd/_engine_conv.py
@@ -17,6 +17,22 @@
 from ._engine_base import *
 
 _WGRAD_JOB = os.environ.get("U3D_WGRAD_JOB", "1") != "0"
+_FUSED_DZ = os.environ.get("U3D_FUSED_DZ", "1") != "0"
+
+
+@dataclass
+class VirtualDz:
+    dg: torch.Tensor
+    coef: torch.Tensor
+    x: torch.Tensor
+    relu_mask: int
+
+    def struct(self):
+        C = self.x.shape[-1]
+        s = nat.U3DDzSrc()
+        s.kind, s.relu_mask, s.dg, s.x, s.coef = 1, self.relu_mask, _p(self.dg), _p(self.x), _p(self.coef)
+        s.Cdg, s.coff, s.Ctot = C, 0, C
+        return s
 
 
 def _reps(t) -> int:
@@ -85,6 +101,7 @@
     b16: bool
     job: object = None
     greps: int = 1
+    vdz_ws: object = None
 
     @property
     def flops(self):
@@ -493,12 +510,20 @@
             nat.call("u3d_subpixel_conv_wgrad", dev.index, _stream(dev), _p(src.t1), _p(rec.affine.view(-1)[2 * C0:]), Ct * 2,
                      _p(c.dz), _p(dwv[C0 * 27:]), Ct, c.N, src.D1, src.H1, src.W1, C1, c.Cout, _p(ws), ws.numel(),
                      flops=128.0 * C1 * c.Cout * c.N * src.D1 * src.H1 * src.W1)
-        a0 = rec.affine_lo if rec.affine_lo is not None else rec.affine[:, :C0].contiguous()
-        s0 = VSrc(src.t0).struct(a0)
-        nat.call("u3d_conv3d_wgrad_job", dev.index, _stream(dev), ctypes.byref(s0), _p(c.dz), _p(dwv), Ct, c.N, c.D, c.H, c.W,
-                 c.Cout, _p(ws), ws.numel(), ctypes.byref(c.job) if c.job is not None else None,
-                 flops=54.0 * C0 * c.Cout * c.N * c.D * c.H * c.W)
+        s0 = self._skip_struct(rec, src)
+        if c.vdz_ws is not None:
+            nat.call("u3d_conv3d_wgrad_reduce_job", dev.index, _stream(dev), ctypes.byref(s0), _p(dwv), Ct, c.N, c.D, c.H, c.W, c.Cout,
+                     _p(c.vdz_ws), c.vdz_ws.numel(), ctypes.byref(c.job) if c.job is not None else None)
+        else:
+            nat.call("u3d_conv3d_wgrad_job", dev.index, _stream(dev), ctypes.byref(s0), _p(c.dz), _p(dwv), Ct, c.N, c.D, c.H, c.W,
+                     c.Cout, _p(ws), ws.numel(), ctypes.byref(c.job) if c.job is not None else None,
+                     flops=54.0 * C0 * c.Cout * c.N * c.D * c.H * c.W)
         c.job = None
+
+    @staticmethod
+    def _skip_struct(rec: ConvRec, src: VSrc):
+        a0 = rec.affine_lo if rec.affine_lo is not None else rec.affine[:, : rec.sub[0]].contiguous()
+        return VSrc(src.t0).struct(a0)
 
     def _wgrad_fp32_side(self, c: "_BwdCall"):
         cx, dev, src, rec = c.cx, c.cx.dev, c.src, c.rec
@@ -515,8 +540,12 @@
     def _wgrad_fp32(self, c: "_BwdCall"):
         cx, dev, src, rec, ws = c.cx, c.cx.dev, c.src, c.rec, c.cx.ws
         s_aff = src.struct(rec.affine)
-        nat.call("u3d_conv3d_wgrad_job", dev.index, _stream(dev), ctypes.byref(s_aff), _p(c.dz), _p(cx.gview(rec.idx_w)), 0, c.N, c.D,
-                 c.H, c.W, c.Cout, _p(ws), ws.numel(), ctypes.byref(c.job) if c.job is not None else None, flops=c.flops)
+        if c.vdz_ws is not None:
+            nat.call("u3d_conv3d_wgrad_reduce_job", dev.index, _stream(dev), ctypes.byref(s_aff), _p(cx.gview(rec.idx_w)), 0, c.N, c.D,
+                     c.H, c.W, c.Cout, _p(c.vdz_ws), c.vdz_ws.numel(), ctypes.byref(c.job) if c.job is not None else None)
+        else:
+            nat.call("u3d_conv3d_wgrad_job", dev.index, _stream(dev), ctypes.byref(s_aff), _p(c.dz), _p(cx.gview(rec.idx_w)), 0, c.N,
+                     c.D, c.H, c.W, c.Cout, _p(ws), ws.numel(), ctypes.byref(c.job) if c.job is not None else None, flops=c.flops)
         c.job = None
 
     def _dgrad_subpixel(self, c: "_BwdCall"):
@@ -602,6 +631,12 @@
         src = rec.src
         Nn, Dd, Hh, Ww = src.N, src.D, src.H, src.W
         Cout = rec.y.shape[-1]
+        vdz = None
+        if isinstance(dz_, VirtualDz):
+            if self._vdz_family(rec, dz_) is not None:
+                vdz, dz_ = dz_, _empty_like(dz_.x)
+            else:
+                dz_ = self._plain_apply(cx, dz_.dg, dz_.coef, dz_.x, dz_.relu_mask)
         if rec.drop is not None:
             kind, mask = rec.drop
             g = _empty_like(dz_)
@@ -642,6 +677,15 @@
         if (self.stat_reps > 1 and rec.pre_norm and rec.norm == "g" and _WGRAD_JOB and self._wgrad_family(call) in ("fp32", "subpixel")
                 and nat.get_lib().u3d_conv3d_wgrad_job_supported(Nn, src.C, rec.G) == 1):
             call.greps = self.stat_reps
+        if vdz is not None:
+            sub = rec.sub is not None
+            s_w = self._skip_struct(rec, src) if sub else src.struct(rec.affine)
+            Cw = rec.sub[0] if sub else src.C
+            wsv = cx.ensure_ws_vdz(nat.get_lib().u3d_wgrad_workspace_floats(Nn, Dd, Hh, Ww, Cw, Cout))
+            nat.call("u3d_conv3d_wgrad_vdz", dev.index, _stream(dev), ctypes.byref(s_w), ctypes.byref(vdz.struct()), _p(dz_), Nn, Dd, Hh,
+                     Ww, Cout, _p(wsv), wsv.numel(), flops=54.0 * Cw * Cout * Nn * Dd * Hh * Ww)
+            call.vdz_ws = wsv
+            del vdz
         dg, gst = getattr(self, self._DGRAD_KERNELS[self._dgrad_family(call)])(call)
         if self.debug is not None and rec.sub is None:
             self.debug[rec.name + ".dg"] = dg.clone()
@@ -656,6 +700,27 @@
         if not had_job or call.job is not None:
             self._norm_bwd_finalize(cx, rec, gst, Nn, src.C, float(Dd * Hh * Ww), coef)
         return dg, coef
+
+    def _vdz_family(self, rec: ConvRec, v: VirtualDz):
+        if not _FUSED_DZ or self.debug is not None or rec.drop is not None or rec.post is not None or rec.small:
+            return None
+        src = rec.src
+        Cout = rec.y.shape[-1]
+        if v.x.dtype != _F32 or v.dg.dtype != _F32 or v.x.shape != v.dg.shape or v.x.shape[-1] != Cout or src.t0.dtype != _F32:
+            return None
+        if src.t1 is None and rec.sub is None and self._bf16_layer(src.C, Cout):
+            return None
+        if rec.sub is not None:
+            fam, Cw, kind = "subpixel", rec.sub[0], 0
+        else:
+            if self.overlap_small_wgrad and src.N * src.D * src.H * src.W <= _BwdCtx.SIDE_MAX_VOXELS:
+                return None
+            fam, Cw, kind = "fp32", src.C, 0 if src.t1 is None else (1 if src.exact2x else 2)
+        if nat.get_lib().u3d_conv3d_wgrad_vdz_supported(src.N, src.D, src.H, src.W, Cw, Cout, kind) != 1:
+            return None
+        if any(t.data_ptr() % 16 for t in (v.dg, v.x, v.coef, src.t0)) or (src.t1 is not None and src.t1.data_ptr() % 16):
+            return None
+        return fam
 
     def _plain_apply(self, cx, dg, coef, x, relu_mask, add=None):
         dev = cx.dev
diff --git a/pytorch-3dunet_amd/pytorch3dunet_amd/_engine_unet.py b/pytorch-3dunet_amd/pytorch3dunet_amd/_engine_unet.py
--- a/pytorch-3dunet_amd/pytorch3dunet_amd/_engine_unet.py
+++ b/pytorch-3dunet_amd/pytorch3dunet_amd/_engine_unet.py
@@ -15,7 +15,7 @@
 from ._native import U3DSrc
 
 from ._engine_base import *
-from ._engine_conv import ConvLayers, _reps, _take_reps
+from ._engine_conv import ConvLayers, VirtualDz, _reps, _take_reps
 from ._engine_weights import WeightImages
 
 
@@ -263,6 +263,13 @@
         def plain_apply(dg, coef, x, relu_mask):
             return self._plain_apply(cx, dg, coef, x, relu_mask)
 
+        def dz_into_conv(dg, coef, x):
+            if self.act not in (ACT_LEAKY, ACT_ELU):
+                return VirtualDz(dg, coef, x, mk)
+            dz_ = plain_apply(dg, coef, x, mk)
+            self._unact(dev, dz_, x)
+            return dz_
+
         recs = tape.convs
         enc_recs = [(recs[2 * i], recs[2 * i + 1]) for i in range(n_levels)]
         dec_recs = [(recs[2 * n_levels + 2 * j], recs[2 * n_levels + 2 * j + 1]) for j in range(n_dec)]
@@ -270,8 +277,7 @@
         for j in range(n_dec - 1, -1, -1):
             r1, r2 = dec_recs[j]
             dg2, coef2 = conv_bwd(r2, dz)
-            dz1 = plain_apply(dg2, coef2, r2.src.t0, mk)
-            self._unact(dev, dz1, r2.src.t0)
+            dz1 = dz_into_conv(dg2, coef2, r2.src.t0)
             del dg2
             dg1, coef1 = conv_bwd(r1, dz1)
             src = tape.cats.get(j, r1.src)
@@ -334,8 +340,7 @@
         for i in range(n_levels - 1, -1, -1):
             r1, r2 = enc_recs[i]
             dg2, coef2 = conv_bwd(r2, dz)
-            dz1 = plain_apply(dg2, coef2, r2.src.t0, mk)
-            self._unact(dev, dz1, r2.src.t0)
+            dz1 = dz_into_conv(dg2, coef2, r2.src.t0)
             del dg2
             dg1, coef1 = conv_bwd(r1, dz1, need_dg=(i > 0 or need_input_grad))
             if self.grad_sync is not None:
diff --git a/pytorch-3dunet_amd/pytorch3dunet_amd/_native.py b/pytorch-3dunet_amd/pytorch3dunet_amd/_native.py
--- a/pytorch-3dunet_amd/pytorch3dunet_amd/_native.py
+++ b/pytorch-3dunet_amd/pytorch3dunet_amd/_native.py
@@ -38,6 +38,12 @@
     _fields_ = [("gstats_lo", c_void_p), ("gstats_hi", c_void_p), ("mean_rstd", c_void_p), ("gamma", c_void_p), ("dgamma", c_void_p),
                 ("dbeta", c_void_p), ("coef", c_void_p), ("coef_hi", c_void_p), ("count", ctypes.c_double), ("C0", c_int32),
                 ("C1", c_int32), ("N", c_int32), ("G", c_int32), ("hi_scale", ctypes.c_float), ("reps_lo", c_int32), ("reps_hi", c_int32), ("reserved", c_int32)]
+
+
+class U3DDzSrc(ctypes.Structure):
+
+    _fields_ = [("kind", c_int32), ("relu_mask", c_int32), ("dg", c_void_p), ("x", c_void_p), ("coef", c_void_p), ("Cdg", c_int32),
+                ("coff", c_int32), ("Ctot", c_int32), ("reserved", c_int32)]
 
 
 class U3DPackDesc(ctypes.Structure):
@@ -160,6 +166,15 @@
          c_float, c_void_p, c_void_p, c_int, c_void_p, c_void_p],
     ),
     "u3d_conv3d_wgrad_job_supported": (c_int, [c_int, c_int, c_int]),
+    "u3d_conv3d_wgrad_vdz_supported": (c_int, [c_int, c_int, c_int, c_int, c_int, c_int, c_int]),
+    "u3d_conv3d_wgrad_vdz": (
+        c_int,
+        [c_int, c_void_p, POINTER(U3DSrc), POINTER(U3DDzSrc), c_void_p, c_int, c_int, c_int, c_int, c_int, c_void_p, c_size_t],
+    ),
+    "u3d_conv3d_wgrad_reduce_job": (
+        c_int,
+        [c_int, c_void_p, POINTER(U3DSrc), c_void_p, c_int, c_int, c_int, c_int, c_int, c_int, c_void_p, c_size_t, POINTER(U3DGnBwdJob)],
+    ),
     "u3d_conv3d_wgrad_job": (
         c_int,
         [c_int, c_void_p, POINTER(U3DSrc), c_void_p, c_void_p, c_int, c_int, c_int, c_int, c_int, c_int, c_void_p, c_size_t,
```

Result: no change. 122.1, median of 6 (+0.9%).
